# uzh-rpg/rpg_ramnet

Measured on AMD Instinct MI355X. Metric: depth samples/sec (346x260 cropped to 256x344, 5-bin grids, K=5 grids + 1 frame per sample; training step), higher is better.
Workload: dtype f32; 1 GPU; EventScape-shaped 346x260 -> 256x344 crop, 5 event bins, K=5, batch 8/GPU, seq-len 8, 1xMI355X-per-rank train, state=convgru, SI loss on [image,events4], Adam, backward-weights co-scheduled on a side stream, decoders on a second stream; global_batch=8, seq_len=8, parallelism=dp1

## Files before the change

include/ramnet_hip.h:

```cpp
#ifndef RAMNET_HIP_H
#define RAMNET_HIP_H
#include <stddef.h>
#include <stdint.h>

#ifdef __cplusplus
extern "C" {
#endif

#define RAMNET_ABI_VERSION 25
#define RAMNET_E_BADARG 10001
#define RAMNET_E_UNSUPPORTED 10002

enum ramnet_in_mode {
    RAMNET_IN_PLAIN = 0,
    RAMNET_IN_CAT = 1,
    RAMNET_IN_CAT_MUL = 2,
    RAMNET_IN_UP2X = 3,
    RAMNET_IN_UP2X_SKIP = 4,
    RAMNET_IN_RELUMASK = 5,
    RAMNET_IN_S2D = 6,
    RAMNET_IN_PARITY4 = 7
};

enum ramnet_algo { RAMNET_ALGO_DIRECT = 0, RAMNET_ALGO_WINOGRAD = 1, RAMNET_ALGO_HEAD = 2, RAMNET_ALGO_WINOGRAD24 = 3, RAMNET_ALGO_WINOGRAD_2X4 = 4,
                   RAMNET_ALGO_WINOGRAD_2X4_SPLIT = 5, RAMNET_ALGO_DIRECT_SPLIT = 6 };

enum ramnet_epilogue {
    RAMNET_EPI_LINEAR = 0,
    RAMNET_EPI_RELU = 1,
    RAMNET_EPI_SIGMOID = 2,
    RAMNET_EPI_RES_RELU = 3,
    RAMNET_EPI_GRU_BLEND = 4,
    RAMNET_EPI_LSTM = 5,
    RAMNET_EPI_GRU_BWD = 6,
    RAMNET_EPI_SIGMOID_HR = 7
};

typedef struct ramnet_conv_desc {
    const float *x0, *x1, *xm;
    int ld0, ld1, ldm;
    int C0, C1;
    int in_mode;
    int B, Hin, Win;
    int ntaps, stride;
    int8_t dy[25], dx[25];
    uint8_t wtap[25];
    const float *w;
    const float *bias;
    int Cout;
    int Ho, Wo;
    int HoF, WoF;
    int osy, osx, ooy, oox;
    int epi;
    float beta;
    const float *e0, *e1;
    int lde0, lde1;
    float *out, *o1, *o2;
    int ldo, ldo1, ldo2;
    int algo;
    int frame;
    int out_s2d;
    int head_cin;
    int s2d_5x5;
    float *splitk_ws;
    size_t splitk_floats;
    const int *active;
} ramnet_conv_desc;

#define RAMNET_WGRAD_MAX_SEGMENTS 48
typedef struct ramnet_wgrad_seg {
    const float *x0, *x1, *xm, *dout, *gmask;
} ramnet_wgrad_seg;

typedef struct ramnet_wgrad_desc {
    const float *x0, *x1, *xm;
    int ld0, ld1, ldm, C0, C1, in_mode;
    int B, Hin, Win;
    int ntaps, stride;
    int8_t dy[25], dx[25];
    const float *dout, *gmask;
    int ldg, ldgm;
    int Cout, Ho, Wo;
    float *dw;
    float *dbias;
    int algo;
    int gsy, gsx, goy, gox;
    int HoG, WoG;
    int head_cin;
    int dw_slabs;
    int nseg;
    const ramnet_wgrad_seg *segs;
} ramnet_wgrad_desc;

int ramnet_set_option(const char *name, int value);
int ramnet_get_option(const char *name);
const char *ramnet_last_error(void);
int ramnet_abi_version(void);
const char *ramnet_last_kernel(void);
int ramnet_stream_fork(void *from, void *to);

int ramnet_gemm(const float *A, const float *B, float *C, int M, int N, int K, int lda, int ldb, int ldc, int trans_a,
                int accumulate, int batch, long stride_a, long stride_b, long stride_c, void *stream);
int ramnet_gemm2(const float *A, const float *B, float *C, int M, long stride_a, long stride_b, long stride_c, int batch, const float *A2,
                 const float *B2, float *C2, int M2, long stride_a2, long stride_b2, long stride_c2, int batch2, int N, int K, int K2, int lda,
                 int ldb, int ldc, int trans_a, int accumulate, void *stream);

int ramnet_nchw_to_nhwc_pad(const float *src, float *dst, int B, int C, int H, int W, int Cpad, void *stream);
int ramnet_reflect_pad(const float *src, float *dst, int B, int C, int H, int W, int Cpad, int top, int left, int Hc, int Wc, int nhwc,
                       void *stream);
int ramnet_wgrad_wino_slabs(int Cin, int Cout);
int ramnet_wgrad_wino2x4_slabs(int Cin, int Cout);
int ramnet_wgrad_dsplit_slabs(int Cin, int Cout);
size_t ramnet_wgrad_dsplit_ws_floats(int Cin, int Cout);
int ramnet_unpack_wgrad_dsplit(const float *ws, float *grad, int Cout, int Cin, int CinWs, int CoutWs, int n_off, void *stream);
size_t ramnet_wgrad_wino2x4_ws_floats(int Cin, int Cout);
int ramnet_reduce_slabs(float *ws, int slabs, size_t n, void *stream);
size_t ramnet_packed_weight_elems(int Cout, int Cin, int KH, int KW, int transposed, int gates);
size_t ramnet_packed_weight_elems_wino(int Cout, int Cin, int transposed, int gates);
int ramnet_pack_weight_wino(const float *w_oihw, float *wp, int Cout, int Cin, int transposed, int gates, void *stream);
size_t ramnet_packed_weight_elems_wino2x4(int Cout, int Cin, int transposed);
int ramnet_pack_weight_wino2x4(const float *w_oihw, float *wp, int Cout, int Cin, int transposed, void *stream);
int ramnet_conv_wino_variant(const ramnet_conv_desc *d, int force);
int ramnet_conv_wino_split_ok(const ramnet_conv_desc *d, int force);
size_t ramnet_packed_weight_elems_wino2x4_split(int Cout, int Cin, int transposed);
int ramnet_pack_weight_wino2x4_split(const float *w_oihw, float *wp, int Cout, int Cin, int transposed, void *stream);
size_t ramnet_conv_splitk_floats(const ramnet_conv_desc *d);
int ramnet_wino2x4_config(int min_wgs);
int ramnet_fold_wino_supported(int Cout, int Cin);
size_t ramnet_packed_weight_elems_fold_wino(int Cout, int Cin);
int ramnet_pack_weight_fold_wino(const float *w_oihw, float *wp, int Cout, int Cin, void *stream);
int ramnet_pack_weight_fold_wino_dgrad(const float *w_oihw, float *wp, int Cout, int Cin, void *stream);
int ramnet_pack_border_weights(const float *w_oihw, float *rows, float *cols, float *rows_t, float *cols_t, int Cout, int Cin, void *stream);
int ramnet_fold_unpack_wgrad(float *w4, float *dU, float *wr, float *wc, float *grad, int Cout, int Cin, int CinWs, void *stream);
size_t ramnet_packed_weight_elems_head(int Cin);
int ramnet_head_supported(int Cin, int Cout);
int ramnet_pack_weight_head(const float *w_oihw, float *wp, int Cout, int Cin, void *stream);
int ramnet_pack_weight(const float *w_oihw, float *wp, int Cout, int Cin, int KH, int KW,
                       int transposed, int gates, void *stream);
int ramnet_unpack_wgrad(const float *ws, float *grad_oihw, int Cout, int Cin, int CinWs, int CoutWs, int n_off,
                        int KH, int KW, void *stream);

int ramnet_unpack_wgrad_wino(const float *ws, float *grad_oihw, int Cout, int Cin, int CinWs, int CoutWs, int n_off,
                             void *stream);
int ramnet_unpack_wgrad_wino2x4(const float *ws, float *grad_oihw, int Cout, int Cin, int CinWs, int CoutWs, int n_off,
                                void *stream);

int ramnet_conv_launch(const ramnet_conv_desc *d, void *stream);
int ramnet_conv_launch_multi(const ramnet_conv_desc *descs, int n, void *stream);
int ramnet_wgrad_launch(const ramnet_wgrad_desc *d, void *stream);

int ramnet_pred_sigmoid_fwd(const float *x, int ldx, int C, const float *w, const float *b, float *y,
                            size_t npix, void *stream);
int ramnet_pred_sigmoid_bwd(const float *x, int ldx, int C, const float *w, const float *y, const float *dy,
                            float *dx, int lddx, float *dw, float *db, size_t npix, void *stream);
#define RAMNET_PRED_SI_MAX_SEGMENTS 8
size_t ramnet_pred_si_scratch_doubles(size_t seg_pix, int nseg);
int ramnet_pred_sigmoid_si_fwd(const float *x, int ldx, int C, const float *w, const float *b, float *y, size_t seg_pix, int nseg,
                               const float *const *targets, float weight, float lambda, double *scratch, double *stats, float *loss,
                               void *stream);
int ramnet_pred_sigmoid_si_bwd(const float *x, int ldx, int C, const float *w, const float *y, const float *dy, size_t seg_pix, int nseg,
                               const float *const *targets, const double *stats, const float *gscale, float weight, float lambda,
                               float *dx, int lddx, float *dw, float *db, double *scratch, int mask_x, void *stream);
int ramnet_pred_linear_fwd(const float *x, int ldx, int C, const float *w, const float *b, float *z, size_t npix, void *stream);
int ramnet_pred_linear_bwd(const float *x, int ldx, int C, const float *w, const float *dz, float *dx, int lddx, float *dw, float *db,
                           size_t npix, void *stream);
int ramnet_relu_bwd(const float *dy, const float *y, float *dx, size_t n, void *stream);
int ramnet_pad2_sum(const float *x, const float *skip, float *out, int B, int H, int W, int C, void *stream);
int ramnet_up2x_border_im2col(const float *x, const float *skip, float *rows, float *cols, int B, int H, int W, int C, void *stream);
int ramnet_pad2_sum_im2col(const float *x, const float *skip, float *out, float *rows, float *cols, int B, int H, int W, int C, void *stream);
int ramnet_unpad2_fold(const float *dxpad, float *dx, int B, int H, int W, int C, void *stream);
int ramnet_up2x_border_col2im(const float *rows, const float *cols, float *dx, int B, int H, int W, int C, void *stream);
int ramnet_frame_gather(const float *dy, const float *mask, float *rows, float *cols, int B, int H2, int W2, int C, void *stream);
int ramnet_space_to_depth2(const float *x, float *out, int B, int H, int W, int C, int inverse, void *stream);
int ramnet_upsample2x_bwd(const float *dup, float *dx, int B, int H, int W, int C, void *stream);
int ramnet_gru_bwd_a(const float *dhn, const float *ur, const float *o, const float *h, float *dpo,
                     float *dpur, float *dh, size_t npix, int C, int ld_dhn ,
                     void *stream);
int ramnet_gru_bwd_a2(const float *dhn, const float *ur, const float *o, const float *h, float *dpo,
                      float *dpur, float *dh, size_t npix, int C, int ld_dhn, int ld_dh ,
                      void *stream);
int ramnet_gru_bwd_b(const float *dxhr, const float *ur, const float *h, float *dpur, float *dh,
                     size_t npix, int C, void *stream);
int ramnet_lstm_bwd(const float *gates, const float *cprev, const float *cnew, const float *dhn,
                    const float *dcn, float *dpre, float *dcprev, size_t npix, int C, void *stream);
int ramnet_lstm_bwd_masked(const float *gates, const float *cprev, const float *cnew, const float *dhn, const float *dcn,
                           const int *active, float *dpre, float *dcprev, float *dxh, size_t npix, int hw, int C, void *stream);
int ramnet_bias_grad(const float *dy, const float *mask, float *db, size_t npix, int C, void *stream);
int ramnet_norm_slabs(int groups, long npix, int C);
int ramnet_norm_partial(const float *a, int lda, const float *y, int ldy, int act, const float *b, int ldb, int groups, long npix,
                        int C, int nslab, double *part, void *stream);
int ramnet_norm_finalize(const double *part, int groups, int nslab, int C, long npix, double eps, const float *gamma, const float *beta,
                         float *running_mean, float *running_var, double momentum, int update_running, int use_running,
                         long long *num_batches_tracked, double *mean, double *rstd, float *scale, float *shift, void *stream);
int ramnet_norm_finalize_bwd(const double *part, int groups, int nslab, int C, long npix, const double *mean, const double *rstd,
                             const float *gamma, int batch_stats, float *c1, float *c2, float *c3, float *dgamma, float *dbeta, void *stream);
int ramnet_norm_apply(const float *x, int ldx, const float *scale, const float *shift, const float *res, int ldr, int act, float *out,
                      int ldo, int groups, long npix, int C, void *stream);
int ramnet_norm_bwd(const float *dy, int lddy, const float *y, int ldy, int act, const float *x, int ldx, const float *c1, const float *c2,
                    const float *c3, float *dx, int lddx, float *dres, int lddres, int groups, long npix, int C, void *stream);
int ramnet_add(const float *a, const float *b, float *y, size_t n, void *stream);
int ramnet_concat2(const float *a, int lda, int Ca, const float *b, int ldb, int Cb, float *y, size_t npix, void *stream);
int ramnet_cat_batch_add(const float *const *parts, int n, size_t npix, int C, int ld, const float *base, float *out, void *stream);
int ramnet_cat_batch_add_masked(const float *const *parts, int n, size_t npix, int C, int ld, const float *base, const float *mask, float *out,
                                void *stream);
int ramnet_split2(const float *y, int ldy, int Ca, int Cb, float *a, float *b, size_t npix, void *stream);

int ramnet_si_loss_fwd(const float *pred, const float *target, size_t n, float weight, float lambda,
                       double *stats, float *loss, void *stream);
int ramnet_si_loss_from_stats(const double *stats, float weight, float lambda, float *loss, void *stream);
int ramnet_si_loss_bwd(const float *pred, const float *target, size_t n, float weight, float lambda,
                       const double *stats, const float *gscale, float *dpred, void *stream);

int ramnet_si_log_loss_fwd(const float *pred, const float *target, size_t n, float lambda, double *stats, float *loss, void *stream);
int ramnet_si_log_loss_bwd(const float *pred, const float *target, size_t n, float lambda, const double *stats, const float *gscale,
                           float *dpred, void *stream);
int ramnet_mse_loss_fwd(const float *pred, const float *target, int B, int H, int W, int half, double *stats, float *loss, void *stream);
int ramnet_mse_loss_bwd(const float *pred, const float *target, int B, int H, int W, int half, const double *stats, const float *gscale,
                        float *dpred, void *stream);

int ramnet_depth_metrics(const float *pred, const float *target, size_t n, float clip_distance, float reg_factor,
                         float cutoff, double *out11, void *stream);

size_t ramnet_msg_workspace_elems(int B, int H, int W, int num_scales);
int ramnet_msg_loss_fwd(const float *pred, const float *target, int B, int H, int W, int num_scales, float *ws,
                        double *stats, float *loss, void *stream);
int ramnet_msg_loss_bwd(const float *ws, const double *stats, const float *gscale, int B, int H, int W, int num_scales,
                        float *dws, float *dpred, void *stream);

int ramnet_voxelize(const double *events, size_t n_events, int bins, int W, int H, float *grid, void *stream);
int ramnet_voxel_indices(const double *events, size_t n_events, int bins, int W, int H,
                         long long *idx_left, long long *idx_right, void *stream);
int ramnet_normalize_nonzero(float *grid, size_t n, double *scratch, void *stream);
int ramnet_voxelize_batch(const double *events, const long long *offsets, int n_grids, size_t max_events, int bins, int W, int H,
                          float *grids, void *stream);
int ramnet_normalize_nonzero_batch(float *grids, int n_grids, size_t n, double *scratch, void *stream);

#ifdef __cplusplus
}
#endif
#endif
```

rpg_ramnet_amd/_hip.py:

```python
import ctypes as C
import os

_PKG = os.path.dirname(os.path.abspath(__file__))
LIB_PATH = os.environ.get("RAMNET_HIP_LIB") or os.path.join(_PKG, "librpg_ramnet_hip.so")

IN_PLAIN, IN_CAT, IN_CAT_MUL, IN_UP2X, IN_UP2X_SKIP, IN_RELUMASK, IN_S2D, IN_PARITY4 = range(8)
ALGO_DIRECT, ALGO_WINOGRAD, ALGO_HEAD, ALGO_WINOGRAD24, ALGO_WINOGRAD_2X4, ALGO_WINOGRAD_2X4_SPLIT, ALGO_DIRECT_SPLIT = 0, 1, 2, 3, 4, 5, 6
EPI_LINEAR, EPI_RELU, EPI_SIGMOID, EPI_RES_RELU, EPI_GRU_BLEND, EPI_LSTM, EPI_GRU_BWD, EPI_SIGMOID_HR = range(8)

_fp = C.c_void_p


class ConvDesc(C.Structure):
    _fields_ = [
        ("x0", _fp), ("x1", _fp), ("xm", _fp),
        ("ld0", C.c_int), ("ld1", C.c_int), ("ldm", C.c_int),
        ("C0", C.c_int), ("C1", C.c_int), ("in_mode", C.c_int),
        ("B", C.c_int), ("Hin", C.c_int), ("Win", C.c_int),
        ("ntaps", C.c_int), ("stride", C.c_int),
        ("dy", C.c_int8 * 25), ("dx", C.c_int8 * 25), ("wtap", C.c_uint8 * 25),
        ("w", _fp), ("bias", _fp),
        ("Cout", C.c_int), ("Ho", C.c_int), ("Wo", C.c_int), ("HoF", C.c_int), ("WoF", C.c_int),
        ("osy", C.c_int), ("osx", C.c_int), ("ooy", C.c_int), ("oox", C.c_int),
        ("epi", C.c_int), ("beta", C.c_float),
        ("e0", _fp), ("e1", _fp), ("lde0", C.c_int), ("lde1", C.c_int),
        ("out", _fp), ("o1", _fp), ("o2", _fp),
        ("ldo", C.c_int), ("ldo1", C.c_int), ("ldo2", C.c_int),
        ("algo", C.c_int),
        ("frame", C.c_int),
        ("out_s2d", C.c_int),
        ("head_cin", C.c_int),
        ("s2d_5x5", C.c_int),
        ("splitk_ws", C.c_void_p), ("splitk_floats", C.c_size_t),
        ("active", _fp),
    ]


class WgradSeg(C.Structure):
    _fields_ = [("x0", _fp), ("x1", _fp), ("xm", _fp), ("dout", _fp), ("gmask", _fp)]


WGRAD_MAX_SEGMENTS = 48


class WgradDesc(C.Structure):
    _fields_ = [
        ("x0", _fp), ("x1", _fp), ("xm", _fp),
        ("ld0", C.c_int), ("ld1", C.c_int), ("ldm", C.c_int),
        ("C0", C.c_int), ("C1", C.c_int), ("in_mode", C.c_int),
        ("B", C.c_int), ("Hin", C.c_int), ("Win", C.c_int),
        ("ntaps", C.c_int), ("stride", C.c_int),
        ("dy", C.c_int8 * 25), ("dx", C.c_int8 * 25),
        ("dout", _fp), ("gmask", _fp), ("ldg", C.c_int), ("ldgm", C.c_int),
        ("Cout", C.c_int), ("Ho", C.c_int), ("Wo", C.c_int),
        ("dw", _fp), ("dbias", _fp),
        ("algo", C.c_int),
        ("gsy", C.c_int), ("gsx", C.c_int), ("goy", C.c_int), ("gox", C.c_int), ("HoG", C.c_int), ("WoG", C.c_int),
        ("head_cin", C.c_int),
        ("dw_slabs", C.c_int),
        ("nseg", C.c_int), ("segs", C.POINTER(WgradSeg)),
    ]


_SIGS = {
    "ramnet_abi_version": (C.c_int, []),
    "ramnet_last_error": (C.c_char_p, []),
    "ramnet_set_option": (C.c_int, [C.c_char_p, C.c_int]),
    "ramnet_get_option": (C.c_int, [C.c_char_p]),
    "ramnet_last_kernel": (C.c_char_p, []),
    "ramnet_stream_fork": (C.c_int, [_fp, _fp]),
    "ramnet_gemm": (C.c_int, [_fp, _fp, _fp] + [C.c_int] * 9 + [C.c_long] * 3 + [_fp]),
    "ramnet_gemm2": (C.c_int, [_fp, _fp, _fp, C.c_int, C.c_long, C.c_long, C.c_long, C.c_int, _fp, _fp, _fp, C.c_int, C.c_long, C.c_long, C.c_long,
                               C.c_int, C.c_int, C.c_int, C.c_int, C.c_int, C.c_int, C.c_int, C.c_int, C.c_int, _fp]),
    "ramnet_nchw_to_nhwc_pad": (C.c_int, [_fp, _fp, C.c_int, C.c_int, C.c_int, C.c_int, C.c_int, _fp]),
    "ramnet_reflect_pad": (C.c_int, [_fp, _fp] + [C.c_int] * 10 + [_fp]),
    "ramnet_wgrad_wino_slabs": (C.c_int, [C.c_int, C.c_int]),
    "ramnet_wgrad_wino2x4_slabs": (C.c_int, [C.c_int, C.c_int]),
    "ramnet_wgrad_dsplit_slabs": (C.c_int, [C.c_int, C.c_int]),
    "ramnet_wgrad_dsplit_ws_floats": (C.c_size_t, [C.c_int, C.c_int]),
    "ramnet_unpack_wgrad_dsplit": (C.c_int, [_fp, _fp, C.c_int, C.c_int, C.c_int, C.c_int, C.c_int, _fp]),
    "ramnet_wgrad_wino2x4_ws_floats": (C.c_size_t, [C.c_int, C.c_int]),
    "ramnet_reduce_slabs": (C.c_int, [_fp, C.c_int, C.c_size_t, _fp]),
    "ramnet_packed_weight_elems": (C.c_size_t, [C.c_int] * 6),
    "ramnet_pack_weight": (C.c_int, [_fp, _fp, C.c_int, C.c_int, C.c_int, C.c_int, C.c_int, C.c_int, _fp]),
    "ramnet_packed_weight_elems_wino": (C.c_size_t, [C.c_int] * 4),
    "ramnet_pack_weight_wino": (C.c_int, [_fp, _fp, C.c_int, C.c_int, C.c_int, C.c_int, _fp]),
    "ramnet_packed_weight_elems_wino2x4": (C.c_size_t, [C.c_int] * 3),
    "ramnet_pack_weight_wino2x4": (C.c_int, [_fp, _fp, C.c_int, C.c_int, C.c_int, _fp]),
    "ramnet_wino2x4_config": (C.c_int, [C.c_int]),
    "ramnet_conv_wino_variant": (C.c_int, [C.POINTER(ConvDesc), C.c_int]),
    "ramnet_conv_wino_split_ok": (C.c_int, [C.POINTER(ConvDesc), C.c_int]),
    "ramnet_packed_weight_elems_wino2x4_split": (C.c_size_t, [C.c_int] * 3),
    "ramnet_pack_weight_wino2x4_split": (C.c_int, [_fp, _fp, C.c_int, C.c_int, C.c_int, _fp]),
    "ramnet_conv_splitk_floats": (C.c_size_t, [C.POINTER(ConvDesc)]),
    "ramnet_packed_weight_elems_head": (C.c_size_t, [C.c_int]),
    "ramnet_head_supported": (C.c_int, [C.c_int, C.c_int]),
    "ramnet_pack_weight_head": (C.c_int, [_fp, _fp, C.c_int, C.c_int, _fp]),
    "ramnet_fold_wino_supported": (C.c_int, [C.c_int, C.c_int]),
    "ramnet_packed_weight_elems_fold_wino": (C.c_size_t, [C.c_int, C.c_int]),
    "ramnet_pack_weight_fold_wino": (C.c_int, [_fp, _fp, C.c_int, C.c_int, _fp]),
    "ramnet_pack_weight_fold_wino_dgrad": (C.c_int, [_fp, _fp, C.c_int, C.c_int, _fp]),
    "ramnet_pack_border_weights": (C.c_int, [_fp] * 5 + [C.c_int, C.c_int, _fp]),
    "ramnet_fold_unpack_wgrad": (C.c_int, [_fp] * 5 + [C.c_int, C.c_int, C.c_int, _fp]),
    "ramnet_unpad2_fold": (C.c_int, [_fp, _fp, C.c_int, C.c_int, C.c_int, C.c_int, _fp]),
    "ramnet_up2x_border_col2im": (C.c_int, [_fp, _fp, _fp, C.c_int, C.c_int, C.c_int, C.c_int, _fp]),
    "ramnet_pad2_sum": (C.c_int, [_fp, _fp, _fp, C.c_int, C.c_int, C.c_int, C.c_int, _fp]),
    "ramnet_up2x_border_im2col": (C.c_int, [_fp, _fp, _fp, _fp, C.c_int, C.c_int, C.c_int, C.c_int, _fp]),
    "ramnet_pad2_sum_im2col": (C.c_int, [_fp, _fp, _fp, _fp, _fp, C.c_int, C.c_int, C.c_int, C.c_int, _fp]),
    "ramnet_space_to_depth2": (C.c_int, [_fp, _fp, C.c_int, C.c_int, C.c_int, C.c_int, C.c_int, _fp]),
    "ramnet_frame_gather": (C.c_int, [_fp, _fp, _fp, _fp, C.c_int, C.c_int, C.c_int, C.c_int, _fp]),
    "ramnet_unpack_wgrad": (C.c_int, [_fp, _fp] + [C.c_int] * 7 + [_fp]),
    "ramnet_unpack_wgrad_wino": (C.c_int, [_fp, _fp] + [C.c_int] * 5 + [_fp]),
    "ramnet_unpack_wgrad_wino2x4": (C.c_int, [_fp, _fp] + [C.c_int] * 5 + [_fp]),
    "ramnet_conv_launch": (C.c_int, [C.POINTER(ConvDesc), _fp]),
    "ramnet_conv_launch_multi": (C.c_int, [C.POINTER(ConvDesc), C.c_int, _fp]),
    "ramnet_wgrad_launch": (C.c_int, [C.POINTER(WgradDesc), _fp]),
    "ramnet_pred_sigmoid_fwd": (C.c_int, [_fp, C.c_int, C.c_int, _fp, _fp, _fp, C.c_size_t, _fp]),
    "ramnet_pred_sigmoid_bwd": (C.c_int, [_fp, C.c_int, C.c_int, _fp, _fp, _fp, _fp, C.c_int, _fp, _fp, C.c_size_t, _fp]),
    "ramnet_pred_si_scratch_doubles": (C.c_size_t, [C.c_size_t, C.c_int]),
    "ramnet_pred_sigmoid_si_fwd": (C.c_int, [_fp, C.c_int, C.c_int, _fp, _fp, _fp, C.c_size_t, C.c_int, C.POINTER(C.c_void_p), C.c_float, C.c_float,
                                             _fp, _fp, _fp, _fp]),
    "ramnet_pred_sigmoid_si_bwd": (C.c_int, [_fp, C.c_int, C.c_int, _fp, _fp, _fp, C.c_size_t, C.c_int, C.POINTER(C.c_void_p), _fp, _fp, C.c_float,
                                             C.c_float, _fp, C.c_int, _fp, _fp, _fp, C.c_int, _fp]),
    "ramnet_pred_linear_fwd": (C.c_int, [_fp, C.c_int, C.c_int, _fp, _fp, _fp, C.c_size_t, _fp]),
    "ramnet_pred_linear_bwd": (C.c_int, [_fp, C.c_int, C.c_int, _fp, _fp, _fp, C.c_int, _fp, _fp, C.c_size_t, _fp]),
    "ramnet_cat_batch_add": (C.c_int, [_fp, C.c_int, C.c_size_t, C.c_int, C.c_int, _fp, _fp, _fp]),
    "ramnet_cat_batch_add_masked": (C.c_int, [_fp, C.c_int, C.c_size_t, C.c_int, C.c_int, _fp, _fp, _fp, _fp]),
    "ramnet_relu_bwd": (C.c_int, [_fp, _fp, _fp, C.c_size_t, _fp]),
    "ramnet_upsample2x_bwd": (C.c_int, [_fp, _fp, C.c_int, C.c_int, C.c_int, C.c_int, _fp]),
    "ramnet_gru_bwd_a": (C.c_int, [_fp] * 7 + [C.c_size_t, C.c_int, C.c_int, _fp]),
    "ramnet_gru_bwd_a2": (C.c_int, [_fp] * 7 + [C.c_size_t, C.c_int, C.c_int, C.c_int, _fp]),
    "ramnet_gru_bwd_b": (C.c_int, [_fp] * 5 + [C.c_size_t, C.c_int, _fp]),
    "ramnet_lstm_bwd": (C.c_int, [_fp] * 7 + [C.c_size_t, C.c_int, _fp]),
    "ramnet_lstm_bwd_masked": (C.c_int, [_fp, _fp, _fp, _fp, _fp, _fp, _fp, _fp, _fp, C.c_size_t, C.c_int, C.c_int, _fp]),
    "ramnet_norm_slabs": (C.c_int, [C.c_int, C.c_long, C.c_int]),
    "ramnet_norm_partial": (C.c_int, [_fp, C.c_int, _fp, C.c_int, C.c_int, _fp, C.c_int, C.c_int, C.c_long, C.c_int, C.c_int, _fp, _fp]),
    "ramnet_norm_finalize": (C.c_int, [_fp, C.c_int, C.c_int, C.c_int, C.c_long, C.c_double, _fp, _fp, _fp, _fp, C.c_double, C.c_int, C.c_int,
                                       _fp, _fp, _fp, _fp, _fp, _fp]),
    "ramnet_norm_finalize_bwd": (C.c_int, [_fp, C.c_int, C.c_int, C.c_int, C.c_long, _fp, _fp, _fp, C.c_int, _fp, _fp, _fp, _fp, _fp, _fp]),
    "ramnet_norm_apply": (C.c_int, [_fp, C.c_int, _fp, _fp, _fp, C.c_int, C.c_int, _fp, C.c_int, C.c_int, C.c_long, C.c_int, _fp]),
    "ramnet_norm_bwd": (C.c_int, [_fp, C.c_int, _fp, C.c_int, C.c_int, _fp, C.c_int, _fp, _fp, _fp, _fp, C.c_int, _fp, C.c_int,
                                  C.c_int, C.c_long, C.c_int, _fp]),
    "ramnet_add": (C.c_int, [_fp, _fp, _fp, C.c_size_t, _fp]),
    "ramnet_split2": (C.c_int, [_fp, C.c_int, C.c_int, C.c_int, _fp, _fp, C.c_size_t, _fp]),
    "ramnet_concat2": (C.c_int, [_fp, C.c_int, C.c_int, _fp, C.c_int, C.c_int, _fp, C.c_size_t, _fp]),
    "ramnet_bias_grad": (C.c_int, [_fp, _fp, _fp, C.c_size_t, C.c_int, _fp]),
    "ramnet_si_loss_fwd": (C.c_int, [_fp, _fp, C.c_size_t, C.c_float, C.c_float, _fp, _fp, _fp]),
    "ramnet_si_loss_from_stats": (C.c_int, [_fp, C.c_float, C.c_float, _fp, _fp]),
    "ramnet_si_loss_bwd": (C.c_int, [_fp, _fp, C.c_size_t, C.c_float, C.c_float, _fp, _fp, _fp, _fp]),
    "ramnet_si_log_loss_fwd": (C.c_int, [_fp, _fp, C.c_size_t, C.c_float, _fp, _fp, _fp]),
    "ramnet_si_log_loss_bwd": (C.c_int, [_fp, _fp, C.c_size_t, C.c_float, _fp, _fp, _fp, _fp]),
    "ramnet_mse_loss_fwd": (C.c_int, [_fp, _fp, C.c_int, C.c_int, C.c_int, C.c_int, _fp, _fp, _fp]),
    "ramnet_mse_loss_bwd": (C.c_int, [_fp, _fp, C.c_int, C.c_int, C.c_int, C.c_int, _fp, _fp, _fp, _fp]),
    "ramnet_depth_metrics": (C.c_int, [_fp, _fp, C.c_size_t, C.c_float, C.c_float, C.c_float, _fp, _fp]),
    "ramnet_msg_workspace_elems": (C.c_size_t, [C.c_int] * 4),
    "ramnet_msg_loss_fwd": (C.c_int, [_fp, _fp, C.c_int, C.c_int, C.c_int, C.c_int, _fp, _fp, _fp, _fp]),
    "ramnet_msg_loss_bwd": (C.c_int, [_fp, _fp, _fp, C.c_int, C.c_int, C.c_int, C.c_int, _fp, _fp, _fp]),
    "ramnet_voxelize": (C.c_int, [_fp, C.c_size_t, C.c_int, C.c_int, C.c_int, _fp, _fp]),
    "ramnet_voxel_indices": (C.c_int, [_fp, C.c_size_t, C.c_int, C.c_int, C.c_int, _fp, _fp, _fp]),
    "ramnet_normalize_nonzero": (C.c_int, [_fp, C.c_size_t, _fp, _fp]),
    "ramnet_voxelize_batch": (C.c_int, [_fp, _fp, C.c_int, C.c_size_t, C.c_int, C.c_int, C.c_int, _fp, _fp]),
    "ramnet_normalize_nonzero_batch": (C.c_int, [_fp, C.c_int, C.c_size_t, _fp, _fp]),
}
EXPORTS = tuple(_SIGS)

_lib = None
_tracer = None


class _Traced:
    def __init__(self, l):
        self._l = l

    def __getattr__(self, name):
        fn = getattr(self._l, name)
        tr = _tracer
        if tr is None:
            return fn
        return lambda *a: tr(name, fn, a)


def set_tracer(fn):
    global _tracer
    _tracer = fn


class HipLibraryMissing(RuntimeError):
    pass


def lib():
    global _lib
    if _lib is None:
        if not os.path.exists(LIB_PATH):
            raise HipLibraryMissing(
                "%s not found: build it with `python -c 'import __graft_entry__ as g; g.build()'` "
                "(hipcc --offload-arch=gfx950). rpg_ramnet_amd has no CPU fallback." % LIB_PATH)
        import torch
        rt = os.path.join(os.path.dirname(torch.__file__), "lib", "libamdhip64.so")
        if os.path.exists(rt):
            C.CDLL(rt, mode=C.RTLD_GLOBAL)
        l = C.CDLL(LIB_PATH)
        for name, (res, args) in _SIGS.items():
            fn = getattr(l, name)
            fn.restype, fn.argtypes = res, args
        if l.ramnet_abi_version() != 25:
            raise RuntimeError("ABI version mismatch in %s" % LIB_PATH)
        _lib = l
    return _lib if _tracer is None else _Traced(_lib)


def check(code, what):
    if code != 0:
        msg = lib().ramnet_last_error()
        raise RuntimeError("%s failed (code %d): %s" % (what, code, msg.decode() if msg else "?"))
```

rpg_ramnet_amd/csrc/conv_igemm.hip:

```cpp
#include <stdlib.h>
#include "common.hpp"
#include "conv_epilogue.hpp"

namespace ramnet {

struct ConvCommon {
    InSrc src;
    int nchunks, CoutPad;
    int patch_floats;
    int nclass;
    int xcd_swizzle;
};

struct ConvClass {
    int ntaps, Ho, Wo, ooy, oox;
    int PH, PW, dymin, dxmin;
    int tiles_x, tiles_y;
    int toff[25];
    unsigned woff[25];
};
struct ConvClasses { ConvClass c[4]; };

template <int BM, int BN, int WM, int WN, bool MASK = false>
__global__ void __launch_bounds__(256) conv_igemm_kernel(const ramnet_conv_desc p, const ConvCommon qc, const ConvClasses qk) {
    int flat = blockIdx.x + gridDim.x * (blockIdx.y + gridDim.y * blockIdx.z);
    if (qc.xcd_swizzle) {
        const int nwg = gridDim.x * gridDim.y * gridDim.z, xcd = flat & 7, qq = nwg >> 3, rr = nwg & 7;
        flat = (xcd < rr ? xcd * (qq + 1) : rr * (qq + 1) + (xcd - rr) * qq) + (flat >> 3);
    }
    int bid = flat % gridDim.x;
    const int by = (flat / gridDim.x) % gridDim.y, bz = flat / (gridDim.x * gridDim.y);
    const ConvClass &q = qk.c[bz];
    constexpr int TM = BM / WM / 32, TN = BN / WN / 32;
    constexpr int TH = BM / TWID;
    constexpr int CKC = CK;
    static_assert(WM * WN == 4 && TM >= 1 && TN >= 1, "4 waves per workgroup");
    extern __shared__ __attribute__((aligned(16))) float smem[];
    float *patch = smem;
    float *wsm = smem + qc.patch_floats;

    const int tid = threadIdx.x, lane = tid & 63;
    const int wave = __builtin_amdgcn_readfirstlane(tid >> 6);
    const int wm = wave / WN, wn = wave % WN;
    const int l31 = lane & 31, kk = lane >> 5;

    if (bid >= q.tiles_x * q.tiles_y * p.B) return;
    const int tx_i = bid % q.tiles_x;
    bid /= q.tiles_x;
    const int ty_i = bid % q.tiles_y;
    const int b = bid / q.tiles_y;
    const int n0 = by * BN;
    const int oy0 = ty_i * TH, ox0 = tx_i * TWID;
    const int iy0 = oy0 * p.stride + q.dymin, ix0 = ox0 * p.stride + q.dxmin;

    int aBase[TM], bBase[TN];
#pragma unroll
    for (int ms = 0; ms < TM; ++ms) {
        const int m = (wm * TM + ms) * 32 + l31;
        aBase[ms] = (((m >> 4) * p.stride) * q.PW + (m & 15) * p.stride) * LDP + 4 * kk;
    }
#pragma unroll
    for (int ns = 0; ns < TN; ++ns) bBase[ns] = ((wn * TN + ns) * 32 + l31) * LDP + 4 * kk;

    f32x16 acc[TM][TN];
#pragma unroll
    for (int ms = 0; ms < TM; ++ms)
#pragma unroll
        for (int ns = 0; ns < TN; ++ns)
#pragma unroll
            for (int r = 0; r < 16; ++r) acc[ms][ns][r] = 0.f;

    constexpr int WF4 = BN * 4;
    constexpr int WPT = (WF4 + 255) / 256;
    float4 wreg[WPT];
    const int ntaps = q.ntaps;
    auto load_w = [&](int chunk, int t) {
        const float *src = p.w + ((size_t)q.woff[t] + ((size_t)chunk * qc.CoutPad + n0)) * 16;
#pragma unroll
        for (int i = 0; i < WPT; ++i) {
            const int f = tid + i * 256;
            if (WF4 % 256 == 0 || f < WF4) wreg[i] = ld4(src + (size_t)f * 4);
        }
    };
    auto store_w = [&](int buf) {
        float *dst = wsm + buf * (BN * LDP);
#pragma unroll
        for (int i = 0; i < WPT; ++i) {
            const int f = tid + i * 256;
            if (WF4 % 256 == 0 || f < WF4) st4(dst + (f >> 2) * LDP + (f & 3) * 4, wreg[i]);
        }
    };

    load_w(0, 0);
    int buf = 0;
    for (int chunk = 0; chunk < qc.nchunks; ++chunk) {
        __syncthreads();
        stage_patch<CKC / 4, LDP, 4, 256>(patch, qc.src, b, iy0, ix0, chunk * CKC, q.PH, q.PW, tid);
        for (int t = 0; t < ntaps; ++t) {
            store_w(buf);
            __syncthreads();
            if (t + 1 < ntaps) load_w(chunk, t + 1);
            else if (chunk + 1 < qc.nchunks) load_w(chunk + 1, 0);
            const float *pa = patch + q.toff[t];
            const float *wb = wsm + buf * (BN * LDP);
#pragma unroll
            for (int k8 = 0; k8 < 2; ++k8) {
                float4 a[TM], bb[TN];
#pragma unroll
                for (int ms = 0; ms < TM; ++ms) a[ms] = ld4(pa + aBase[ms] + k8 * 8);
#pragma unroll
                for (int ns = 0; ns < TN; ++ns) bb[ns] = ld4(wb + bBase[ns] + k8 * 8);
#pragma unroll
                for (int ms = 0; ms < TM; ++ms)
#pragma unroll
                    for (int ns = 0; ns < TN; ++ns) {
                        acc[ms][ns] = __builtin_amdgcn_mfma_f32_32x32x2f32(a[ms].x, bb[ns].x, acc[ms][ns], 0, 0, 0);
                        acc[ms][ns] = __builtin_amdgcn_mfma_f32_32x32x2f32(a[ms].y, bb[ns].y, acc[ms][ns], 0, 0, 0);
                        acc[ms][ns] = __builtin_amdgcn_mfma_f32_32x32x2f32(a[ms].z, bb[ns].z, acc[ms][ns], 0, 0, 0);
                        acc[ms][ns] = __builtin_amdgcn_mfma_f32_32x32x2f32(a[ms].w, bb[ns].w, acc[ms][ns], 0, 0, 0);
                    }
            }
            buf ^= 1;
        }
    }

    const int epi = p.epi;
    const bool act = !MASK || sample_active(p, b);
#pragma unroll
    for (int ms = 0; ms < TM; ++ms) {
#pragma unroll
        for (int r = 0; r < 16; ++r) {
            const int m = (wm * TM + ms) * 32 + (r & 3) + 8 * (r >> 2) + 4 * kk;
            const int oy = oy0 + (m >> 4), ox = ox0 + (m & 15);
            if (oy >= q.Ho || ox >= q.Wo) continue;
            const size_t pix = ((size_t)b * p.HoF + (oy * p.osy + q.ooy)) * p.WoF + (ox * p.osx + q.oox);
            const bool addold = epilogue_addold(p, oy * p.osy + q.ooy, ox * p.osx + q.oox);
            if (epi == RAMNET_EPI_LSTM) {
                if constexpr (TN == 4) {
                    const int C = p.Cout, ch = by * 32 + l31;
                    if (MASK && !act) {
                        if (ch < C) epilogue_inactive(p, epi, pix, ch);
                    } else if (ch < C) {
                        const float gi = sigmoidf_(acc[ms][0][r] + p.bias[ch]);
                        const float gf = sigmoidf_(acc[ms][1][r] + p.bias[C + ch]);
                        const float go = sigmoidf_(acc[ms][2][r] + p.bias[2 * C + ch]);
                        const float gc = tanhf_(acc[ms][3][r] + p.bias[3 * C + ch]);
                        const float cp = p.e1 ? p.e1[pix * p.lde1 + ch] : 0.f;
                        const float cn = gf * cp + gi * gc;
                        p.out[pix * p.ldo + ch] = go * tanhf_(cn);
                        p.o1[pix * p.ldo1 + ch] = cn;
                        if (p.o2) {
                            float *g = p.o2 + pix * p.ldo2 + ch;
                            g[0] = gi, g[C] = gf, g[2 * C] = go, g[3 * C] = gc;
                        }
                    }
                }
                continue;
            }
#pragma unroll
            for (int ns = 0; ns < TN; ++ns) {
                const int n = n0 + (wn * TN + ns) * 32 + l31;
                if (n >= p.Cout) continue;
                if (MASK && !act) {
                    epilogue_inactive(p, epi, pix, n);
                    continue;
                }
                epilogue_store(p, epi, pix, n, acc[ms][ns][r] + epilogue_side(p, epi, b, oy * p.osy + q.ooy, ox * p.osx + q.oox, n), addold);
            }
        }
    }
}

template <int BM, int BN, int WM, int WN>
static int launch_cfg(const ramnet_conv_desc &d, const ConvCommon &qc, const ConvClasses &qk, int max_tiles, hipStream_t st) {
    auto kern = d.active ? conv_igemm_kernel<BM, BN, WM, WN, true> : conv_igemm_kernel<BM, BN, WM, WN>;
    const size_t lds = ((size_t)qc.patch_floats + 2 * BN * LDP) * sizeof(float);
    static size_t lds_set[2] = {0, 0};
    if (lds > lds_set[d.active != nullptr]) {
        RAMNET_FULL_LDS((kern));
        lds_set[d.active != nullptr] = 160 * 1024;
    }
    if (lds > 160 * 1024) {
        set_error("conv patch does not fit LDS (%zu bytes)", lds);
        return RAMNET_E_UNSUPPORTED;
    }
    dim3 grid(max_tiles * d.B, qc.CoutPad / BN, qc.nclass);
    note_kernel(d.active ? "conv_igemm_kernel<%d,%d,%d,%d,masked>" : "conv_igemm_kernel<%d,%d,%d,%d>", BM, BN, WM, WN);
    hipLaunchKernelGGL(kern, grid, dim3(256), lds, st, d, qc, qk);
    RAMNET_LAUNCH_CHECK();
    return 0;
}

static int check_desc(const ramnet_conv_desc &d) {
    RAMNET_CHECK_ARG(d.x0 && d.w && d.out);
    RAMNET_CHECK_ARG(d.ntaps >= 1 && d.ntaps <= 25 && (d.stride == 1 || d.stride == 2));
    RAMNET_CHECK_ARG(d.B > 0 && d.Ho > 0 && d.Wo > 0 && d.Hin > 0 && d.Win > 0 && d.Cout > 0);
    RAMNET_CHECK_ARG(d.C0 > 0 && d.C0 % 4 == 0 && d.ld0 % 4 == 0 && d.ldo > 0);
    RAMNET_CHECK_ARG(d.osy >= 1 && d.osx >= 1);
    const bool cat = d.in_mode == RAMNET_IN_CAT || d.in_mode == RAMNET_IN_CAT_MUL;
    if (cat) RAMNET_CHECK_ARG(d.x1 && d.C1 > 0 && d.C1 % 4 == 0 && d.ld1 % 4 == 0);
    if (d.in_mode == RAMNET_IN_CAT_MUL || d.in_mode == RAMNET_IN_RELUMASK) RAMNET_CHECK_ARG(d.xm && d.ldm % 4 == 0);
    if (d.in_mode == RAMNET_IN_UP2X_SKIP) RAMNET_CHECK_ARG(d.x1 && d.ld1 % 4 == 0);
    if (d.in_mode == RAMNET_IN_UP2X || d.in_mode == RAMNET_IN_UP2X_SKIP) RAMNET_CHECK_ARG(d.Hin % 2 == 0 && d.Win % 2 == 0);
    if (d.epi == RAMNET_EPI_RES_RELU) RAMNET_CHECK_ARG(d.e0);
    if (d.epi == RAMNET_EPI_GRU_BLEND) RAMNET_CHECK_ARG(d.e0);
    if (d.epi == RAMNET_EPI_LSTM) RAMNET_CHECK_ARG(d.o1 && d.bias);
    if (d.epi == RAMNET_EPI_GRU_BWD) RAMNET_CHECK_ARG(d.e0 && d.o1 && d.Cout % 8 == 0 && !d.bias && d.beta == 0.f && d.frame == 0 && d.out_s2d == 0);
    if (d.epi == RAMNET_EPI_SIGMOID_HR) RAMNET_CHECK_ARG(d.e1 && d.o1 && d.Cout % 8 == 0 && d.beta == 0.f && d.frame == 0 && d.out_s2d == 0 &&
                                                         d.algo != RAMNET_ALGO_WINOGRAD24 && d.algo != RAMNET_ALGO_HEAD);
    {
        unsigned long long ld = (unsigned long long)d.ld0;
        if (cat || d.in_mode == RAMNET_IN_UP2X_SKIP) ld = ld > (unsigned long long)d.ld1 ? ld : (unsigned long long)d.ld1;
        if (d.xm) ld = ld > (unsigned long long)d.ldm ? ld : (unsigned long long)d.ldm;
        const unsigned long long px = (unsigned long long)d.B * d.Hin * d.Win * (d.in_mode == RAMNET_IN_S2D ? 4 : 1);
        RAMNET_CHECK_ARG(px * ld < (1ull << 32));
    }
    RAMNET_CHECK_ARG(d.frame >= 0);
    if (d.active) RAMNET_CHECK_ARG((d.epi == RAMNET_EPI_SIGMOID || d.epi == RAMNET_EPI_SIGMOID_HR || d.epi == RAMNET_EPI_GRU_BLEND ||
                                    (d.epi == RAMNET_EPI_LSTM && d.e0)) && d.frame == 0 && d.out_s2d == 0 &&
                                   (d.algo == RAMNET_ALGO_DIRECT || d.algo == RAMNET_ALGO_WINOGRAD || d.algo == RAMNET_ALGO_WINOGRAD_2X4 ||
                                    d.algo == RAMNET_ALGO_WINOGRAD_2X4_SPLIT));
    if (d.frame > 0) RAMNET_CHECK_ARG(d.e0 && d.e1 && (d.epi == RAMNET_EPI_RELU || d.epi == RAMNET_EPI_LINEAR));
    return 0;
}

static int launch_classes(const ramnet_conv_desc *ds, int n, hipStream_t st) {
    const ramnet_conv_desc &d = ds[0];
    for (int i = 0; i < n; ++i) {
        const int rc = check_desc(ds[i]);
        if (rc) return rc;
        RAMNET_CHECK_ARG(ds[i].x0 == d.x0 && ds[i].w == d.w && ds[i].out == d.out && ds[i].stride == d.stride &&
                         ds[i].Cout == d.Cout && ds[i].epi == d.epi && ds[i].osy == d.osy && ds[i].osx == d.osx &&
                         ds[i].B == d.B && ds[i].in_mode == d.in_mode && ds[i].active == d.active);
    }
    const bool cat = d.in_mode == RAMNET_IN_CAT || d.in_mode == RAMNET_IN_CAT_MUL;
    ConvCommon qc;
    ConvClasses qk;
    qc.src.x0 = d.x0, qc.src.x1 = d.x1, qc.src.xm = d.xm;
    qc.src.ld0 = d.ld0, qc.src.ld1 = d.ld1, qc.src.ldm = d.ldm;
    qc.src.C0 = d.C0, qc.src.Cin = d.C0 + (cat ? d.C1 : 0);
    qc.src.mode = d.in_mode, qc.src.Hin = d.Hin, qc.src.Win = d.Win;
    qc.nchunks = cdiv(qc.src.Cin, CK);
    qc.CoutPad = d.epi == RAMNET_EPI_LSTM ? 4 * roundup(d.Cout, 32) : roundup(d.Cout, 32);
    qc.nclass = n;
    qc.xcd_swizzle = 0;
    const int lstm = d.epi == RAMNET_EPI_LSTM;
    int BM = 128, BN = lstm ? 128 : (qc.CoutPad % 128 == 0 ? 128 : qc.CoutPad % 64 == 0 ? 64 : 32);
    auto blocks = [&](int bm, int bn) {
        long t = 0;
        for (int i = 0; i < n; ++i) t += (long)cdiv(ds[i].Wo, TWID) * cdiv(ds[i].Ho, bm / TWID);
        return t * d.B * (qc.CoutPad / bn);
    };
    if (!lstm && BN >= 64) {
        const long want = 768;
        if (blocks(BM, BN) < want) BM = 64;
        if (blocks(BM, BN) < want && BN == 128) BN = 64;
    }
    if (!lstm && BN == 32 && blocks(256, 32) >= 1024)
        BM = 256;
    const int TH = BM / TWID;
    int max_tiles = 0;
    qc.patch_floats = 0;
    for (int i = 0; i < n; ++i) {
        const ramnet_conv_desc &e = ds[i];
        ConvClass &q = qk.c[i];
        int dymin = 127, dymax = -127, dxmin = 127, dxmax = -127;
        for (int t = 0; t < e.ntaps; ++t) {
            dymin = e.dy[t] < dymin ? e.dy[t] : dymin, dymax = e.dy[t] > dymax ? e.dy[t] : dymax;
            dxmin = e.dx[t] < dxmin ? e.dx[t] : dxmin, dxmax = e.dx[t] > dxmax ? e.dx[t] : dxmax;
        }
        q.ntaps = e.ntaps, q.Ho = e.Ho, q.Wo = e.Wo, q.ooy = e.ooy, q.oox = e.oox;
        q.dymin = dymin, q.dxmin = dxmin;
        q.PH = (TH - 1) * e.stride + (dymax - dymin) + 1;
        q.PW = (TWID - 1) * e.stride + (dxmax - dxmin) + 1;
        q.tiles_x = cdiv(e.Wo, TWID), q.tiles_y = cdiv(e.Ho, TH);
        for (int t = 0; t < e.ntaps; ++t) {
            q.toff[t] = ((e.dy[t] - dymin) * q.PW + (e.dx[t] - dxmin)) * LDP;
            q.woff[t] = (unsigned)e.wtap[t] * (unsigned)qc.nchunks * (unsigned)qc.CoutPad;
        }
        if (q.PH * q.PW * LDP > qc.patch_floats) qc.patch_floats = q.PH * q.PW * LDP;
        if (q.tiles_x * q.tiles_y > max_tiles) max_tiles = q.tiles_x * q.tiles_y;
    }
    if (lstm) return launch_cfg<128, 128, 4, 1>(d, qc, qk, max_tiles, st);
    if (BM == 128 && BN == 128) return launch_cfg<128, 128, 2, 2>(d, qc, qk, max_tiles, st);
    if (BM == 128 && BN == 64) return launch_cfg<128, 64, 2, 2>(d, qc, qk, max_tiles, st);
    if (BM == 64 && BN == 128) return launch_cfg<64, 128, 2, 2>(d, qc, qk, max_tiles, st);
    if (BM == 64 && BN == 64) return launch_cfg<64, 64, 2, 2>(d, qc, qk, max_tiles, st);
    if (BM == 256) return launch_cfg<256, 32, 4, 1>(d, qc, qk, max_tiles, st);
    return launch_cfg<128, 32, 4, 1>(d, qc, qk, max_tiles, st);
}

}

using namespace ramnet;

extern "C" int ramnet_conv_launch(const ramnet_conv_desc *dp, void *stream) {
    RAMNET_CHECK_ARG(dp != nullptr);
    if (dp->algo == RAMNET_ALGO_WINOGRAD) {
        const int rc = check_desc(*dp);
        return rc ? rc : launch_wino(*dp, (hipStream_t)stream);
    }
    if (dp->algo == RAMNET_ALGO_WINOGRAD_2X4) {
        const int rc = check_desc(*dp);
        return rc ? rc : launch_wino6(*dp, (hipStream_t)stream);
    }
    if (dp->algo == RAMNET_ALGO_WINOGRAD_2X4_SPLIT) {
        const int rc = check_desc(*dp);
        return rc ? rc : launch_wino6s(*dp, (hipStream_t)stream);
    }
    if (dp->algo == RAMNET_ALGO_WINOGRAD24) {
        const int rc = check_desc(*dp);
        return rc ? rc : launch_wino24(*dp, (hipStream_t)stream);
    }
    if (dp->algo == RAMNET_ALGO_HEAD) {
        const int rc = check_desc(*dp);
        return rc ? rc : launch_head(*dp, (hipStream_t)stream);
    }
    RAMNET_CHECK_ARG(dp->algo == RAMNET_ALGO_DIRECT && dp->in_mode != RAMNET_IN_S2D && dp->out_s2d == 0);
    return launch_classes(dp, 1, (hipStream_t)stream);
}

extern "C" int ramnet_conv_launch_multi(const ramnet_conv_desc *descs, int n, void *stream) {
    RAMNET_CHECK_ARG(descs != nullptr && n >= 1 && n <= 4);
    for (int i = 0; i < n; ++i) RAMNET_CHECK_ARG(descs[i].in_mode != RAMNET_IN_S2D && descs[i].out_s2d == 0);
    return launch_classes(descs, n, (hipStream_t)stream);
}
```

rpg_ramnet_amd/csrc/conv_wino24.hip:

```cpp
#include <stdlib.h>
#include "common.hpp"
#include "conv_epilogue.hpp"

typedef float f32x4 __attribute__((ext_vector_type(4)));

namespace ramnet {

constexpr int W24_PS = 512;
constexpr int W24_V = 25 * W24_PS;

__device__ __forceinline__ float2 ld2f(const float *p) { return *reinterpret_cast<const float2 *>(p); }

__device__ __forceinline__ auto make_rsrc(const void *p, unsigned bytes) {
    const unsigned long long a = (unsigned long long)p;
    const unsigned lo = __builtin_amdgcn_readfirstlane((unsigned)a), hi = __builtin_amdgcn_readfirstlane((unsigned)(a >> 32));
    return __builtin_amdgcn_make_buffer_rsrc((void *)(((unsigned long long)hi << 32) | lo), (short)0, (int)bytes, 0x00020000);
}

#ifdef W24_TRACE
__device__ unsigned long long *g_w24_trace;
#define W24_STAMP(chunk_, slot)                                                                                          \
    do {                                                                                                                 \
        if (lane == 0 && (chunk_) <= 16) g_w24_trace[(((size_t)blockIdx.x * 8 + wave) * 17 + (chunk_)) * 6 + (slot)] = __builtin_amdgcn_s_memtime(); \
    } while (0)
#else
#define W24_STAMP(chunk_, slot)
#endif

struct Wino24Params {
    const float *x;
    const float *wp;
    int Hp, Wp, ldx, nchunks, nblk, tiles_x, tiles_y, Hc, Wc;
    int cpc;
    unsigned xbytes, wbytes;
    int ksplit;
    float *ws;
    int *cnt;
};

template <int NCQ, bool DG, int TXW, bool PAIR = false>
__global__ void __launch_bounds__(512, 1) conv_wino24_kernel(const ramnet_conv_desc p, const Wino24Params q) {
    static_assert(!PAIR || (NCQ == 4 && !DG), "pair mode: forward, 64-column workgroups");
    constexpr int W24_K = NCQ == 4 ? 16 : 8;
    constexpr int W24_TX = TXW, W24_TY = (NCQ == 4 ? 32 : 64) / TXW;
    constexpr int VEC = W24_K / 4;
    constexpr int W24_U = 25 * NCQ * 64 * VEC;
    extern __shared__ __attribute__((aligned(16))) float smem[];
    float *V = smem;
    const int tid = threadIdx.x, lane = tid & 63;
    const int wave = __builtin_amdgcn_readfirstlane(tid >> 6);
    const int l15 = lane & 15, ks = lane >> 4;
    const int th = NCQ == 4 ? wave & 1 : wave & 3, cq = NCQ == 4 ? wave >> 1 : wave >> 2;

    int bid = blockIdx.x;
    const int cls = DG ? 0 : PAIR ? bid & 1 : bid & 3;
    if (!DG) bid >>= PAIR ? 1 : 2;
    const int nb = bid % q.nblk;
    bid /= q.nblk;
    const int tbx = bid % q.tiles_x;
    bid /= q.tiles_x;
    const int tby = bid % q.tiles_y, b = bid / q.tiles_y;
    const int py = PAIR ? cls : cls >> 1, px = PAIR ? 0 : cls & 1;
    const int n0 = nb * 16 * NCQ;

    const int it = tid / W24_K, ik = tid % W24_K;
    const int iy0 = 2 * (tby * W24_TY + it / W24_TX) + py, ix0 = 2 * (tbx * W24_TX + it % W24_TX) + px;
    unsigned rowo[5], colo[5];
    int cur_cls = -1;
    auto set_class = [&](int c) {
        cur_cls = c;
        const int cy = c >> 1, cx = c & 1;
        const int u0 = 2 * (tby * W24_TY + it / W24_TX), v0 = 2 * (tbx * W24_TX + it % W24_TX);
#pragma unroll
        for (int r = 0; r < 5; ++r) {
            const int i = u0 - cy - 3 + r, j = v0 - cx - 3 + r;
            rowo[r] = (unsigned)i < (unsigned)q.Hc ? 4u * (unsigned)((b * q.Hp + 2 * i + cy) * q.Wp * q.ldx) : 0x40000000u;
            colo[r] = (unsigned)j < (unsigned)q.Wc ? 4u * (unsigned)((2 * j + cx) * q.ldx + ik) : 0x40000000u;
        }
    };
    if (!DG) {
#pragma unroll
        for (int r = 0; r < 5; ++r)
            rowo[r] = 4u * (unsigned)((b * q.Hp + min(iy0 + r, q.Hp - 1)) * q.Wp * q.ldx), colo[r] = 4u * (unsigned)(min(ix0 + r, q.Wp - 1) * q.ldx + ik);
    }
    const int ksp = DG ? 1 : q.ksplit;
    const int cps = ((q.nchunks / 2 + ksp - 1) / ksp) * 2, cbeg = DG ? 0 : (int)blockIdx.y * cps;
    const auto xrs = make_rsrc(q.x + cbeg * W24_K, q.xbytes - (unsigned)cbeg * W24_K * 4u);
    const int vdst = NCQ == 4 ? it * 16 + (((ik >> 2) ^ ((it >> 2) & 3)) << 2) + (ik & 3) : it * 8 + (((ik >> 1) ^ ((it >> 3) & 1)) << 1) + (ik & 1);
    float raw[25];
    auto load_raw = [&](int chunk) {
        int soff = chunk * (W24_K * 4);
        if (DG) {
            const int c = chunk / q.cpc;
            if (c != cur_cls) set_class(c);
            soff = (chunk - c * q.cpc) * (W24_K * 4);
        }
#pragma unroll
        for (int r = 0; r < 5; ++r)
#pragma unroll
            for (int c = 0; c < 5; ++c)
                raw[r * 5 + c] = __builtin_bit_cast(float, __builtin_amdgcn_raw_buffer_load_b32(xrs, (int)(rowo[r] + colo[c]), soff, 0));
    };
    int lr_soff = 0;
    auto load_row_begin = [&](int chunk) {
        lr_soff = chunk * (W24_K * 4);
        if (DG) {
            const int c = chunk / q.cpc;
            if (c != cur_cls) set_class(c);
            lr_soff = (chunk - c * q.cpc) * (W24_K * 4);
        }
    };
    auto load_row = [&](int r) {
#pragma unroll
        for (int c = 0; c < 5; ++c)
            raw[r * 5 + c] = __builtin_bit_cast(float, __builtin_amdgcn_raw_buffer_load_b32(xrs, (int)(rowo[r] + colo[c]), lr_soff, 0));
    };
    auto tr_col = [&](int c) {
        const float d0 = raw[c], d1 = raw[5 + c], d2 = raw[10 + c], d3 = raw[15 + c], d4 = raw[20 + c];
        raw[c] = 2.f * (d0 - d2) - d1 + d3;
        raw[5 + c] = d3 - d2 - 2.f * d1;
        raw[10 + c] = 2.f * d1 - 3.f * d2 + d3;
        raw[15 + c] = d3 - d1;
        raw[20 + c] = 2.f * (d1 - d3) - d2 + d4;
    };
    auto tr_row = [&](float *vbuf, int i) {
        const float d0 = raw[i * 5], d1 = raw[i * 5 + 1], d2 = raw[i * 5 + 2], d3 = raw[i * 5 + 3], d4 = raw[i * 5 + 4];
        float *dst = vbuf + (i * 5) * W24_PS + vdst;
        dst[0 * W24_PS] = 2.f * (d0 - d2) - d1 + d3;
        dst[1 * W24_PS] = d3 - d2 - 2.f * d1;
        dst[2 * W24_PS] = 2.f * d1 - 3.f * d2 + d3;
        dst[3 * W24_PS] = d3 - d1;
        dst[4 * W24_PS] = 2.f * (d1 - d3) - d2 + d4;
    };

    const int tile = th * 16 + l15;
    const int aoff = NCQ == 4 ? tile * 16 + ((ks ^ ((tile >> 2) & 3)) << 2) : tile * 8 + ((ks ^ ((tile >> 3) & 1)) << 1);
    constexpr int WPOS = NCQ * 64 * VEC;
    const auto wrs = make_rsrc(q.wp, q.wbytes);
    const int wsrc = (((cls * q.nchunks + cbeg) * q.nblk + nb) * W24_U + cq * (64 * VEC)) * 4;
    const int wlane = lane * VEC * 4;
    auto ldv = [&](const float *ptr) {
        if (VEC == 4) return ld4(ptr);
        const float2 t = ld2f(ptr);
        return make_float4(t.x, t.y, 0.f, 0.f);
    };
    auto ldw = [&](int soff) {
        if constexpr (VEC == 4) {
            return __builtin_bit_cast(float4, __builtin_amdgcn_raw_buffer_load_b128(wrs, wlane, soff, 0));
        } else {
            const float2 t = __builtin_bit_cast(float2, __builtin_amdgcn_raw_buffer_load_b64(wrs, wlane, soff, 0));
            return make_float4(t.x, t.y, 0.f, 0.f);
        }
    };
    const int wchunk = q.nblk * W24_U * 4;

    f32x4 acc[25];
#pragma unroll
    for (int i = 0; i < 25; ++i) acc[i] = f32x4{0.f, 0.f, 0.f, 0.f};

    const int nch = DG ? q.nchunks : min(cps, q.nchunks - cbeg);
    W24_STAMP(16, 0);
    load_raw(0);
    constexpr int RING = 10, DIST = 8;
    float4 bq[RING];
#pragma unroll
    for (int i = 0; i < DIST; ++i) bq[i] = ldw(wsrc + i * (WPOS * 4));
#pragma unroll
    for (int c = 0; c < 5; ++c) tr_col(c);
#pragma unroll
    for (int i = 0; i < 5; ++i) tr_row(V, i);
    load_raw(min(1, nch - 1));
    __syncthreads();

    W24_STAMP(16, 1);
    for (int chunk0 = 0; chunk0 < nch; chunk0 += 2) {
#pragma unroll
        for (int half = 0; half < 2; ++half) {
            const int chunk = chunk0 + half;
            const float *vb = V + half * W24_V;
            float *vn = V + (half ^ 1) * W24_V;
            const int cnext = min(chunk + 1, nch - 1), cnext2 = min(chunk + 2, nch - 1);
            const int wcur = wsrc + chunk * wchunk, wnext = wsrc + cnext * wchunk;
            W24_STAMP(chunk, 0);
            float4 aq[2][2];
            aq[0][0] = ldv(vb + aoff), aq[0][1] = ldv(vb + W24_PS + aoff);
#pragma unroll
            for (int pp = 0; pp < 13; ++pp) {
                const int pos = 2 * pp, g = half * 25 + pos;
                const bool two = pos + 1 < 25;
                if (pos + 2 < 25) aq[(pp + 1) & 1][0] = ldv(vb + (pos + 2) * W24_PS + aoff);
                if (pos + 3 < 25) aq[(pp + 1) & 1][1] = ldv(vb + (pos + 3) * W24_PS + aoff);
                const float4 a0 = aq[pp & 1][0], a1 = aq[pp & 1][1];
#if !defined(W24_ABLATE) || !(W24_ABLATE & 2)
                bq[(g + DIST) % RING] = pos + DIST < 25 ? ldw(wcur + (pos + DIST) * (WPOS * 4)) : ldw(wnext + (pos + DIST - 25) * (WPOS * 4));
                if (two) bq[(g + 1 + DIST) % RING] = pos + 1 + DIST < 25 ? ldw(wcur + (pos + 1 + DIST) * (WPOS * 4)) : ldw(wnext + (pos + 1 + DIST - 25) * (WPOS * 4));
#endif
                const float4 b0 = bq[g % RING], b1 = bq[(g + 1) % RING];
                __builtin_amdgcn_sched_barrier(0);
                acc[pos] = __builtin_amdgcn_mfma_f32_16x16x4f32(a0.x, b0.x, acc[pos], 0, 0, 0);
                if (two) acc[pos + 1] = __builtin_amdgcn_mfma_f32_16x16x4f32(a1.x, b1.x, acc[pos + 1], 0, 0, 0);
                acc[pos] = __builtin_amdgcn_mfma_f32_16x16x4f32(a0.y, b0.y, acc[pos], 0, 0, 0);
                if (two) acc[pos + 1] = __builtin_amdgcn_mfma_f32_16x16x4f32(a1.y, b1.y, acc[pos + 1], 0, 0, 0);
                __builtin_amdgcn_sched_barrier(0);
                auto slot = [&](int sl) {
                    if (sl == 4) W24_STAMP(chunk, 1);
                    if (sl >= 4 && sl <= 8) tr_col(sl - 4);
                    if (sl == 9) W24_STAMP(chunk, 2);
                    if (sl >= 9 && sl <= 17 && (sl & 1)) tr_row(vn, (sl - 9) >> 1);
#if !defined(W24_ABLATE) || !(W24_ABLATE & 1)
                    if (sl == 10) load_row_begin(cnext2);
                    if (sl >= 10 && sl <= 18 && !(sl & 1)) load_row((sl - 10) >> 1);
#endif
                    if (sl == 18) W24_STAMP(chunk, 3);
                };
                slot(2 * pp);
                __builtin_amdgcn_sched_barrier(0);
                if (VEC == 4) {
                    acc[pos] = __builtin_amdgcn_mfma_f32_16x16x4f32(a0.z, b0.z, acc[pos], 0, 0, 0);
                    if (two) acc[pos + 1] = __builtin_amdgcn_mfma_f32_16x16x4f32(a1.z, b1.z, acc[pos + 1], 0, 0, 0);
                    acc[pos] = __builtin_amdgcn_mfma_f32_16x16x4f32(a0.w, b0.w, acc[pos], 0, 0, 0);
                    if (two) acc[pos + 1] = __builtin_amdgcn_mfma_f32_16x16x4f32(a1.w, b1.w, acc[pos + 1], 0, 0, 0);
                }
                __builtin_amdgcn_sched_barrier(0);
                slot(2 * pp + 1);
                __builtin_amdgcn_sched_barrier(0);
            }
            W24_STAMP(chunk, 4);
            __syncthreads();
            W24_STAMP(chunk, 5);
        }
    }
    W24_STAMP(16, 2);

    const int ncol = n0 + cq * 16 + l15;
    const int pxc = PAIR ? ncol >> 5 : px, n = PAIR ? ncol & 31 : ncol;
    if (n >= p.Cout) return;
    const int epi = p.epi;
    const float bias_n = (!DG && p.bias) ? p.bias[n] : 0.f;
    const bool relu = epi == RAMNET_EPI_RELU;
    float ov[16];
    size_t op[16];
    bool oo[16];
#pragma unroll
    for (int r = 0; r < 4; ++r) {
        float s[2][5];
#pragma unroll
        for (int j = 0; j < 5; ++j) {
            const float m0 = acc[j][r], m1 = acc[5 + j][r], m2 = acc[10 + j][r], m3 = acc[15 + j][r], m4 = acc[20 + j][r];
            s[0][j] = m0 + m1 + m2 + m3;
            s[1][j] = m1 - m2 + 2.f * m3 + m4;
        }
#pragma unroll
        for (int a2 = 0; a2 < 2; ++a2) {
            ov[(r * 2 + a2) * 2] = s[a2][0] + s[a2][1] + s[a2][2] + s[a2][3];
            ov[(r * 2 + a2) * 2 + 1] = s[a2][1] - s[a2][2] + 2.f * s[a2][3] + s[a2][4];
        }
    }
    if (!DG && ksp > 1) {
        typedef unsigned u32x4 __attribute__((ext_vector_type(4)));
        constexpr int AUX_SC1 = 16;
        const auto wr = make_rsrc(q.ws + (size_t)blockIdx.x * ksp * 8192, (unsigned)(ksp * 8192 * 4));
#pragma unroll
        for (int i = 0; i < 4; ++i)
            __builtin_amdgcn_raw_buffer_store_b128(__builtin_bit_cast(u32x4, make_float4(ov[4 * i], ov[4 * i + 1], ov[4 * i + 2], ov[4 * i + 3])), wr,
                                                   (i * 512 + tid) * 16, (int)blockIdx.y * 32768, AUX_SC1);
        __builtin_amdgcn_fence(__ATOMIC_RELEASE, "workgroup");
        __syncthreads();
        if (tid == 0) {
            const int arrived = __hip_atomic_fetch_add(q.cnt + blockIdx.x, 1, __ATOMIC_RELAXED, __HIP_MEMORY_SCOPE_AGENT);
            if (arrived == ksp - 1) __hip_atomic_store(q.cnt + blockIdx.x, 0, __ATOMIC_RELAXED, __HIP_MEMORY_SCOPE_AGENT);
            reinterpret_cast<int *>(smem)[0] = arrived == ksp - 1;
        }
        __syncthreads();
        if (!reinterpret_cast<int *>(smem)[0]) return;
#pragma unroll
        for (int i = 0; i < 16; ++i) ov[i] = 0.f;
        for (int sp = 0; sp < ksp; ++sp)
#pragma unroll
            for (int i = 0; i < 4; ++i) {
                const float4 t = __builtin_bit_cast(float4, __builtin_amdgcn_raw_buffer_load_b128(wr, (i * 512 + tid) * 16, sp * 32768, AUX_SC1));
                ov[4 * i] += t.x, ov[4 * i + 1] += t.y, ov[4 * i + 2] += t.z, ov[4 * i + 3] += t.w;
            }
    }
#pragma unroll
    for (int r = 0; r < 4; ++r) {
        const int t = th * 16 + 4 * ks + r;
        const int oy0 = 2 * (tby * W24_TY + t / W24_TX), ox0 = 2 * (tbx * W24_TX + t % W24_TX) - (PAIR ? pxc : 0);
#pragma unroll
        for (int a2 = 0; a2 < 2; ++a2) {
#pragma unroll
            for (int c2 = 0; c2 < 2; ++c2) {
                const int oy = oy0 + a2, ox = ox0 + c2, idx = (r * 2 + a2) * 2 + c2;
                if (DG) {
                    oo[idx] = oy < p.Ho && ox < p.Wo;
                    op[idx] = (((size_t)b * p.Ho + oy) * p.Wo + ox) * p.ldo + n;
                    continue;
                }
                oo[idx] = !(oy >= q.Hc || ox >= q.Wc || (PAIR && ox < 0));
                const int oyF = 2 * oy + py, oxF = 2 * ox + pxc;
                op[idx] = (((size_t)b * p.HoF + oyF) * p.WoF + oxF) * p.ldo + n;
                float v = ov[idx] + bias_n;
                if (oo[idx]) v += epilogue_side(p, epi, b, oyF, oxF, n);
                ov[idx] = relu ? fmaxf(v, 0.f) : v;
            }
        }
    }
#pragma unroll
    for (int idx = 0; idx < 16; ++idx)
        if (oo[idx]) p.out[op[idx]] = ov[idx];
    W24_STAMP(16, 3);
}

__global__ void pack_weight_fold_wino_kernel(const float *__restrict__ w, float *__restrict__ wp, int Cout, int Cin, int kc, int ncq,
                                             int pair, size_t total) {
    const double FA[2][4][5] = {{{.25, 0, 0, 0, 0}, {.75, .75, .25, 0, 0}, {0, .25, .75, .75, .25}, {0, 0, 0, .25, .75}},
                                {{.75, .25, 0, 0, 0}, {.25, .75, .75, .25, 0}, {0, 0, .25, .75, .75}, {0, 0, 0, 0, .25}}};
    const double G[5][4] = {{0.5, 0, 0, 0}, {-0.5, -0.5, -0.5, -0.5}, {-1.0 / 6, 1.0 / 6, -1.0 / 6, 1.0 / 6}, {1.0 / 6, 1.0 / 3, 2.0 / 3, 4.0 / 3}, {0, 0, 0, 1}};
    const int vec = kc / 4, nblk = pair ? 1 : Cout / (16 * ncq), nch = Cin / kc;
    for (size_t i = blockIdx.x * (size_t)blockDim.x + threadIdx.x; i < total; i += (size_t)gridDim.x * blockDim.x) {
        size_t r = i;
        const int j = (int)(r % vec);
        r /= vec;
        const int l15 = (int)(r % 16);
        r /= 16;
        const int ks = (int)(r % 4);
        r /= 4;
        const int cq = (int)(r % ncq);
        r /= ncq;
        const int pos = (int)(r % 25);
        r /= 25;
        const int nb = (int)(r % nblk);
        r /= nblk;
        const int chunk = (int)(r % nch), cls = (int)(r / nch);
        const int k = chunk * kc + ks * vec + j, col = (nb * ncq + cq) * 16 + l15;
        const int n = pair ? col & 31 : col;
        const int py = pair ? cls : cls >> 1, px = pair ? col >> 5 : cls & 1, a = pos / 5, b = pos % 5;
        double ga[5], gb[5];
        for (int kh = 0; kh < 5; ++kh) {
            ga[kh] = 0, gb[kh] = 0;
            for (int t = 0; t < 4; ++t) ga[kh] += G[a][t] * FA[py][t][kh], gb[kh] += G[b][t] * FA[px][t][kh];
        }
        double u = 0;
        const float *wk = w + ((size_t)n * Cin + k) * 25;
        for (int kh = 0; kh < 5; ++kh)
            for (int kw = 0; kw < 5; ++kw) u += ga[kh] * gb[kw] * (double)wk[kh * 5 + kw];
        wp[i] = (float)u;
    }
}

static bool fold_wino_pair(int Cout, int Cin) {
    return Cout == 32 && Cin % 32 == 0 && g_opt_fold_pair;
}

static bool fold_wino_geometry(int Cout, int Cin, int &kc, int &ncq) {
    kc = ((Cout % 64 == 0 && Cin % 16 == 0) || fold_wino_pair(Cout, Cin)) ? 16 : 8, ncq = kc == 16 ? 4 : 2;
    return Cout % 32 == 0 && Cin % (2 * kc) == 0;
}

static int launch_wino24_dgrad(const ramnet_conv_desc &d, hipStream_t st) {
    RAMNET_CHECK_ARG(d.stride == 1 && d.C0 % 16 == 0 && d.Cout % 64 == 0);
    RAMNET_CHECK_ARG(d.Hin % 2 == 0 && d.Win % 2 == 0 && d.Ho == d.Hin / 2 + 4 && d.Wo == d.Win / 2 + 4 && d.HoF == d.Ho && d.WoF == d.Wo);
    RAMNET_CHECK_ARG(d.epi == RAMNET_EPI_LINEAR && !d.bias && d.beta == 0.f && d.frame == 0 && d.out_s2d == 0);
    Wino24Params q;
    q.x = d.x0, q.wp = d.w, q.Hp = d.Hin, q.Wp = d.Win, q.ldx = d.ld0;
    q.cpc = d.C0 / 16, q.nchunks = 4 * q.cpc, q.nblk = d.Cout / 64;
    q.ksplit = 1, q.ws = nullptr, q.cnt = nullptr;
    q.Hc = d.Hin / 2, q.Wc = d.Win / 2;
    const size_t xb = (size_t)d.B * d.Hin * d.Win * d.ld0 * sizeof(float), wb = (size_t)100 * d.C0 * d.Cout * sizeof(float);
    RAMNET_CHECK_ARG(xb < 0x40000000ull && wb < 0x7fffffffull);
    q.xbytes = (unsigned)xb, q.wbytes = (unsigned)wb;
    const bool flat = cdiv(d.Wo, 16) * cdiv(d.Ho, 8) < cdiv(d.Wo, 8) * cdiv(d.Ho, 16);
    q.tiles_x = cdiv(d.Wo, flat ? 16 : 8), q.tiles_y = cdiv(d.Ho, flat ? 8 : 16);
    const size_t lds = (size_t)2 * W24_V * sizeof(float);
    const dim3 grid((unsigned)(q.tiles_x * q.tiles_y * d.B * q.nblk));
    if (flat) {
        RAMNET_FULL_LDS((conv_wino24_kernel<4, true, 8>));
        note_kernel("conv_wino24_kernel<4,1,8,0>");
        hipLaunchKernelGGL((conv_wino24_kernel<4, true, 8>), grid, dim3(512), lds, st, d, q);
    } else {
        RAMNET_FULL_LDS((conv_wino24_kernel<4, true, 4>));
        note_kernel("conv_wino24_kernel<4,1,4,0>");
        hipLaunchKernelGGL((conv_wino24_kernel<4, true, 4>), grid, dim3(512), lds, st, d, q);
    }
    RAMNET_LAUNCH_CHECK();
    return 0;
}

static int wino24_ksplit(const ramnet_conv_desc &d, int gridx, int nchunks) {
    if (!g_opt_wino_ksplit || d.in_mode != RAMNET_IN_PLAIN) return 1;
    const bool pair = fold_wino_pair(d.Cout, d.C0), wide = pair || (d.Cout % 64 == 0 && d.C0 % 16 == 0);
    if (!pair && d.Cout % (wide ? 64 : 32) != 0) return 1;
    int ks = 256 / gridx < 4 ? 256 / gridx : 4;
    if (nchunks / 4 < ks) ks = nchunks / 4;
    if (g_opt_wino_ksplit > 1) ks = g_opt_wino_ksplit < nchunks / 2 ? g_opt_wino_ksplit : nchunks / 2;
    if (ks < 1) ks = 1;
    while (ks > 1 && (ks - 1) * (cdiv(nchunks / 2, ks) * 2) >= nchunks) --ks;
    return ks;
}
static size_t wino24_ksplit_floats(unsigned gridx, int ks) { return (size_t)cdiv((int)gridx, 64) * 64 + (size_t)gridx * ks * 8192; }

size_t wino24_splitk_floats(const ramnet_conv_desc &d) {
    if (d.in_mode != RAMNET_IN_PLAIN || d.C0 % 16 != 0 || d.Cout % 32 != 0) return 0;
    const bool pair = fold_wino_pair(d.Cout, d.C0), wide = pair || (d.Cout % 64 == 0 && d.C0 % 16 == 0);
    if (d.C0 % (wide ? 32 : 16) != 0) return 0;
    const int nchunks = d.C0 / (wide ? 16 : 8), nblk = pair ? 1 : d.Cout / (wide ? 64 : 32);
    const int Wt = pair ? d.Wo + 2 : d.Wo;
    const bool flat = wide && cdiv(Wt, 16) * cdiv(d.Ho, 8) < cdiv(Wt, 8) * cdiv(d.Ho, 16);
    const int tiles_x = cdiv(Wt, wide && !flat ? 8 : 16), tiles_y = cdiv(d.Ho, flat ? 8 : 16);
    const unsigned gridx = (unsigned)(tiles_x * tiles_y * d.B * nblk * (pair ? 2 : 4));
    const int ks = wino24_ksplit(d, (int)gridx, nchunks);
    return ks > 1 ? wino24_ksplit_floats(gridx, ks) : 0;
}

int launch_wino24(const ramnet_conv_desc &d, hipStream_t st) {
    if (d.in_mode == RAMNET_IN_PARITY4) return launch_wino24_dgrad(d, st);
    RAMNET_CHECK_ARG(d.in_mode == RAMNET_IN_PLAIN && d.stride == 1);
    const bool pair = fold_wino_pair(d.Cout, d.C0);
    const bool wide = pair || (d.Cout % 64 == 0 && d.C0 % 16 == 0);
    RAMNET_CHECK_ARG(d.C0 % (wide ? 32 : 16) == 0);
    RAMNET_CHECK_ARG(d.C0 % 8 == 0 && d.Cout % 32 == 0 && d.Hin == d.Ho + 4 && d.Win == d.Wo + 4 && d.HoF == 2 * d.Ho && d.WoF == 2 * d.Wo);
    RAMNET_CHECK_ARG((d.epi == RAMNET_EPI_RELU || d.epi == RAMNET_EPI_LINEAR) && d.beta == 0.f && d.out_s2d == 0 && d.Ho >= 2 && d.Wo >= 2);
    Wino24Params q;
    q.x = d.x0, q.wp = d.w, q.Hp = d.Hin, q.Wp = d.Win, q.ldx = d.ld0;
    q.nchunks = d.C0 / (wide ? 16 : 8), q.nblk = pair ? 1 : d.Cout / (wide ? 64 : 32);
    q.Hc = d.Ho, q.Wc = d.Wo, q.cpc = 1;
    const size_t xb = (size_t)d.B * d.Hin * d.Win * d.ld0 * sizeof(float), wb = (size_t)100 * d.C0 * d.Cout * sizeof(float);
    RAMNET_CHECK_ARG(xb < 0xffffffffull && wb < 0x7fffffffull);
    q.xbytes = (unsigned)xb, q.wbytes = (unsigned)wb;
    const int Wt = pair ? d.Wo + 2 : d.Wo;
    const bool flat = wide && cdiv(Wt, 16) * cdiv(d.Ho, 8) < cdiv(Wt, 8) * cdiv(d.Ho, 16);
    q.tiles_x = cdiv(Wt, wide && !flat ? 8 : 16), q.tiles_y = cdiv(d.Ho, flat ? 8 : 16);
    const size_t lds = (size_t)2 * W24_V * sizeof(float);
    const unsigned gridx = (unsigned)(q.tiles_x * q.tiles_y * d.B * q.nblk * (pair ? 2 : 4));
    const int want = wino24_ksplit(d, (int)gridx, q.nchunks);
    q.ksplit = d.splitk_ws ? want : 1;
    q.cnt = reinterpret_cast<int *>(d.splitk_ws);
    q.ws = d.splitk_ws ? d.splitk_ws + cdiv((int)gridx, 64) * 64 : nullptr;
    if (q.ksplit > 1) RAMNET_CHECK_ARG(d.splitk_floats >= wino24_ksplit_floats(gridx, want) && ((uintptr_t)d.splitk_ws & 15) == 0);
    const dim3 grid(gridx, q.ksplit);
    if (pair && flat) {
        RAMNET_FULL_LDS((conv_wino24_kernel<4, false, 8, true>));
        note_kernel("conv_wino24_kernel<4,0,8,1>");
        hipLaunchKernelGGL((conv_wino24_kernel<4, false, 8, true>), grid, dim3(512), lds, st, d, q);
    } else if (pair) {
        RAMNET_FULL_LDS((conv_wino24_kernel<4, false, 4, true>));
        note_kernel("conv_wino24_kernel<4,0,4,1>");
        hipLaunchKernelGGL((conv_wino24_kernel<4, false, 4, true>), grid, dim3(512), lds, st, d, q);
    } else if (wide && flat) {
        RAMNET_FULL_LDS((conv_wino24_kernel<4, false, 8>));
        note_kernel("conv_wino24_kernel<4,0,8,0>");
        hipLaunchKernelGGL((conv_wino24_kernel<4, false, 8>), grid, dim3(512), lds, st, d, q);
    } else if (wide) {
        RAMNET_FULL_LDS((conv_wino24_kernel<4, false, 4>));
        note_kernel("conv_wino24_kernel<4,0,4,0>");
        hipLaunchKernelGGL((conv_wino24_kernel<4, false, 4>), grid, dim3(512), lds, st, d, q);
    } else {
        RAMNET_FULL_LDS((conv_wino24_kernel<2, false, 8>));
        note_kernel("conv_wino24_kernel<2,0,8,0>");
        hipLaunchKernelGGL((conv_wino24_kernel<2, false, 8>), grid, dim3(512), lds, st, d, q);
    }
    RAMNET_LAUNCH_CHECK();
    return 0;
}

__global__ void pack_weight_fold_wino_dgrad_kernel(const float *__restrict__ w, float *__restrict__ wp, int Cout, int Cin, size_t total) {
    const double FA[2][4][5] = {{{.25, 0, 0, 0, 0}, {.75, .75, .25, 0, 0}, {0, .25, .75, .75, .25}, {0, 0, 0, .25, .75}},
                                {{.75, .25, 0, 0, 0}, {.25, .75, .75, .25, 0}, {0, 0, .25, .75, .75}, {0, 0, 0, 0, .25}}};
    const double G[5][4] = {{0.5, 0, 0, 0}, {-0.5, -0.5, -0.5, -0.5}, {-1.0 / 6, 1.0 / 6, -1.0 / 6, 1.0 / 6}, {1.0 / 6, 1.0 / 3, 2.0 / 3, 4.0 / 3}, {0, 0, 0, 1}};
    const int NB = Cin / 64;
    for (size_t i = blockIdx.x * (size_t)blockDim.x + threadIdx.x; i < total; i += (size_t)gridDim.x * blockDim.x) {
        size_t r = i;
        const int j = (int)(r & 3), l15 = (int)((r >> 2) & 15), ks = (int)((r >> 6) & 3), cq = (int)((r >> 8) & 3);
        r >>= 10;
        const int pos = (int)(r % 25);
        r /= 25;
        const int nb = (int)(r % NB), chunk = (int)(r / NB);
        const int k = chunk * 16 + ks * 4 + j, c = nb * 64 + cq * 16 + l15;
        const int pq = k / Cout, n = k - pq * Cout, pp = pq >> 1, qq = pq & 1, a = pos / 5, b = pos % 5;
        double ga[5], gb[5];
        for (int kh = 0; kh < 5; ++kh) {
            ga[kh] = 0, gb[kh] = 0;
            for (int t = 0; t < 4; ++t) ga[kh] += G[a][t] * FA[pp][3 - t][kh], gb[kh] += G[b][t] * FA[qq][3 - t][kh];
        }
        double u = 0;
        const float *wk = w + ((size_t)n * Cin + c) * 25;
        for (int kh = 0; kh < 5; ++kh)
            for (int kw = 0; kw < 5; ++kw) u += ga[kh] * gb[kw] * (double)wk[kh * 5 + kw];
        wp[i] = (float)u;
    }
}

__global__ void pack_border_weights_kernel(const float *__restrict__ w, float *__restrict__ rows, float *__restrict__ cols, float *__restrict__ rows_t,
                                           float *__restrict__ cols_t, int Cout, int Cin, size_t total) {
    for (size_t i = blockIdx.x * (size_t)blockDim.x + threadIdx.x; i < total; i += (size_t)gridDim.x * blockDim.x) {
        size_t r = i;
        const int co = (int)(r % Cout);
        r /= Cout;
        const int slot = (int)(r & 1);
        r >>= 1;
        const int ci = (int)(r % Cin);
        r /= Cin;
        const int kb = (int)(r % 5), side = (int)(r / 5);
        const int a0 = side == 0 ? 0 : (slot == 0 ? 4 : 3), na = side == 0 ? (slot == 0 ? 2 : 1) : (slot == 0 ? 1 : 2);
        const float *wk = w + ((size_t)co * Cin + ci) * 25;
        float sr = 0.f, sc = 0.f;
        for (int e = 0; e < na; ++e) sr += wk[(a0 + e) * 5 + kb], sc += wk[kb * 5 + (a0 + e)];
        const size_t K = (size_t)kb * Cin + ci, N = (size_t)slot * Cout + co;
        rows[((size_t)side * 5 * Cin + K) * 2 * Cout + N] = -sr;
        cols[((size_t)side * 5 * Cin + K) * 2 * Cout + N] = -sc;
        rows_t[((size_t)side * 2 * Cout + N) * 5 * Cin + K] = -sr;
        cols_t[((size_t)side * 2 * Cout + N) * 5 * Cin + K] = -sc;
    }
}

__global__ void fold_unpack_wgrad_kernel(float *__restrict__ w4, float *__restrict__ dU, float *__restrict__ wr, float *__restrict__ wc,
                                         float *__restrict__ grad, int Cout, int Cin, int CinWs) {
    const float FA[2][4][5] = {{{.25f, 0, 0, 0, 0}, {.75f, .75f, .25f, 0, 0}, {0, .25f, .75f, .75f, .25f}, {0, 0, 0, .25f, .75f}},
                               {{.75f, .25f, 0, 0, 0}, {.25f, .75f, .75f, .25f, 0}, {0, 0, .25f, .75f, .75f}, {0, 0, 0, 0, .25f}}};
    const float G[5][4] = {{0.5f, 0, 0, 0}, {-0.5f, -0.5f, -0.5f, -0.5f}, {-1.f / 6, 1.f / 6, -1.f / 6, 1.f / 6}, {1.f / 6, 1.f / 3, 2.f / 3, 4.f / 3}, {0, 0, 0, 1.f}};
    const size_t total = (size_t)Cout * Cin;
    for (size_t idx = blockIdx.x * (size_t)blockDim.x + threadIdx.x; idx < total; idx += (size_t)gridDim.x * blockDim.x) {
        const int o = (int)(idx % Cout), i = (int)(idx / Cout);
        float g5[25];
        for (int e = 0; e < 25; ++e) g5[e] = 0.f;
        for (int pq = 0; pq < 4; ++pq) {
            const int pp = pq >> 1, qq = pq & 1;
            float d4[16];
            for (int ts = 0; ts < 16; ++ts) {
                float *cell = w4 + ((size_t)(pq * 16 + ts) * CinWs + i) * Cout + o;
                d4[ts] = *cell;
                *cell = 0.f;
            }
            if (dU != nullptr) {
                for (int ab = 0; ab < 25; ++ab) {
                    float *cell = dU + ((size_t)(pq * 25 + ab) * CinWs + i) * Cout + o;
                    const float u = *cell;
                    *cell = 0.f;
                    const int a = ab / 5, b = ab % 5;
                    for (int t = 0; t < 4; ++t)
                        for (int s = 0; s < 4; ++s) d4[t * 4 + s] += G[a][t] * G[b][s] * u;
                }
            }
            for (int t = 0; t < 4; ++t)
                for (int s = 0; s < 4; ++s) {
                    const float v = d4[t * 4 + s];
                    for (int k = 0; k < 5; ++k) {
                        const float fk = FA[pp][t][k] * v;
                        for (int l = 0; l < 5; ++l) g5[k * 5 + l] += fk * FA[qq][s][l];
                    }
                }
        }
        for (int side = 0; side < 2; ++side)
            for (int slot = 0; slot < 2; ++slot) {
                const int a0 = side == 0 ? 0 : (slot == 0 ? 4 : 3), na = side == 0 ? (slot == 0 ? 2 : 1) : (slot == 0 ? 1 : 2);
                for (int kb = 0; kb < 5; ++kb) {
                    float *rc = wr + (((size_t)side * 5 + kb) * Cin + i) * 2 * Cout + (size_t)slot * Cout + o;
                    float *cc = wc + (((size_t)side * 5 + kb) * Cin + i) * 2 * Cout + (size_t)slot * Cout + o;
                    const float r = *rc, c = *cc;
                    *rc = 0.f, *cc = 0.f;
                    for (int e = 0; e < na; ++e) g5[(a0 + e) * 5 + kb] -= r, g5[kb * 5 + (a0 + e)] -= c;
                }
            }
        float *g = grad + ((size_t)o * Cin + i) * 25;
        for (int e = 0; e < 25; ++e) g[e] += g5[e];
    }
}

}

using namespace ramnet;

extern "C" int ramnet_fold_wino_supported(int Cout, int Cin) {
    int kc, ncq;
    return fold_wino_geometry(Cout, Cin, kc, ncq) ? 1 : 0;
}

extern "C" size_t ramnet_packed_weight_elems_fold_wino(int Cout, int Cin) { return (size_t)100 * Cout * Cin; }

extern "C" int ramnet_pack_weight_fold_wino(const float *w, float *wp, int Cout, int Cin, void *stream) {
    int kc, ncq;
    RAMNET_CHECK_ARG(w && wp && Cout > 0 && Cin > 0 && fold_wino_geometry(Cout, Cin, kc, ncq));
    const size_t total = (size_t)100 * Cout * Cin;
    size_t blocks = (total + 255) / 256;
    if (blocks > 65535) blocks = 65535;
    hipLaunchKernelGGL(pack_weight_fold_wino_kernel, dim3((unsigned)blocks), dim3(256), 0, (hipStream_t)stream, w, wp, Cout, Cin, kc, ncq,
                       (int)fold_wino_pair(Cout, Cin), total);
    RAMNET_LAUNCH_CHECK();
    return 0;
}

extern "C" int ramnet_pack_weight_fold_wino_dgrad(const float *w, float *wp, int Cout, int Cin, void *stream) {
    RAMNET_CHECK_ARG(w && wp && Cout > 0 && Cin > 0 && Cin % 64 == 0 && (4 * Cout) % 16 == 0);
    const size_t total = (size_t)100 * Cout * Cin;
    size_t blocks = (total + 255) / 256;
    if (blocks > 65535) blocks = 65535;
    hipLaunchKernelGGL(pack_weight_fold_wino_dgrad_kernel, dim3((unsigned)blocks), dim3(256), 0, (hipStream_t)stream, w, wp, Cout, Cin, total);
    RAMNET_LAUNCH_CHECK();
    return 0;
}

extern "C" int ramnet_pack_border_weights(const float *w, float *rows, float *cols, float *rows_t, float *cols_t, int Cout, int Cin, void *stream) {
    RAMNET_CHECK_ARG(w && rows && cols && rows_t && cols_t && Cout > 0 && Cin > 0);
    const size_t total = (size_t)2 * 5 * Cin * 2 * Cout;
    size_t blocks = (total + 255) / 256;
    if (blocks > 65535) blocks = 65535;
    hipLaunchKernelGGL(pack_border_weights_kernel, dim3((unsigned)blocks), dim3(256), 0, (hipStream_t)stream, w, rows, cols, rows_t, cols_t, Cout, Cin, total);
    RAMNET_LAUNCH_CHECK();
    return 0;
}

extern "C" int ramnet_fold_unpack_wgrad(float *w4, float *dU, float *wr, float *wc, float *grad, int Cout, int Cin, int CinWs, void *stream) {
    RAMNET_CHECK_ARG(w4 && wr && wc && grad && Cout > 0 && Cin > 0 && CinWs >= Cin);
    const size_t total = (size_t)Cout * Cin;
    size_t blocks = (total + 127) / 128;
    if (blocks > 65535) blocks = 65535;
    hipLaunchKernelGGL(fold_unpack_wgrad_kernel, dim3((unsigned)blocks), dim3(128), 0, (hipStream_t)stream, w4, dU, wr, wc, grad, Cout, Cin, CinWs);
    RAMNET_LAUNCH_CHECK();
    return 0;
}
```

rpg_ramnet_amd/ops.py:

```python
import contextlib
import ctypes as C
import os as _os

import torch
from torch.autograd import Function

from . import _hip as H

_NULL = None
_ABL_SKIP_WGRAD = _os.environ.get("RAMNET_ABL_SKIP_WGRAD") == "1"
if _ABL_SKIP_WGRAD:
    import warnings as _warnings
    _warnings.warn("RAMNET_ABL_SKIP_WGRAD=1: backward-weights launches are SKIPPED — every weight gradient of this process is zero "
                   "(tuning runs only; unset the variable for anything else)", RuntimeWarning)

_WINOGRAD = True
_WINO_MIN_CIN = 32


def set_winograd(on):
    global _WINOGRAD
    _WINOGRAD = bool(on)


_WINO_2X4 = "auto"
_WGRAD_SLABS = True
_WGRAD_2X4 = "auto"


def set_wgrad_slabs(on):
    global _WGRAD_SLABS
    _WGRAD_SLABS = bool(on)



def set_winograd_2x4(mode, min_wgs=None):
    global _WINO_2X4
    assert mode in ("auto", "off", "force")
    _WINO_2X4 = mode
    if min_wgs is not None:
        H.check(H.lib().ramnet_wino2x4_config(int(min_wgs)), "wino2x4_config")
        invalidate_descs()


def get_winograd():
    return _WINOGRAD


_FOLD_UP = True


_FOLD_WINO = True
_FOLD_WINO_MIN_COUT = 32
_FOLD_WINO_WGRAD = True
_SAVE_XPAD = False


def set_fold_winograd_wgrad(on):
    global _FOLD_WINO_WGRAD
    _FOLD_WINO_WGRAD = bool(on)


def set_fold_pair(on):
    H.check(H.lib().ramnet_set_option(b"fold_pair", int(bool(on))), "set_option")
    invalidate_packs()
    invalidate_descs()


_GRU_BWD_FUSED = True


def set_gru_bwd_fused(on):
    global _GRU_BWD_FUSED
    _GRU_BWD_FUSED = bool(on)


_GRU_HR = _os.environ.get("RAMNET_GRU_HR", "1") != "0"


def set_gru_materialize_hr(on):
    global _GRU_HR
    _GRU_HR = bool(on)


_SPLIT_OPERANDS = False


def set_split_operands(on):
    global _SPLIT_OPERANDS
    _SPLIT_OPERANDS = bool(on)
    invalidate_descs()


def get_split_operands():
    return _SPLIT_OPERANDS


_SPLIT_WGRAD = _os.environ.get("RAMNET_SPLIT_WGRAD", "0") == "1"


def set_split_wgrad(on):
    global _SPLIT_WGRAD
    _SPLIT_WGRAD = bool(on)


def get_split_wgrad():
    return _SPLIT_WGRAD


def set_wgrad_winograd_2x4(mode):
    global _WGRAD_2X4
    assert mode in ("auto", "off", "force")
    _WGRAD_2X4 = mode


def set_winograd_split(on):
    H.check(H.lib().ramnet_set_option(b"wino_ksplit", int(on)), "set_option")
    invalidate_descs()


def _fold_pair(Cout, Cin):
    return Cout == 32 and Cin % 32 == 0 and bool(H.lib().ramnet_get_option(b"fold_pair"))


def _fold_wino_ok(Cin, Cout):
    kc = 16 if ((Cout % 64 == 0 and Cin % 16 == 0) or _fold_pair(Cout, Cin)) else 8
    return Cout % 32 == 0 and Cout >= _FOLD_WINO_MIN_COUT and Cin % (2 * kc) == 0


def set_fold_winograd(on):
    global _FOLD_WINO
    _FOLD_WINO = bool(on)


def set_fold_upsample(on):
    global _FOLD_UP
    _FOLD_UP = bool(on)


def get_fold_upsample():
    return _FOLD_UP


_RAW_STREAM = getattr(torch._C, "_cuda_getCurrentRawStream", None)
_RAW_DEVICE = getattr(torch._C, "_cuda_getDevice", None)


def _st():
    if _RAW_STREAM is not None and _RAW_DEVICE is not None:
        return C.c_void_p(_RAW_STREAM(_RAW_DEVICE()))
    return C.c_void_p(torch.cuda.current_stream().cuda_stream)


def _p(t, off=0):
    return None if t is None else C.c_void_p(t.data_ptr() + 4 * off)


def dense(t):
    if t is None:
        return None
    B, Hh, W, Cc = t.shape
    s = t.stride()
    ok = (s[3] == 1 or Cc == 1) and s[2] % 4 == 0 and s[1] == W * s[2] and s[0] == Hh * s[1] and t.data_ptr() % 16 == 0
    if ok and t.dtype == torch.float32:
        return t
    return t.contiguous().float()


def ld(t):
    return t.stride(2)


class Taps:
    _cache = {}

    def __init__(self, triples):
        self.n = len(triples)
        assert 1 <= self.n <= 25
        self.dy = (C.c_int8 * 25)(*[t[0] for t in triples])
        self.dx = (C.c_int8 * 25)(*[t[1] for t in triples])
        self.wt = (C.c_uint8 * 25)(*[t[2] for t in triples])
        self.wino = False
        self.head = False
        self.flop_taps = self.n

    @classmethod
    def get(cls, kind, k, pad, py=0, px=0):
        key = (kind, k, pad, py, px)
        if key not in cls._cache:
            if kind in ("conv", "conv_s2d"):
                tr = [(kh - pad, kw - pad, kh * k + kw) for kh in range(k) for kw in range(k)]
            elif kind in ("dgrad1", "dgrad1_s2d"):
                tr = [(pad - kh, pad - kw, kh * k + kw) for kh in range(k) for kw in range(k)]
            elif kind == "dgrad2":
                tr = [((py + pad - kh) // 2, (px + pad - kw) // 2, kh * k + kw)
                      for kh in range(k) for kw in range(k)
                      if (py + pad - kh) % 2 == 0 and (px + pad - kw) % 2 == 0]
            elif kind == "fold":
                tr = [(py + ty, px + tx, (py * 2 + px) * 16 + ty * 4 + tx) for ty in range(4) for tx in range(4)]
            else:
                raise KeyError(kind)
            cls._cache[key] = cls(tr)
            cls._cache[key].wino = kind in ("conv", "dgrad1", "conv_s2d", "dgrad1_s2d") and k == 3 and pad == 1
            cls._cache[key].head = kind == "conv" and k == 5 and pad == 2
            if kind.endswith("_s2d"):
                cls._cache[key].flop_taps = 25.0 / 4.0
            if kind == "fold":
                cls._cache[key].flop_taps = 25
        return cls._cache[key]


def conv_launch(x0, taps, w, out, Cout, active=None, **kw):
    d = _conv_desc(x0, taps, w, out, Cout, **kw)
    if active is not None:
        d.active = _p(active)
    H.check(H.lib().ramnet_conv_launch(C.byref(d), _st()), "ramnet_conv_launch")


def conv_launch_multi(x0, w, out, Cout, classes, **kw):
    arr = (H.ConvDesc * len(classes))()
    if isinstance(w, PackRef):
        w = w.cp.pack(w.transposed, False)
    for i, (taps, Ho, Wo, os_) in enumerate(classes):
        arr[i] = _conv_desc(x0, taps, w, out, Cout, Ho=Ho, Wo=Wo, os=os_, **kw)
    H.check(H.lib().ramnet_conv_launch_multi(arr, len(classes), _st()), "ramnet_conv_launch_multi")


def uses_winograd(taps, w, stride, epi, in_mode, C0, C1):
    return bool(isinstance(w, PackRef) and _WINOGRAD and taps.wino and stride == 1
                and (w.cp.gates == 1 or w.transposed or (epi == H.EPI_LSTM and w.cp.Cout % 16 == 0))
                and (epi != H.EPI_LSTM or w.cp.gates == 4) and in_mode not in (H.IN_UP2X, H.IN_UP2X_SKIP)
                and C0 + C1 >= _WINO_MIN_CIN and (C1 == 0 or C0 % 8 == 0))


_HEAD = True


def set_head_kernel(on):
    global _HEAD
    _HEAD = bool(on)


def get_head_kernel():
    return _HEAD


def uses_head(taps, w, stride, epi, in_mode):
    return bool(isinstance(w, PackRef) and _HEAD and taps.head and stride == 1 and not w.transposed
                and w.cp.gates == 1 and len(w.cp.weights) == 1 and in_mode == H.IN_PLAIN and epi in (H.EPI_LINEAR, H.EPI_RELU)
                and H.lib().ramnet_head_supported(w.cp.Cin, w.cp.Cout))


_DESC_CACHE = {}
_DESC_EPOCH = 0
_DESC_CACHE_ON = _os.environ.get("RAMNET_DESC_CACHE", "1") != "0"


def invalidate_descs():
    global _DESC_EPOCH
    _DESC_EPOCH += 1
    _DESC_CACHE.clear()
    _WDESC_CACHE.clear()


def _sd(t):
    return -1 if t is None else t.stride(2)


def _conv_desc(x0, taps, w, out, Cout, *, stride=1, x1=None, xm=None, xm_off=0, in_mode=H.IN_PLAIN,
               C0=None, C1=0, Hin=None, Win=None, bias=None, epi=H.EPI_LINEAR, beta=0.0, e0=None, e1=None,
               o1=None, o2=None, Ho=None, Wo=None, os=(1, 1, 0, 0), out_off=0, frame=0, out_s2d=0, wino24=False, ws_owner=None):
    is_ref = isinstance(w, PackRef)
    al = out.data_ptr() | (4 * out_off)
    for t in (e0, e1, o1, o2, bias):
        if t is not None:
            al |= t.data_ptr()
    key = (id(taps), id(w.cp) if is_ref else 0, w.transposed if is_ref else -1, id(ws_owner), Cout, stride, in_mode, C0, C1, Hin, Win, epi, beta, Ho,
           Wo, os, out_off, frame, out_s2d, wino24, xm_off, tuple(x0.shape), x0.stride(2), _sd(x1), _sd(xm), out.shape[1], out.shape[2],
           out.stride(2), _sd(e0), _sd(e1), _sd(o1), _sd(o2), bias is None, al & 15, _WINOGRAD, _WINO_2X4, _SPLIT_OPERANDS, _HEAD, _S2D_SPARSE, _S2D_2X4,
           _DESC_EPOCH, x0.device.index)
    hit = _DESC_CACHE.get(key) if _DESC_CACHE_ON else None
    if hit is not None and (not is_ref or hit[3]() is w.cp) and (ws_owner is None or hit[4]() is ws_owner):
        tmpl, kind, nsplit = hit[0], hit[1], hit[2]
        d = H.ConvDesc.from_buffer_copy(tmpl)
        d.x0, d.x1, d.xm = _p(x0), _p(x1), _p(xm, xm_off)
        d.bias, d.e0, d.e1 = _p(bias), _p(e0), _p(e1)
        d.out, d.o1, d.o2 = _p(out, out_off), _p(o1), _p(o2)
        d.w = _p(w) if kind is None else _p(w.cp.pack(0, "head") if kind == "head" else w.cp.pack(w.transposed, kind))
        if nsplit:
            d.splitk_ws = _p((w.cp if is_ref else ws_owner).splitk_ws(nsplit, x0.device))
        return d
    meta = []
    d = _conv_desc_build(x0, taps, w, out, Cout, meta, stride=stride, x1=x1, xm=xm, xm_off=xm_off, in_mode=in_mode, C0=C0, C1=C1, Hin=Hin, Win=Win,
                         bias=bias, epi=epi, beta=beta, e0=e0, e1=e1, o1=o1, o2=o2, Ho=Ho, Wo=Wo, os=os, out_off=out_off, frame=frame,
                         out_s2d=out_s2d, wino24=wino24, ws_owner=ws_owner)
    import weakref
    if len(_DESC_CACHE) > 4096:
        _DESC_CACHE.clear()
    _DESC_CACHE[key] = (H.ConvDesc.from_buffer_copy(d), meta[0], meta[1], weakref.ref(w.cp) if is_ref else None,
                        weakref.ref(ws_owner) if ws_owner is not None else None)
    return d


def _conv_desc_build(x0, taps, w, out, Cout, meta, *, stride=1, x1=None, xm=None, xm_off=0, in_mode=H.IN_PLAIN,
                     C0=None, C1=0, Hin=None, Win=None, bias=None, epi=H.EPI_LINEAR, beta=0.0, e0=None, e1=None,
                     o1=None, o2=None, Ho=None, Wo=None, os=(1, 1, 0, 0), out_off=0, frame=0, out_s2d=0, wino24=False, ws_owner=None):
    B = x0.shape[0]
    kind, nsplit = None, 0
    d = H.ConvDesc()
    d.x0, d.x1, d.xm = _p(x0), _p(x1), _p(xm, xm_off)
    d.ld0, d.ld1, d.ldm = ld(x0), (ld(x1) if x1 is not None else 0), (ld(xm) if xm is not None else 0)
    d.C0, d.C1, d.in_mode = (x0.shape[3] if C0 is None else C0), C1, in_mode
    d.algo = H.ALGO_DIRECT
    ref = None
    cp = w.cp if isinstance(w, PackRef) else ws_owner
    if isinstance(w, PackRef) and beta == 0.0 and frame == 0 and os == (1, 1, 0, 0) and uses_head(taps, w, stride, epi, in_mode):
        d.algo, d.head_cin = H.ALGO_HEAD, w.cp.Cin
        kind = "head"
        w = w.cp.pack(0, "head")
    elif isinstance(w, PackRef):
        wino = uses_winograd(taps, w, stride, epi, in_mode, d.C0, C1)
        d.algo = H.ALGO_WINOGRAD if wino else H.ALGO_DIRECT
        d.s2d_5x5 = int(wino and isinstance(w.cp, S2DConvParam) and _S2D_SPARSE and (in_mode == H.IN_S2D or out_s2d > 0))
        if wino and w.cp.gates == 1 and os == (1, 1, 0, 0) and (_S2D_2X4 or not isinstance(w.cp, S2DConvParam)):
            ref = w
        kind = bool(wino)
        w = w.cp.pack(w.transposed, wino)
    d.B, d.Hin, d.Win = B, (x0.shape[1] if Hin is None else Hin), (x0.shape[2] if Win is None else Win)
    d.ntaps, d.stride = taps.n, stride
    d.dy, d.dx, d.wtap = taps.dy, taps.dx, taps.wt
    d.w, d.bias = _p(w), _p(bias)
    d.Cout = Cout
    d.HoF, d.WoF = out.shape[1], out.shape[2]
    d.Ho, d.Wo = (d.HoF if Ho is None else Ho), (d.WoF if Wo is None else Wo)
    d.osy, d.osx, d.ooy, d.oox = os
    d.epi, d.beta, d.frame, d.out_s2d = epi, beta, frame, out_s2d
    d.e0, d.e1 = _p(e0), _p(e1)
    d.lde0, d.lde1 = (ld(e0) if e0 is not None else 0), (ld(e1) if e1 is not None else 0)
    d.out, d.o1, d.o2 = _p(out, out_off), _p(o1), _p(o2)
    d.ldo, d.ldo1, d.ldo2 = ld(out), (ld(o1) if o1 is not None else 0), (ld(o2) if o2 is not None else 0)
    if wino24:
        d.algo = H.ALGO_WINOGRAD24
    if ref is not None and _WINO_2X4 != "off" and H.lib().ramnet_conv_wino_variant(C.byref(d), int(_WINO_2X4 == "force")):
        d.algo, d.s2d_5x5 = H.ALGO_WINOGRAD_2X4, 0
        kind = "2x4"
        if _SPLIT_OPERANDS and H.lib().ramnet_conv_wino_split_ok(C.byref(d), int(_WINO_2X4 == "force")):
            d.algo, kind = H.ALGO_WINOGRAD_2X4_SPLIT, "2x4s"
        d.w = _p(ref.cp.pack(ref.transposed, kind))
    if d.algo in (H.ALGO_WINOGRAD, H.ALGO_WINOGRAD24) and cp is not None:
        n = H.lib().ramnet_conv_splitk_floats(C.byref(d))
        if n:
            d.splitk_ws, d.splitk_floats = _p(cp.splitk_ws(n, x0.device)), n
            nsplit = n
    meta[:] = [kind, nsplit]
    return d


_WDESC_CACHE = {}


def _wgrad_desc_build(x0, taps, dout, dw, Cout, stride, x1, xm, xm_off, in_mode, C0, C1, Hin, Win, gmask, dbias, Ho, Wo, gview, dw_off, wino24):
    d = H.WgradDesc()
    d.x0, d.x1, d.xm = _p(x0), _p(x1), _p(xm, xm_off)
    d.ld0, d.ld1, d.ldm = ld(x0), (ld(x1) if x1 is not None else 0), (ld(xm) if xm is not None else 0)
    d.C0, d.C1, d.in_mode = (x0.shape[3] if C0 is None else C0), C1, in_mode
    d.B, d.Hin, d.Win = x0.shape[0], (x0.shape[1] if Hin is None else Hin), (x0.shape[2] if Win is None else Win)
    d.ntaps, d.stride = taps.n, stride
    d.dy, d.dx = taps.dy, taps.dx
    d.dout, d.gmask = _p(dout), _p(gmask)
    d.ldg, d.ldgm = ld(dout), (ld(gmask) if gmask is not None else 0)
    d.Cout, d.Ho, d.Wo = Cout, (dout.shape[1] if Ho is None else Ho), (dout.shape[2] if Wo is None else Wo)
    d.dw, d.dbias = _p(dw, dw_off), _p(dbias)
    if gview is not None:
        d.gsy, d.gsx, d.goy, d.gox, d.HoG, d.WoG = gview
    d.algo = H.ALGO_WINOGRAD if getattr(dw, "wino", False) else H.ALGO_DIRECT
    if getattr(dw, "wino6", False):
        d.algo = H.ALGO_WINOGRAD_2X4
    if getattr(dw, "wg_dsplit", False):
        d.algo = H.ALGO_DIRECT_SPLIT
    d.dw_slabs = getattr(dw, "slabs", 0) if (d.algo in (H.ALGO_WINOGRAD, H.ALGO_WINOGRAD_2X4, H.ALGO_DIRECT_SPLIT) and _WGRAD_SLABS) else 0
    if wino24:
        d.algo = H.ALGO_WINOGRAD24
    hc = getattr(dw, "head_cin", 0)
    if hc and _HEAD and taps.head and stride == 1 and in_mode == H.IN_PLAIN and gview is None and dw_off == 0:
        d.algo, d.head_cin = H.ALGO_HEAD, hc
    if d.algo in (H.ALGO_WINOGRAD, H.ALGO_WINOGRAD_2X4) and C1 and d.C0 % 32:
        raise RuntimeError("Winograd backward-weights needs the concatenation boundary at a multiple of 32 channels")
    return d


def wgrad_launch(x0, taps, dout, dw, Cout, *, stride=1, x1=None, xm=None, xm_off=0, in_mode=H.IN_PLAIN, C0=None,
                 C1=0, Hin=None, Win=None, gmask=None, dbias=None, Ho=None, Wo=None, gview=None, dw_off=0, wino24=False, segs=None, stream=None):
    key = (id(taps), id(dw), getattr(dw, "wino", False), getattr(dw, "wino6", False), getattr(dw, "wg_dsplit", False), getattr(dw, "slabs", 0), getattr(dw, "head_cin", 0), Cout, stride,
           in_mode, C0, C1, Hin, Win, Ho, Wo, gview, dw_off, wino24, xm_off, tuple(x0.shape), x0.stride(2), _sd(x1), _sd(xm), dout.shape[1],
           dout.shape[2], dout.stride(2), _sd(gmask), _WGRAD_SLABS, _HEAD, x0.device.index)
    tmpl = _WDESC_CACHE.get(key) if _DESC_CACHE_ON else None
    if tmpl is not None:
        d = H.WgradDesc.from_buffer_copy(tmpl)
        d.x0, d.x1, d.xm = _p(x0), _p(x1), _p(xm, xm_off)
        d.dout, d.gmask = _p(dout), _p(gmask)
        d.dw, d.dbias = _p(dw, dw_off), _p(dbias)
    else:
        d = _wgrad_desc_build(x0, taps, dout, dw, Cout, stride, x1, xm, xm_off, in_mode, C0, C1, Hin, Win, gmask, dbias, Ho, Wo, gview, dw_off, wino24)
        if len(_WDESC_CACHE) > 4096:
            _WDESC_CACHE.clear()
        _WDESC_CACHE[key] = H.WgradDesc.from_buffer_copy(d)
    if segs is not None:
        d.nseg, d.segs = len(segs), C.cast(segs, C.POINTER(H.WgradSeg))
    if _ABL_SKIP_WGRAD:
        return
    H.check(H.lib().ramnet_wgrad_launch(C.byref(d), _st() if stream is None else stream), "ramnet_wgrad_launch")


_SIDE = {}
_USE_SIDE = False


def set_wgrad_overlap(on):
    global _USE_SIDE
    _USE_SIDE = bool(on)
    H.check(H.lib().ramnet_set_option(b"wgrad_wino_nf", 2 if _USE_SIDE else 1), "set_option")


_DECODE = {}
_USE_DECODE = False
_DECODE_USED = set()


def set_decoder_overlap(on):
    global _USE_DECODE
    _USE_DECODE = bool(on)


def decoder_overlap():
    return _USE_DECODE


def decode_stream(dev):
    st = _DECODE.get(dev)
    if st is None:
        st = _DECODE[dev] = torch.cuda.Stream(device=dev)
    _DECODE_USED.add(dev)
    return st


_BRANCH = {}
_USE_BRANCH = False


def set_branch_overlap(on):
    global _USE_BRANCH
    _USE_BRANCH = bool(on)


def branch_overlap():
    return _USE_BRANCH


def branch_stream(dev, i):
    st = _BRANCH.get((dev, i))
    if st is None:
        st = _BRANCH[(dev, i)] = torch.cuda.Stream(device=dev)
    return st


def _side_stream(dev):
    st = _SIDE.get(dev)
    if st is None:
        st = _SIDE[dev] = torch.cuda.Stream(device=dev)
    return st


@contextlib.contextmanager
def side_work(tensors, dev):
    if not _USE_SIDE:
        yield
        return
    side = _side_stream(dev)
    side.wait_event(torch.cuda.current_stream().record_event())
    with torch.cuda.stream(side):
        yield
    for t in tensors:
        if t is not None:
            t.record_stream(side)
    _Engine.side_used = dev


def wgrad_side(tensors, *args, **kw):
    if not _USE_SIDE:
        return wgrad_launch(*args, **kw)
    dev = args[0].device
    side = _side_stream(dev)
    raw = C.c_void_p(side.cuda_stream)
    H.check(H.lib().ramnet_stream_fork(_st(), raw), "ramnet_stream_fork")
    wgrad_launch(*args, stream=raw, **kw)
    for t in tensors:
        if t is not None:
            t.record_stream(side)
    _Engine.side_used = dev


_WGRAD_DEFER = 0


def set_wgrad_defer(n):
    global _WGRAD_DEFER
    n = int(n)
    assert 0 <= n <= H.WGRAD_MAX_SEGMENTS
    _WGRAD_DEFER = n


def wgrad_defer():
    return _WGRAD_DEFER


def _wgrad_cell(cp, dw, tensors, x0, taps, dout, Cout, **kw):
    if _WGRAD_DEFER <= 1 or not getattr(dw, "wino6", False) or not _WGRAD_SLABS:
        return wgrad_side(tensors, x0, taps, dout, dw, Cout, **kw)
    x1, xm = kw.get("x1"), kw.get("xm")
    key = (id(dw), tuple(x0.shape), ld(x0), ld(x1) if x1 is not None else 0, ld(xm) if xm is not None else 0, ld(dout), Cout,
           kw.get("in_mode"), kw.get("C1"), kw.get("xm_off", 0), x0.device)
    q = cp._defer
    if q and q[0][0] != key:
        cp.flush_deferred()
    cp._defer.append((key, tensors, x0, taps, dout, dw, Cout, kw))
    if len(cp._defer) >= _WGRAD_DEFER:
        cp.flush_deferred()


_ZERO_BATCH = None


def _zero_later(t):
    if _ZERO_BATCH is None:
        t.zero_()
    else:
        _ZERO_BATCH.append(t)


class _Engine:
    dirty = []
    task = -1
    side_used = None

    @classmethod
    def enter(cls):
        tid = torch._C._current_graph_task_id()
        if tid != cls.task:
            if cls.dirty:
                cls.reset()
            cls.task = tid
            if tid != -1:
                torch.autograd.Variable._execution_engine.queue_callback(cls.flush)

    @classmethod
    def mark(cls, cp):
        cls.enter()
        if not cp._dirty:
            cp._dirty = True
            cls.dirty.append(cp)

    @classmethod
    def _join(cls):
        for dev in _DECODE_USED:
            torch.cuda.current_stream(dev).wait_stream(_DECODE[dev])
        if cls.side_used is not None:
            torch.cuda.current_stream().wait_event(_side_stream(cls.side_used).record_event())
            cls.side_used = None

    @classmethod
    def flush(cls):
        for cp in cls.dirty:
            cp.flush_deferred()
        cls._join()
        dirty, cls.dirty, cls.task = cls.dirty, [], -1
        hook = _FINALIZE_HOOK if (_FINALIZE_HOOK is not None and not (torch.cuda.is_available() and torch.cuda.is_current_stream_capturing())) else None
        if hook is not None:
            hook.begin(dirty)
        global _ZERO_BATCH
        _ZERO_BATCH = []
        try:
            for cp in dirty:
                cp.finalize()
                if hook is not None:
                    hook.finalized(cp)
        finally:
            zs, _ZERO_BATCH = _ZERO_BATCH, None
            zs = [z for z in zs if z.numel() > 0]
            if zs:
                torch._foreach_zero_(zs)
        if hook is not None and hasattr(hook, "end"):
            hook.end()

    @classmethod
    def reset(cls):
        for cp in cls.dirty:
            cp._defer = []
        cls._join()
        dirty, cls.dirty, cls.task = cls.dirty, [], -1
        for cp in dirty:
            cp.discard()


_FINALIZE_HOOK = None


def set_finalize_hook(hook):
    global _FINALIZE_HOOK
    _FINALIZE_HOOK = hook


def get_finalize_hook():
    return _FINALIZE_HOOK


def ensure_grad(p):
    if p.grad is None:
        p.grad = torch.zeros_like(p)
    return p.grad


FOLD_A = ([[.25, 0, 0, 0, 0], [.75, .75, .25, 0, 0], [0, .25, .75, .75, .25], [0, 0, 0, .25, .75]],
          [[.75, .25, 0, 0, 0], [.25, .75, .75, .25, 0], [0, 0, .25, .75, .75], [0, 0, 0, 0, .25]])


_CONSTS = {}


def _const(name, values, device, dtype):
    key = (name, str(device), dtype)
    t = _CONSTS.get(key)
    if t is None:
        t = _CONSTS[key] = torch.tensor(values, dtype=dtype, device=device)
    return t


def fold_weights(w):
    A = _const("FOLD_A", FOLD_A, w.device, torch.float64)
    return torch.einsum("ptk,qsl,oikl->oipqts", A, A, w.double())


S2D_TAP = [(-1, 0), (-1, 1), (0, 0), (0, 1), (1, 0)]


def s2d_weights(w):
    O, I = w.shape[0], w.shape[1]
    out = w.new_zeros(O, 4, I, 3, 3)
    for ky, (dy, a) in enumerate(S2D_TAP):
        for kx, (dx, b) in enumerate(S2D_TAP):
            out[:, a * 2 + b, :, dy + 1, dx + 1] = w[:, :, ky, kx]
    return out.reshape(O, 4 * I, 3, 3)


_S2D_ADJ_IDX = {}


def s2d_weights_adjoint(g3, I):
    O = g3.shape[0]
    idx = _S2D_ADJ_IDX.get(g3.device)
    if idx is None:
        idx = _S2D_ADJ_IDX[g3.device] = torch.tensor([(a * 2 + b) * 9 + (dy + 1) * 3 + (dx + 1) for (dy, a) in S2D_TAP for (dx, b) in S2D_TAP],
                                                     dtype=torch.int64, device=g3.device)
    t = g3.view(O, 4, I, 9).permute(0, 2, 1, 3).reshape(O, I, 36)
    return t.index_select(2, idx).view(O, I, 5, 5)


_PACK_EPOCH = 0


def invalidate_packs():
    global _PACK_EPOCH
    _PACK_EPOCH += 1


class PackRef:
    __slots__ = ("cp", "transposed")

    def __init__(self, cp, transposed):
        self.cp, self.transposed = cp, transposed


class ConvParam:

    def __init__(self, weights, biases, gates=1):
        self.weights, self.biases, self.gates = list(weights), list(biases), gates
        w0 = self.weights[0]
        self.Cout = sum(w.shape[0] for w in self.weights)
        self.Cin, self.k = w0.shape[1], w0.shape[2]
        self.CinWs = (self.Cin + 3) // 4 * 4
        self._bias = self._ws = self._bws = None
        self._ws_fold = None
        self._fold_used = self._ws_used = False
        self._vbias = None
        self._packs = {}
        self._dirty = False
        self._defer = []

    def flush_deferred(self):
        q, self._defer = self._defer, []
        if not q:
            return
        _, _, x0, taps, dout, dw, Cout, kw = q[0]
        if len(q) == 1:
            return wgrad_side(q[0][1], x0, taps, dout, dw, Cout, **kw)
        segs = (H.WgradSeg * len(q))()
        keep = []
        for i, (_, tensors, xi, _, di, _, _, kwi) in enumerate(q):
            segs[i].x0, segs[i].x1, segs[i].xm = _p(xi), _p(kwi.get("x1")), _p(kwi.get("xm"), kwi.get("xm_off", 0))
            segs[i].dout, segs[i].gmask = _p(di), _p(kwi.get("gmask"))
            keep += list(tensors)
        wgrad_side(keep, x0, taps, dout, dw, Cout, segs=segs, **kw)

    def splitk_ws(self, n, device):
        pool = self.__dict__.setdefault("_splitk", {})
        ws = pool.get(n)
        if ws is None or ws.device != device:
            if torch.cuda.is_current_stream_capturing():
                raise RuntimeError("split-reduction workspace of a layer first used inside a graph capture: run the launch eagerly once "
                                   "before capturing (graph._warm)")
            ws = pool[n] = torch.zeros(n, device=device, dtype=torch.float32)
        return ws

    def _versions(self, ts):
        return (_PACK_EPOCH,) + tuple((t._version, t.data_ptr()) for t in ts)

    def _cat_w(self):
        w = self.weights[0] if len(self.weights) == 1 else torch.cat([w.detach() for w in self.weights], 0)
        return w.detach().contiguous()

    def _pack(self, transposed, wino):
        L, g = H.lib(), (self.gates if not transposed else 1)
        w = self._cat_w()
        if wino == "head":
            out = torch.empty(L.ramnet_packed_weight_elems_head(self.Cin), device=w.device, dtype=torch.float32)
            H.check(L.ramnet_pack_weight_head(_p(w), _p(out), self.Cout, self.Cin, _st()), "ramnet_pack_weight_head")
            return out
        if wino == "2x4":
            out = torch.empty(L.ramnet_packed_weight_elems_wino2x4(self.Cout, self.Cin, transposed), device=w.device, dtype=torch.float32)
            H.check(L.ramnet_pack_weight_wino2x4(_p(w), _p(out), self.Cout, self.Cin, transposed, _st()), "ramnet_pack_weight_wino2x4")
            return out
        if wino == "2x4s":
            out = torch.empty(L.ramnet_packed_weight_elems_wino2x4_split(self.Cout, self.Cin, transposed), device=w.device, dtype=torch.float32)
            H.check(L.ramnet_pack_weight_wino2x4_split(_p(w), _p(out), self.Cout, self.Cin, transposed, _st()), "ramnet_pack_weight_wino2x4_split")
            return out
        if wino:
            n = L.ramnet_packed_weight_elems_wino(self.Cout, self.Cin, transposed, g)
            out = torch.empty(n, device=w.device, dtype=torch.float32)
            H.check(L.ramnet_pack_weight_wino(_p(w), _p(out), self.Cout, self.Cin, transposed, g, _st()), "ramnet_pack_weight_wino")
            return out
        n = L.ramnet_packed_weight_elems(self.Cout, self.Cin, self.k, self.k, transposed, g)
        out = torch.empty(n, device=w.device, dtype=torch.float32)
        H.check(L.ramnet_pack_weight(_p(w), _p(out), self.Cout, self.Cin, self.k, self.k, transposed, g, _st()), "ramnet_pack_weight")
        return out

    def pack(self, transposed, wino=False):
        v = self._versions(self.weights)
        wino = wino if wino in ("head", "2x4", "2x4s") else bool(wino)
        key = (transposed, wino)
        hit = self._packs.get(key)
        if hit is None or hit[0] != v:
            hit = self._packs[key] = (v, self._pack(transposed, wino))
        return hit[1]

    def fwd(self):
        return PackRef(self, 0)

    _FOLD_A = FOLD_A

    def pack_fold(self):
        v = (self._versions(self.weights), "fold")
        hit = self._packs.get("fold")
        if hit is None or hit[0] != v:
            w4 = fold_weights(self._cat_w()).reshape(self.Cout, self.Cin, 8, 8).float().contiguous()
            L = H.lib()
            out = torch.empty(L.ramnet_packed_weight_elems(self.Cout, self.Cin, 8, 8, 0, 1), device=w4.device)
            H.check(L.ramnet_pack_weight(_p(w4), _p(out), self.Cout, self.Cin, 8, 8, 0, 1, _st()), "ramnet_pack_weight")
            hit = self._packs["fold"] = (v, out)
        return hit[1]

    def pack_fold_wino(self):
        v = (self._versions(self.weights), "fold24")
        hit = self._packs.get("fold24")
        if hit is None or hit[0] != v:
            L, w = H.lib(), self._cat_w()
            out = torch.empty(L.ramnet_packed_weight_elems_fold_wino(self.Cout, self.Cin), device=w.device, dtype=torch.float32)
            H.check(L.ramnet_pack_weight_fold_wino(_p(w), _p(out), self.Cout, self.Cin, _st()), "ramnet_pack_weight_fold_wino")
            hit = self._packs["fold24"] = (v, out)
        return hit[1]

    def pack_fold_wino_dgrad(self):
        v = (self._versions(self.weights), "fold24d")
        hit = self._packs.get("fold24d")
        if hit is None or hit[0] != v:
            L, w = H.lib(), self._cat_w()
            out = torch.empty(L.ramnet_packed_weight_elems_fold_wino(self.Cout, self.Cin), device=w.device, dtype=torch.float32)
            H.check(L.ramnet_pack_weight_fold_wino_dgrad(_p(w), _p(out), self.Cout, self.Cin, _st()), "ramnet_pack_weight_fold_wino_dgrad")
            hit = self._packs["fold24d"] = (v, out)
        return hit[1]

    def _border_pack(self):
        v = (self._versions(self.weights), "border")
        hit = self._packs.get("border")
        if hit is None or hit[0] != v:
            w = self._cat_w()
            rows, cols = (torch.empty(2, 5 * self.Cin, 2 * self.Cout, device=w.device) for _ in range(2))
            rows_t, cols_t = (torch.empty(2, 2 * self.Cout, 5 * self.Cin, device=w.device) for _ in range(2))
            H.check(H.lib().ramnet_pack_border_weights(_p(w), _p(rows), _p(cols), _p(rows_t), _p(cols_t), self.Cout, self.Cin, _st()),
                    "ramnet_pack_border_weights")
            hit = self._packs["border"] = (v, (rows, cols, rows_t, cols_t))
        return hit[1]

    def border_weights(self):
        return self._border_pack()[:2]

    def border_weights_t(self):
        return self._border_pack()[2:]

    def bwd(self):
        return PackRef(self, 1)

    def s2d(self):
        if getattr(self, "_s2d", None) is None:
            self._s2d = S2DConvParam(self)
        return self._s2d

    def bias(self):
        if self.biases[0] is None:
            return None
        if len(self.biases) == 1:
            return self.biases[0].detach()
        v = self._versions(self.biases)
        if self._bias is None or v != self._vbias:
            self._bias, self._vbias = torch.cat([b.detach() for b in self.biases]).contiguous(), v
        return self._bias

    def grad_ws(self, wino_ok=False):
        if self._ws is None:
            dev = self.weights[0].device
            slots = 24 if self.k == 3 else self.k * self.k
            self._slabs = H.lib().ramnet_wgrad_wino_slabs(self.CinWs, self.Cout) if self.k == 3 else 1
            n6 = H.lib().ramnet_wgrad_wino2x4_ws_floats(self.CinWs, self.Cout) * H.lib().ramnet_wgrad_wino2x4_slabs(self.CinWs, self.Cout) if self.k == 3 else 0
            self._ws = torch.zeros(max(self._slabs * slots * self.CinWs * self.Cout, n6), device=dev)
            self._bws = torch.zeros(self._slabs * self.Cout, device=dev)
            self._ws.slabs = self._slabs
        _Engine.enter()
        if not self._dirty:
            self._ws.wino = bool(wino_ok and _WINOGRAD and self.k == 3
                                 and self.CinWs >= _WINO_MIN_CIN)
            self._ws.wino6 = bool(self._ws.wino and (_WGRAD_2X4 == "force" or (_WGRAD_2X4 == "auto" and _USE_SIDE))
                                  and (type(self) is ConvParam or (_S2D_2X4 and self.Cin >= 128)) and self.CinWs >= 64)
            self._ws.wg_dsplit = bool(self._ws.wino6 and _SPLIT_OPERANDS and _SPLIT_WGRAD)
            if self._ws.wg_dsplit:
                ns, nf = H.lib().ramnet_wgrad_dsplit_slabs(self.CinWs, self.Cout), H.lib().ramnet_wgrad_dsplit_ws_floats(self.CinWs, self.Cout)
                if self._ws.numel() < ns * nf or self._bws.numel() < ns * self.Cout:
                    old = self._ws
                    self._ws = torch.zeros(max(ns * nf, old.numel()), device=old.device)
                    self._ws.wg_dsplit = True
                    self._bws = torch.zeros(max(ns, self._slabs) * self.Cout, device=old.device)
                self._ws.wino = self._ws.wino6 = False
                self._ws.slabs = ns
            elif self._ws.wino6:
                self._ws.wino = False
                self._ws.slabs = min(self._slabs, H.lib().ramnet_wgrad_wino2x4_slabs(self.CinWs, self.Cout))
            else:
                self._ws.slabs = self._slabs
            self._ws.head_cin = self.Cin if (self.k == 5 and self.gates == 1 and len(self.weights) == 1
                                             and H.lib().ramnet_head_supported(self.Cin, self.Cout)) else 0
        _Engine.mark(self)
        self._ws_used = True
        return self._ws, self._bws

    def grad_ws_fold(self):
        assert len(self.weights) == 1 and self.k == 5
        dev = self.weights[0].device
        if self._bws is None:
            self._bws = torch.zeros(self.Cout, device=dev)
        if self._ws_fold is None:
            self._ws_fold = (torch.zeros(64 * self.CinWs * self.Cout, device=dev),
                             torch.zeros(2, 5 * self.Cin, 2 * self.Cout, device=dev),
                             torch.zeros(2, 5 * self.Cin, 2 * self.Cout, device=dev))
        _Engine.mark(self)
        self._fold_used = True
        return self._ws_fold + (self._bws,)

    def grad_ws_fold24(self):
        if getattr(self, "_ws_fold24", None) is None:
            self._ws_fold24 = torch.zeros(4 * 25 * self.CinWs * self.Cout, device=self.weights[0].device)
        self._fold24_used = True
        return self._ws_fold24

    def _finalize_fold(self):
        w4, wr, wc = self._ws_fold
        g = ensure_grad(self.weights[0])
        dU = self._ws_fold24 if getattr(self, "_fold24_used", False) else None
        H.check(H.lib().ramnet_fold_unpack_wgrad(_p(w4), _p(dU), _p(wr), _p(wc), _p(g), self.Cout, self.Cin, self.CinWs, _st()),
                "ramnet_fold_unpack_wgrad")
        self._fold24_used = False
        self._fold_used = False

    def discard(self):
        for t in (self._ws, self._bws, getattr(self, "_ws_fold24", None)) + tuple(self._ws_fold or ()):
            if t is not None:
                t.zero_()
        self._dirty = self._ws_used = self._fold_used = self._fold24_used = False

    def _join_slabs(self):
        w6, ds = getattr(self._ws, "wino6", False), getattr(self._ws, "wg_dsplit", False)
        ns = getattr(self._ws, "slabs", 1)
        if ns > 1 and (w6 or ds or getattr(self._ws, "wino", False)):
            n = (H.lib().ramnet_wgrad_wino2x4_ws_floats(self.CinWs, self.Cout) if w6 else
                 H.lib().ramnet_wgrad_dsplit_ws_floats(self.CinWs, self.Cout) if ds else 16 * self.CinWs * self.Cout)
            H.check(H.lib().ramnet_reduce_slabs(_p(self._ws), ns, n, _st()), "ramnet_reduce_slabs")
            H.check(H.lib().ramnet_reduce_slabs(_p(self._bws), ns, self.Cout, _st()), "ramnet_reduce_slabs")

    def _zero_ws(self):
        w6, wn, ds = getattr(self._ws, "wino6", False), getattr(self._ws, "wino", False), getattr(self._ws, "wg_dsplit", False)
        ns = getattr(self._ws, "slabs", 1)
        if w6:
            n = H.lib().ramnet_wgrad_wino2x4_ws_floats(self.CinWs, self.Cout)
        elif wn:
            n = 16 * self.CinWs * self.Cout
        elif ds:
            n = H.lib().ramnet_wgrad_dsplit_ws_floats(self.CinWs, self.Cout)
        else:
            n, ns = self.k * self.k * self.CinWs * self.Cout, 1
        joined = ns > 1 and (w6 or wn or ds)
        _zero_later(self._ws[:n if joined else min(self._ws.numel(), n * max(ns, 1))])
        _zero_later(self._bws[:self.Cout if joined else self._bws.numel()])

    def finalize(self):
        if self._fold_used:
            self._finalize_fold()
        if self._ws_used:
            self._join_slabs()
        if not self._ws_used:
            if self.biases[0] is not None and self.biases[0].shape[0] == self.Cout:
                ensure_grad(self.biases[0]).add_(self._bws[:self.Cout])
            _zero_later(self._bws)
            self._dirty = False
            return
        off = 0
        for w, b in zip(self.weights, self.biases):
            n = w.shape[0]
            g = ensure_grad(w)
            if getattr(self._ws, "wino6", False):
                H.check(H.lib().ramnet_unpack_wgrad_wino2x4(_p(self._ws), _p(g), n, self.Cin, self.CinWs, self.Cout, off, _st()),
                        "ramnet_unpack_wgrad_wino2x4")
            elif getattr(self._ws, "wg_dsplit", False):
                H.check(H.lib().ramnet_unpack_wgrad_dsplit(_p(self._ws), _p(g), n, self.Cin, self.CinWs, self.Cout, off, _st()),
                        "ramnet_unpack_wgrad_dsplit")
            elif getattr(self._ws, "wino", False):
                H.check(H.lib().ramnet_unpack_wgrad_wino(_p(self._ws), _p(g), n, self.Cin, self.CinWs, self.Cout, off, _st()),
                        "ramnet_unpack_wgrad_wino")
            else:
                H.check(H.lib().ramnet_unpack_wgrad(_p(self._ws), _p(g), n, self.Cin, self.CinWs, self.Cout, off,
                                                    self.k, self.k, _st()), "ramnet_unpack_wgrad")
            if b is not None and b.shape[0] == n:
                ensure_grad(b).add_(self._bws[off:off + n])
            off += n
        self._zero_ws()
        self._dirty = self._ws_used = False


class S2DConvParam(ConvParam):

    def __init__(self, parent):
        assert len(parent.weights) == 1 and parent.k == 5 and parent.gates == 1
        self.parent = parent
        self.weights, self.biases, self.gates = parent.weights, parent.biases, 1
        self.Cout, self.Cin, self.k = parent.Cout, 4 * parent.Cin, 3
        self.CinWs = self.Cin
        self._bias = self._ws = self._bws = None
        self._vbias = None
        self._ws_fold = None
        self._fold_used = self._ws_used = False
        self._packs = {}
        self._dirty = False
        self._defer = []

    def _cat_w(self):
        return s2d_weights(self.parent.weights[0].detach()).contiguous()

    def finalize(self):
        w, b = self.parent.weights[0], self.parent.biases[0]
        g3 = torch.zeros(self.Cout, self.Cin, 3, 3, device=w.device)
        L = H.lib()
        self._join_slabs()
        if getattr(self._ws, "wino6", False):
            H.check(L.ramnet_unpack_wgrad_wino2x4(_p(self._ws), _p(g3), self.Cout, self.Cin, self.CinWs, self.Cout, 0, _st()), "ramnet_unpack_wgrad_wino2x4")
        elif getattr(self._ws, "wg_dsplit", False):
            H.check(L.ramnet_unpack_wgrad_dsplit(_p(self._ws), _p(g3), self.Cout, self.Cin, self.CinWs, self.Cout, 0, _st()), "ramnet_unpack_wgrad_dsplit")
        elif getattr(self._ws, "wino", False):
            H.check(L.ramnet_unpack_wgrad_wino(_p(self._ws), _p(g3), self.Cout, self.Cin, self.CinWs, self.Cout, 0, _st()), "ramnet_unpack_wgrad_wino")
        else:
            H.check(L.ramnet_unpack_wgrad(_p(self._ws), _p(g3), self.Cout, self.Cin, self.CinWs, self.Cout, 0, 3, 3, _st()), "ramnet_unpack_wgrad")
        ensure_grad(w).add_(s2d_weights_adjoint(g3, self.parent.Cin))
        if b is not None:
            ensure_grad(b).add_(self._bws[:self.Cout])
        self._zero_ws()
        self._dirty = self._ws_used = False


def pack_input(x, device, crop=None):
    x = x.to(device=device, dtype=torch.float32).contiguous()
    B, Cc, Hh, W = x.shape
    cp = (Cc + 3) // 4 * 4
    if crop is not None and (crop.height_crop_size, crop.width_crop_size) != (Hh, W):
        assert (crop.height, crop.width) == (Hh, W), "full-frame mode: CropParameters built for %dx%d, input is %dx%d" % (crop.height, crop.width, Hh, W)
        out = torch.empty(B, crop.height_crop_size, crop.width_crop_size, cp, device=device)
        H.check(H.lib().ramnet_reflect_pad(_p(x), _p(out), B, Cc, Hh, W, cp, crop.padding_top, crop.padding_left, crop.height_crop_size,
                                           crop.width_crop_size, 1, _st()), "ramnet_reflect_pad")
        return out
    out = torch.empty(B, Hh, W, cp, device=device)
    H.check(H.lib().ramnet_nchw_to_nhwc_pad(_p(x), _p(out), B, Cc, Hh, W, cp, _st()), "ramnet_nchw_to_nhwc_pad")
    return out


class CropParameters:

    def __init__(self, width, height, num_encoders):
        from math import ceil, floor
        self.height, self.width, self.num_encoders = height, width, num_encoders
        f = 2 ** num_encoders
        self.width_crop_size = int(f * ceil(width / f))
        self.height_crop_size = int(f * ceil(height / f))
        self.padding_top = ceil(0.5 * (self.height_crop_size - height))
        self.padding_bottom = floor(0.5 * (self.height_crop_size - height))
        self.padding_left = ceil(0.5 * (self.width_crop_size - width))
        self.padding_right = floor(0.5 * (self.width_crop_size - width))
        self.cx, self.cy = floor(self.width_crop_size / 2), floor(self.height_crop_size / 2)
        self.ix0, self.ix1 = self.cx - floor(width / 2), self.cx + ceil(width / 2)
        self.iy0, self.iy1 = self.cy - floor(height / 2), self.cy + ceil(height / 2)

    @property
    def identity(self):
        return (self.height_crop_size, self.width_crop_size) == (self.height, self.width)

    def pad(self, x):
        x = x.to(device=torch.device("cuda", torch.cuda.current_device()), dtype=torch.float32).contiguous()
        B, Cc, Hh, W = x.shape
        assert (Hh, W) == (self.height, self.width)
        out = torch.empty(B, Cc, self.height_crop_size, self.width_crop_size, device=x.device)
        H.check(H.lib().ramnet_reflect_pad(_p(x), _p(out), B, Cc, Hh, W, 0, self.padding_top, self.padding_left, self.height_crop_size,
                                           self.width_crop_size, 0, _st()), "ramnet_reflect_pad")
        return out

    def crop(self, y):
        return y[..., self.iy0:self.iy1, self.ix0:self.ix1]


def gemm(a, b, out, trans_a=False, accumulate=False):
    nb, M, N = out.shape
    K = a.shape[1] if trans_a else a.shape[2]
    H.check(H.lib().ramnet_gemm(_p(a), _p(b), _p(out), M, N, K, a.stride(1), b.stride(1), out.stride(1), int(trans_a), int(accumulate),
                                nb, a.stride(0), b.stride(0), out.stride(0), _st()), "ramnet_gemm")


def gemm2(a1, b1, out1, a2, b2, out2, trans_a=False, accumulate=False):
    nb1, M1, N = out1.shape
    nb2, M2, N2 = out2.shape
    K1 = a1.shape[1] if trans_a else a1.shape[2]
    K2 = a2.shape[1] if trans_a else a2.shape[2]
    assert N == N2 and a1.stride(1) == a2.stride(1) and b1.stride(1) == b2.stride(1) and out1.stride(1) == out2.stride(1)
    H.check(H.lib().ramnet_gemm2(_p(a1), _p(b1), _p(out1), M1, a1.stride(0), b1.stride(0), out1.stride(0), nb1, _p(a2), _p(b2), _p(out2), M2,
                                 a2.stride(0), b2.stride(0), out2.stride(0), nb2, N, K1, K2, a1.stride(1), b1.stride(1), out1.stride(1),
                                 int(trans_a), int(accumulate), _st()), "ramnet_gemm2")


def _folded_upsample_conv(x, skip, cp, y, epi):
    L = H.lib()
    B, Hh, W, Cc = x.shape
    dev = x.device
    if Cc != cp.Cin:
        raise RuntimeError("folded upsample-conv needs un-padded input channels")
    H2, W2 = 2 * Hh, 2 * W
    xpad = torch.empty(B, Hh + 4, W + 4, Cc, device=dev)
    side = branch_stream(dev, 8) if (_USE_BRANCH and not torch.is_grad_enabled()) else None
    main = torch.cuda.current_stream()
    w_rows, w_cols = cp.border_weights()
    if side is not None:
        side.wait_stream(main)
    if side is not None:
        H.check(L.ramnet_pad2_sum(_p(x), _p(skip), _p(xpad), B, Hh, W, Cc, _st()), "ramnet_pad2_sum")
    with torch.cuda.stream(side if side is not None else main):
        a_rows = torch.empty(2, B * W2, 5 * Cc, device=dev)
        a_cols = torch.empty(2, B * H2, 5 * Cc, device=dev)
        if side is not None:
            H.check(L.ramnet_up2x_border_im2col(_p(x), _p(skip), _p(a_rows), _p(a_cols), B, Hh, W, Cc, _st()), "ramnet_up2x_border_im2col")
        else:
            H.check(L.ramnet_pad2_sum_im2col(_p(x), _p(skip), _p(xpad), _p(a_rows), _p(a_cols), B, Hh, W, Cc, _st()), "ramnet_pad2_sum_im2col")
        g_rows = torch.empty(2, B * W2, 2 * cp.Cout, device=dev)
        g_cols = torch.empty(2, B * H2, 2 * cp.Cout, device=dev)
        gemm2(a_rows, w_rows, g_rows, a_cols, w_cols, g_cols)
    if side is not None:
        main.wait_stream(side)
        if not torch.cuda.is_current_stream_capturing():
            for t in (x, skip):
                if t is not None:
                    t.record_stream(side)
            g_rows.record_stream(main), g_cols.record_stream(main)
    desc_kw = dict(bias=cp.bias(), epi=epi, frame=2, e0=g_cols.view(2 * B, H2, 1, 2 * cp.Cout), e1=g_rows.view(2 * B, W2, 1, 2 * cp.Cout))
    if _FOLD_WINO and _fold_wino_ok(Cc, cp.Cout):
        conv_launch(xpad, Taps.get("fold", 4, 0, 0, 0), cp.pack_fold_wino(), y, cp.Cout, Ho=Hh, Wo=W, wino24=True, ws_owner=cp, **desc_kw)
        return xpad
    conv_launch_multi(xpad, cp.pack_fold(), y, cp.Cout,
                      [(Taps.get("fold", 4, 0, py, px), Hh, W, (2, 2, py, px)) for py in range(2) for px in range(2)], **desc_kw)
    return xpad


_S2D = True


def set_space_to_depth(on):
    global _S2D
    _S2D = bool(on)


def get_space_to_depth():
    return _S2D


def _s2d_eligible(x, cp, k, stride, up):
    return bool(_S2D and _WINOGRAD and stride == 2 and k == 5 and not up and x.shape[1] % 2 == 0
                and x.shape[2] % 2 == 0 and x.shape[3] == cp.Cin and cp.Cin % 8 == 0 and cp.gates == 1 and len(cp.weights) == 1)


_S2D_FUSED = True
_S2D_SPARSE = True
_S2D_2X4 = _os.environ.get("RAMNET_S2D_2X4", "1") != "0"


def set_space_to_depth_2x4(on):
    global _S2D_2X4
    _S2D_2X4 = bool(on)


def set_space_to_depth_fused(on):
    global _S2D_FUSED
    _S2D_FUSED = bool(on)


def _s2d_fused(C):
    return bool(_S2D_FUSED and C >= 32 and C & (C - 1) == 0)


def _space_to_depth(x, inverse=False):
    B, Hh, W, Cc = x.shape
    out = torch.empty((B, 2 * Hh, 2 * W, Cc // 4) if inverse else (B, Hh // 2, W // 2, 4 * Cc), device=x.device)
    full = out if inverse else x
    H.check(H.lib().ramnet_space_to_depth2(_p(x), _p(out), B, full.shape[1], full.shape[2], full.shape[3], int(inverse), _st()),
            "ramnet_space_to_depth2")
    return out


def _fold_eligible(x, cp, k, stride, up):
    return bool(up and k == 5 and stride == 1 and _FOLD_UP and x.shape[1] >= 4 and x.shape[2] >= 4
                and x.shape[3] == cp.Cin)


def _folded_upsample_wgrad(x, skip, dy, y, cp, xpad=None):
    L = H.lib()
    B, Hh, W, Cc = x.shape
    H2, W2 = 2 * Hh, 2 * W
    dev = x.device
    w4, wr, wc, bws = cp.grad_ws_fold()
    with side_work([x, skip, dy, y, xpad], dev):
        a_rows = torch.empty(2, B * W2, 5 * Cc, device=dev)
        a_cols = torch.empty(2, B * H2, 5 * Cc, device=dev)
        if xpad is None:
            xpad = torch.empty(B, Hh + 4, W + 4, Cc, device=dev)
            H.check(L.ramnet_pad2_sum_im2col(_p(x), _p(skip), _p(xpad), _p(a_rows), _p(a_cols), B, Hh, W, Cc, _st()), "ramnet_pad2_sum_im2col")
        else:
            H.check(L.ramnet_up2x_border_im2col(_p(x), _p(skip), _p(a_rows), _p(a_cols), B, Hh, W, Cc, _st()), "ramnet_up2x_border_im2col")
        if _FOLD_WINO_WGRAD and Cc == cp.CinWs and ((Cc % 32 == 0 and cp.Cout % 64 == 0) or
                                                                                 (Cc % 64 == 0 and cp.Cout % 32 == 0)):
            wgrad_launch(xpad, Taps.get("fold", 4, 0, 0, 0), dy, cp.grad_ws_fold24(), cp.Cout, gmask=y, dbias=bws, Ho=Hh, Wo=W,
                         gview=(0, 0, 0, 0, H2, W2), wino24=True)
        else:
            for py in range(2):
                for px in range(2):
                    wgrad_launch(xpad, Taps.get("fold", 4, 0, py, px), dy, w4, cp.Cout, gmask=y, dbias=bws, Ho=Hh, Wo=W,
                                 gview=(2, 2, py, px, H2, W2), dw_off=(py * 2 + px) * 16 * cp.CinWs * cp.Cout)
        g_rows = torch.empty(2, B * W2, 2 * cp.Cout, device=dev)
        g_cols = torch.empty(2, B * H2, 2 * cp.Cout, device=dev)
        H.check(L.ramnet_frame_gather(_p(dy), _p(y), _p(g_rows), _p(g_cols), B, H2, W2, cp.Cout, _st()), "ramnet_frame_gather")
        gemm2(a_rows, g_rows, wr, a_cols, g_cols, wc, trans_a=True, accumulate=True)


_FOLD_DGRAD = True


def set_fold_dgrad(on):
    global _FOLD_DGRAD
    _FOLD_DGRAD = bool(on)


def _fold_dgrad_ok(B, H2, W2, cp):
    return bool(_FOLD_DGRAD and _FOLD_UP and cp.Cout % 16 == 0 and cp.Cin % 64 == 0
                and B * H2 * W2 * cp.Cout * 4 < 2 ** 30)


def _folded_upsample_dgrad(x, dy, y, cp):
    L = H.lib()
    B, Hh, W, Cc = x.shape
    H2, W2 = 2 * Hh, 2 * W
    dev = x.device
    g = dy
    if y is not None:
        g = torch.empty_like(dy)
        H.check(L.ramnet_relu_bwd(_p(dy), _p(y), _p(g), dy.numel(), _st()), "ramnet_relu_bwd")
    dxpad = torch.empty(B, Hh + 4, W + 4, Cc, device=dev)
    conv_launch(g, Taps.get("fold", 4, 0, 0, 0), cp.pack_fold_wino_dgrad(), dxpad, Cc, in_mode=H.IN_PARITY4, wino24=True)
    dx = torch.empty(B, Hh, W, Cc, device=dev)
    H.check(L.ramnet_unpad2_fold(_p(dxpad), _p(dx), B, Hh, W, Cc, _st()), "ramnet_unpad2_fold")
    g_rows = torch.empty(2, B * W2, 2 * cp.Cout, device=dev)
    g_cols = torch.empty(2, B * H2, 2 * cp.Cout, device=dev)
    H.check(L.ramnet_frame_gather(_p(g), None, _p(g_rows), _p(g_cols), B, H2, W2, cp.Cout, _st()), "ramnet_frame_gather")
    wt_rows, wt_cols = cp.border_weights_t()
    d_rows = torch.empty(2, B * W2, 5 * Cc, device=dev)
    d_cols = torch.empty(2, B * H2, 5 * Cc, device=dev)
    gemm2(g_rows, wt_rows, d_rows, g_cols, wt_cols, d_cols)
    H.check(L.ramnet_up2x_border_col2im(_p(d_rows), _p(d_cols), _p(dx), B, Hh, W, Cc, _st()), "ramnet_up2x_border_col2im")
    return dx


class ConvAct(Function):

    @staticmethod
    def forward(ctx, x, skip, w, b, cp, stride, relu, up):
        x, skip = dense(x), dense(skip)
        if skip is not None and skip.shape != x.shape:
            raise RuntimeError("skip connection %s does not match the decoder feature map %s (NHWC)" % (tuple(skip.shape), tuple(x.shape)))
        if x.shape[3] != (cp.Cin + 3) // 4 * 4:
            raise RuntimeError("conv expects %d input channels, got %d" % (cp.Cin, x.shape[3]))
        B, Hh, W, _ = x.shape
        k, pad = cp.k, cp.k // 2
        Hin, Win = (2 * Hh, 2 * W) if up else (Hh, W)
        Ho, Wo = (Hin + 2 * pad - k) // stride + 1, (Win + 2 * pad - k) // stride + 1
        y = torch.empty(B, Ho, Wo, cp.Cout, device=x.device)
        mode = (H.IN_UP2X_SKIP if skip is not None else H.IN_UP2X) if up else H.IN_PLAIN
        epi = H.EPI_RELU if relu else H.EPI_LINEAR
        xpad = None
        ctx.s2d = _s2d_eligible(x, cp, k, stride, up)
        ctx.s2d_fused = ctx.s2d and _s2d_fused(x.shape[3])
        if ctx.s2d_fused:
            conv_launch(x, Taps.get("conv_s2d", 3, 1), cp.s2d().fwd(), y, cp.Cout, in_mode=H.IN_S2D, Hin=Hh // 2, Win=W // 2,
                        bias=cp.bias(), epi=epi)
        elif ctx.s2d:
            x = _space_to_depth(x)
            conv_launch(x, Taps.get("conv_s2d", 3, 1), cp.s2d().fwd(), y, cp.Cout, bias=cp.bias(), epi=epi)
        elif _fold_eligible(x, cp, k, stride, up):
            xpad = _folded_upsample_conv(x, skip, cp, y, epi)
        else:
            conv_launch(x, Taps.get("conv", k, pad), cp.fwd(), y, cp.Cout, stride=stride, x1=skip, in_mode=mode,
                        Hin=Hin, Win=Win, bias=cp.bias(), epi=epi)
        ctx.cp, ctx.stride, ctx.relu, ctx.up, ctx.mode = cp, stride, relu, up, mode
        ctx.premask_ok, ctx.premasked = bool(relu), False
        ctx.save_for_backward(x, skip, y, xpad if _SAVE_XPAD else None)
        return y

    @staticmethod
    def backward(ctx, dy):
        x, skip, y, xpad = ctx.saved_tensors
        cp, stride, relu, up, mode = ctx.cp, ctx.stride, ctx.relu, ctx.up, ctx.mode
        relu = relu and not ctx.premasked
        dy = dense(dy)
        if ctx.s2d_fused:
            sp = cp.s2d()
            ws, bws = sp.grad_ws(wino_ok=True)
            Hl, Wl = x.shape[1] // 2, x.shape[2] // 2
            wgrad_side([x, dy, y], x, Taps.get("conv_s2d", 3, 1), dy, ws, cp.Cout, in_mode=H.IN_S2D, Hin=Hl, Win=Wl,
                       gmask=y if relu else None, dbias=bws)
            dx = None
            if ctx.needs_input_grad[0]:
                dx = torch.empty_like(x)
                conv_launch(dy, Taps.get("dgrad1_s2d", 3, 1), sp.bwd(), dx, sp.Cin, xm=y if relu else None,
                            in_mode=H.IN_RELUMASK if relu else H.IN_PLAIN, Ho=Hl, Wo=Wl, out_s2d=x.shape[3])
            return dx, None, None, None, None, None, None, None
        if ctx.s2d:
            sp = cp.s2d()
            ws, bws = sp.grad_ws(wino_ok=True)
            wgrad_side([x, dy, y], x, Taps.get("conv_s2d", 3, 1), dy, ws, cp.Cout, gmask=y if relu else None, dbias=bws)
            dx = None
            if ctx.needs_input_grad[0]:
                gs = torch.empty_like(x)
                conv_launch(dy, Taps.get("dgrad1_s2d", 3, 1), sp.bwd(), gs, sp.Cin, xm=y if relu else None,
                            in_mode=H.IN_RELUMASK if relu else H.IN_PLAIN)
                dx = _space_to_depth(gs, inverse=True)
            return dx, None, None, None, None, None, None, None
        B, Hh, W, _ = x.shape
        k, pad = cp.k, cp.k // 2
        Hin, Win = (2 * Hh, 2 * W) if up else (Hh, W)
        if _fold_eligible(x, cp, k, stride, up):
            dy = dy.contiguous()
            _folded_upsample_wgrad(x, skip, dy, y if relu else None, cp, xpad)
        else:
            ws, bws = cp.grad_ws(wino_ok=(stride == 1 and k == 3 and pad == 1 and mode == H.IN_PLAIN))
            wgrad_side([x, skip, dy, y], x, Taps.get("conv", k, pad), dy, ws, cp.Cout, stride=stride, x1=skip, in_mode=mode,
                       Hin=Hin, Win=Win, gmask=y if relu else None, dbias=bws)
        dx = dskip = None
        if (ctx.needs_input_grad[0] or (skip is not None and ctx.needs_input_grad[1])) and _fold_eligible(x, cp, k, stride, up) \
                and _fold_dgrad_ok(B, Hin, Win, cp):
            dx = _folded_upsample_dgrad(x, dy, y if relu else None, cp)
            return dx, (dx if skip is not None else None), None, None, None, None, None, None
        if ctx.needs_input_grad[0] or (skip is not None and ctx.needs_input_grad[1]):
            gin = torch.empty(B, Hin, Win, cp.Cin, device=x.device)
            gmode = H.IN_RELUMASK if relu else H.IN_PLAIN
            if stride == 1:
                conv_launch(dy, Taps.get("dgrad1", k, pad), cp.bwd(), gin, cp.Cin, xm=y if relu else None, in_mode=gmode)
            else:
                conv_launch_multi(dy, cp.bwd(), gin, cp.Cin,
                                  [(Taps.get("dgrad2", k, pad, py, px), (Hin - py + 1) // 2, (Win - px + 1) // 2, (2, 2, py, px))
                                   for py in range(2) for px in range(2)], xm=y if relu else None, in_mode=gmode)
            if up:
                dx = torch.empty(B, Hh, W, cp.Cin, device=x.device)
                H.check(H.lib().ramnet_upsample2x_bwd(_p(gin), _p(dx), B, Hh, W, cp.Cin, _st()), "ramnet_upsample2x_bwd")
            else:
                dx = gin
            dskip = dx if skip is not None else None
        return dx, dskip, None, None, None, None, None, None


class TConvAct(Function):

    @staticmethod
    def forward(ctx, x, w, b, cp, relu=True):
        x = dense(x)
        B, Hh, W, _ = x.shape
        Ct = cp.Cin
        y = torch.empty(B, 2 * Hh, 2 * W, Ct, device=x.device)
        conv_launch_multi(x, cp.bwd(), y, Ct, [(Taps.get("dgrad2", 5, 2, py, px), Hh, W, (2, 2, py, px))
                                               for py in range(2) for px in range(2)], bias=cp.bias(),
                          epi=H.EPI_RELU if relu else H.EPI_LINEAR)
        ctx.cp, ctx.relu = cp, relu
        ctx.save_for_backward(x, y)
        return y

    @staticmethod
    def backward(ctx, dy):
        x, y = ctx.saved_tensors
        cp = ctx.cp
        dy = dense(dy)
        B, Hh, W, Cx = x.shape
        taps = Taps.get("conv", 5, 2)
        ws, _ = cp.grad_ws()
        mask, mode = (y, H.IN_RELUMASK) if ctx.relu else (None, H.IN_PLAIN)
        wgrad_launch(dy, taps, x, ws, Cx, stride=2, xm=mask, in_mode=mode)
        if cp.biases[0] is not None:
            dyc = dy.contiguous()
            H.check(H.lib().ramnet_bias_grad(_p(dyc), _p(mask), _p(ensure_grad(cp.biases[0])), B * 4 * Hh * W, cp.Cin, _st()), "bias_grad")
        dx = None
        if ctx.needs_input_grad[0]:
            dx = torch.empty(B, Hh, W, Cx, device=x.device)
            conv_launch(dy, taps, cp.fwd(), dx, Cx, stride=2, xm=mask, in_mode=mode)
        return dx, None, None, None, None


class ResConv(Function):

    @staticmethod
    def forward(ctx, t, res, w, b, cp):
        t, res = dense(t), dense(res)
        assert t.shape == res.shape
        y = torch.empty_like(res, memory_format=torch.contiguous_format)
        conv_launch(t, Taps.get("conv", 3, 1), cp.fwd(), y, cp.Cout, bias=cp.bias(), epi=H.EPI_RES_RELU, e0=res)
        ctx.cp = cp
        ctx.save_for_backward(t, y)
        return y

    @staticmethod
    def backward(ctx, dy):
        t, y = ctx.saved_tensors
        cp = ctx.cp
        dy = dense(dy).contiguous()
        dpre = torch.empty_like(y)
        H.check(H.lib().ramnet_relu_bwd(_p(dy), _p(y), _p(dpre), y.numel(), _st()), "ramnet_relu_bwd")
        ws, bws = cp.grad_ws(wino_ok=True)
        wgrad_side([t, dpre], t, Taps.get("conv", 3, 1), dpre, ws, cp.Cout, dbias=bws)
        dt = torch.empty_like(t, memory_format=torch.contiguous_format)
        conv_launch(dpre, Taps.get("dgrad1", 3, 1), cp.bwd(), dt, cp.Cin)
        dres = dpre
        if _USE_SIDE:
            dres = torch.empty_like(y)
            H.check(H.lib().ramnet_relu_bwd(_p(dy), _p(y), _p(dres), y.numel(), _st()), "ramnet_relu_bwd")
        return dt, dres, None, None, None


def _norm_partial(a, y, act, b, groups):
    B, Hh, W, Cc = b.shape
    npix = B * Hh * W // groups
    L = H.lib()
    nslab = L.ramnet_norm_slabs(groups, npix, Cc)
    part = torch.empty(groups, nslab, Cc, 2, device=b.device, dtype=torch.float64)
    H.check(L.ramnet_norm_partial(_p(a), Cc, _p(y), Cc, act, _p(b), Cc, groups, npix, Cc, nslab, _p(part), _st()), "ramnet_norm_partial")
    return part, nslab, npix


def norm_stats(x, groups):
    part, _, npix = _norm_partial(x, None, 0, x, groups)
    s = part.sum(1)
    mean = s[..., 0] / npix
    return mean, (s[..., 1] / npix - mean * mean).clamp_(min=0.0)


class NormAct(Function):

    @staticmethod
    def forward(ctx, x, gamma, beta, res, mean, rstd, scale, shift, batch_stats, act):
        x, res = dense(x).contiguous(), (dense(res).contiguous() if res is not None else None)
        B, Hh, W, Cc = x.shape
        groups = mean.shape[0]
        y = torch.empty_like(x)
        H.check(H.lib().ramnet_norm_apply(_p(x), Cc, _p(scale), _p(shift), _p(res), Cc, act, _p(y), Cc, groups, B * Hh * W // groups, Cc,
                                          _st()), "ramnet_norm_apply")
        ctx.batch_stats, ctx.act, ctx.has_res = batch_stats, act, res is not None
        ctx.save_for_backward(x, y, gamma, mean, rstd)
        return y

    @staticmethod
    def backward(ctx, dy):
        x, y, gamma, mean, rstd = ctx.saved_tensors
        dy = dense(dy).contiguous()
        Cc = x.shape[3]
        groups, act, L = mean.shape[0], ctx.act, H.lib()
        part, nslab, npix = _norm_partial(dy, y if act else None, act, x, groups)
        c = torch.empty(3, groups, Cc, device=x.device)
        dgb = torch.empty(2, Cc, device=x.device) if gamma is not None else None
        H.check(L.ramnet_norm_finalize_bwd(_p(part), groups, nslab, Cc, npix, _p(mean), _p(rstd), _p(gamma.detach()) if gamma is not None else None,
                                           int(ctx.batch_stats), _p(c[0]), _p(c[1]), _p(c[2]), _p(dgb[0]) if dgb is not None else None,
                                           _p(dgb[1]) if dgb is not None else None, _st()), "ramnet_norm_finalize_bwd")
        dx = torch.empty_like(x)
        dres = torch.empty_like(x) if ctx.has_res else None
        H.check(L.ramnet_norm_bwd(_p(dy), Cc, _p(y) if act else None, Cc, act, _p(x), Cc, _p(c[0]), _p(c[1]), _p(c[2]), _p(dx), Cc, _p(dres), Cc,
                                  groups, npix, Cc, _st()), "ramnet_norm_bwd")
        return dx, (dgb[0] if dgb is not None else None), (dgb[1] if dgb is not None else None), dres, None, None, None, None, None, None


_ACT_CODE = {None: 0, "relu": 1, "sigmoid": 2}


def norm_act(x, layer, act=None, res=None):
    x = dense(x).contiguous()
    B, Hh, W, Cc = x.shape
    inst = isinstance(layer, torch.nn.InstanceNorm2d)
    tracked = layer.running_mean is not None
    use_input = layer.training or not tracked
    groups = (B if inst else 1) if use_input else 1
    npix = B * Hh * W // groups
    update = bool(tracked and layer.training)
    if update and npix < 2:
        raise ValueError("Expected more than 1 value per channel when training, got input size %s" % ([B, Cc, Hh, W],))
    if update and layer.momentum is None:
        raise NotImplementedError("cumulative moving average (momentum=None): the reference builds its norm layers with momentum 0.1")
    dev = x.device
    mr = torch.empty(2, groups, Cc, device=dev, dtype=torch.float64)
    ss = torch.empty(2, groups, Cc, device=dev)
    part, nslab = None, 0
    if use_input:
        part, nslab, _ = _norm_partial(x, None, 0, x, groups)
    g, b = layer.weight, layer.bias
    H.check(H.lib().ramnet_norm_finalize(_p(part), groups, nslab, Cc, npix, float(layer.eps), _p(g.detach()) if g is not None else None,
                                         _p(b.detach()) if b is not None else None, _p(layer.running_mean), _p(layer.running_var),
                                         float(layer.momentum or 0.0), int(update), int(not use_input),
                                         _p(layer.num_batches_tracked) if (update and not inst) else None,
                                         _p(mr[0]), _p(mr[1]), _p(ss[0]), _p(ss[1]), _st()), "ramnet_norm_finalize")
    return NormAct.apply(x, g, b, res, mr[0], mr[1], ss[0], ss[1], use_input, _ACT_CODE[act])


def active_mask(active, B, device):
    if active is None:
        return None
    if not torch.is_tensor(active) or active.dim() != 1 or active.shape[0] != B:
        raise ValueError("active: a bool / integer tensor of shape [%d] expected, got %s" % (
            B, tuple(active.shape) if torch.is_tensor(active) else type(active).__name__))
    if active.dtype.is_floating_point or active.is_complex():
        raise ValueError("active: a bool / integer tensor expected, got %s" % active.dtype)
    if active.device.type == "cpu":
        return (active != 0).to(torch.int32).to(device)
    if active.device != device:
        raise ValueError("active: on %s, the cell runs on %s" % (active.device, device))
    return active if (active.dtype == torch.int32 and active.is_contiguous()) else (active != 0).to(torch.int32).contiguous()


class GRUCell(Function):

    @staticmethod
    def forward(ctx, x, h, wu, bu, wr, br, wo, bo, cp_ur, cp_o, out=None, active=None):
        x, h = dense(x), dense(h)
        act = active_mask(active, x.shape[0], x.device)
        if x.shape != h.shape:
            raise RuntimeError("Sizes of tensors must match except in dimension 1. Expected %s but got %s (input vs state; "
                               "NHWC)" % (tuple(x.shape), tuple(h.shape)))
        B, Hh, W, Cc = x.shape
        taps = Taps.get("conv", 3, 1)
        ur = torch.empty(B, Hh, W, 2 * Cc, device=x.device)
        hr = torch.empty(B, Hh, W, Cc, device=x.device) if (_GRU_HR and Cc % 4 == 0) else None
        if hr is not None:
            conv_launch(x, taps, cp_ur.fwd(), ur, 2 * Cc, x1=h, in_mode=H.IN_CAT, C1=Cc, bias=cp_ur.bias(), epi=H.EPI_SIGMOID_HR, e1=h, o1=hr,
                        active=act)
        else:
            conv_launch(x, taps, cp_ur.fwd(), ur, 2 * Cc, x1=h, in_mode=H.IN_CAT, C1=Cc, bias=cp_ur.bias(), epi=H.EPI_SIGMOID, active=act)
        hn = torch.empty(B, Hh, W, Cc, device=x.device) if out is None else out
        if out is not None:
            if tuple(out.shape) != (B, Hh, W, Cc) or not out.is_contiguous() or out.dtype != torch.float32:
                raise RuntimeError("GRUCell: `out` must be a contiguous fp32 NHWC buffer of the state's shape")
            ctx.mark_dirty(out)
        need = any(ctx.needs_input_grad)
        o = torch.empty_like(hn) if need else None
        if hr is not None:
            conv_launch(x, taps, cp_o.fwd(), hn, Cc, x1=hr, in_mode=H.IN_CAT, C1=Cc, bias=cp_o.bias(), epi=H.EPI_GRU_BLEND, e0=ur, e1=h, o1=o,
                        active=act)
        else:
            conv_launch(x, taps, cp_o.fwd(), hn, Cc, x1=h, xm=ur, xm_off=Cc, in_mode=H.IN_CAT_MUL, C1=Cc, bias=cp_o.bias(),
                        epi=H.EPI_GRU_BLEND, e0=ur, e1=h, o1=o, active=act)
        ctx.cps = (cp_ur, cp_o)
# ... 517 lines not shown
```

Measured before the change: 237.3 samples/s.

## Add F(2x3) Winograd variant for folded upsample conv forward and dgrad

Adds a Winograd variant with a 3-wide output tile in the folded-upsample wino24 kernel, using 5x6 input tiles (30 transform positions instead of 25). It covers 50% more output columns per tile for about 20% more transform work, so MFMA work and input loads per output should drop. It comes with new weight packing kernels, a variant selector with auto/off/force modes, and a smaller prefetch ring. The variant disables split-K and raises register and LDS pressure, which may hurt occupancy or accuracy on some shapes.

```diff
diff --git a/include/ramnet_hip.h b/include/ramnet_hip.h
--- a/include/ramnet_hip.h
+++ b/include/ramnet_hip.h
@@ -7,7 +7,7 @@
 extern "C" {
 #endif
 
-#define RAMNET_ABI_VERSION 25
+#define RAMNET_ABI_VERSION 26
 #define RAMNET_E_BADARG 10001
 #define RAMNET_E_UNSUPPORTED 10002
 
@@ -23,7 +23,7 @@
 };
 
 enum ramnet_algo { RAMNET_ALGO_DIRECT = 0, RAMNET_ALGO_WINOGRAD = 1, RAMNET_ALGO_HEAD = 2, RAMNET_ALGO_WINOGRAD24 = 3, RAMNET_ALGO_WINOGRAD_2X4 = 4,
-                   RAMNET_ALGO_WINOGRAD_2X4_SPLIT = 5, RAMNET_ALGO_DIRECT_SPLIT = 6 };
+                   RAMNET_ALGO_WINOGRAD_2X4_SPLIT = 5, RAMNET_ALGO_DIRECT_SPLIT = 6, RAMNET_ALGO_WINOGRAD24_2X3 = 7 };
 
 enum ramnet_epilogue {
     RAMNET_EPI_LINEAR = 0,
@@ -131,6 +131,10 @@
 int ramnet_pack_weight_fold_wino(const float *w_oihw, float *wp, int Cout, int Cin, void *stream);
 int ramnet_pack_weight_fold_wino_dgrad(const float *w_oihw, float *wp, int Cout, int Cin, void *stream);
 int ramnet_pack_border_weights(const float *w_oihw, float *rows, float *cols, float *rows_t, float *cols_t, int Cout, int Cin, void *stream);
+int ramnet_fold_wino_variant(const ramnet_conv_desc *d, int force);
+size_t ramnet_packed_weight_elems_fold_wino2x3(int Cout, int Cin);
+int ramnet_pack_weight_fold_wino2x3(const float *w_oihw, float *wp, int Cout, int Cin, void *stream);
+int ramnet_pack_weight_fold_wino2x3_dgrad(const float *w_oihw, float *wp, int Cout, int Cin, void *stream);
 int ramnet_fold_unpack_wgrad(float *w4, float *dU, float *wr, float *wc, float *grad, int Cout, int Cin, int CinWs, void *stream);
 size_t ramnet_packed_weight_elems_head(int Cin);
 int ramnet_head_supported(int Cin, int Cout);
diff --git a/rpg_ramnet_amd/_hip.py b/rpg_ramnet_amd/_hip.py
--- a/rpg_ramnet_amd/_hip.py
+++ b/rpg_ramnet_amd/_hip.py
@@ -6,6 +6,7 @@
 
 IN_PLAIN, IN_CAT, IN_CAT_MUL, IN_UP2X, IN_UP2X_SKIP, IN_RELUMASK, IN_S2D, IN_PARITY4 = range(8)
 ALGO_DIRECT, ALGO_WINOGRAD, ALGO_HEAD, ALGO_WINOGRAD24, ALGO_WINOGRAD_2X4, ALGO_WINOGRAD_2X4_SPLIT, ALGO_DIRECT_SPLIT = 0, 1, 2, 3, 4, 5, 6
+ALGO_WINOGRAD24_2X3 = 7
 EPI_LINEAR, EPI_RELU, EPI_SIGMOID, EPI_RES_RELU, EPI_GRU_BLEND, EPI_LSTM, EPI_GRU_BWD, EPI_SIGMOID_HR = range(8)
 
 _fp = C.c_void_p
@@ -100,6 +101,10 @@
     "ramnet_packed_weight_elems_fold_wino": (C.c_size_t, [C.c_int, C.c_int]),
     "ramnet_pack_weight_fold_wino": (C.c_int, [_fp, _fp, C.c_int, C.c_int, _fp]),
     "ramnet_pack_weight_fold_wino_dgrad": (C.c_int, [_fp, _fp, C.c_int, C.c_int, _fp]),
+    "ramnet_fold_wino_variant": (C.c_int, [C.POINTER(ConvDesc), C.c_int]),
+    "ramnet_packed_weight_elems_fold_wino2x3": (C.c_size_t, [C.c_int, C.c_int]),
+    "ramnet_pack_weight_fold_wino2x3": (C.c_int, [_fp, _fp, C.c_int, C.c_int, _fp]),
+    "ramnet_pack_weight_fold_wino2x3_dgrad": (C.c_int, [_fp, _fp, C.c_int, C.c_int, _fp]),
     "ramnet_pack_border_weights": (C.c_int, [_fp] * 5 + [C.c_int, C.c_int, _fp]),
     "ramnet_fold_unpack_wgrad": (C.c_int, [_fp] * 5 + [C.c_int, C.c_int, C.c_int, _fp]),
     "ramnet_unpad2_fold": (C.c_int, [_fp, _fp, C.c_int, C.c_int, C.c_int, C.c_int, _fp]),
@@ -204,7 +209,7 @@
         for name, (res, args) in _SIGS.items():
             fn = getattr(l, name)
             fn.restype, fn.argtypes = res, args
-        if l.ramnet_abi_version() != 25:
+        if l.ramnet_abi_version() != 26:
             raise RuntimeError("ABI version mismatch in %s" % LIB_PATH)
         _lib = l
     return _lib if _tracer is None else _Traced(_lib)
diff --git a/rpg_ramnet_amd/csrc/conv_igemm.hip b/rpg_ramnet_amd/csrc/conv_igemm.hip
--- a/rpg_ramnet_amd/csrc/conv_igemm.hip
+++ b/rpg_ramnet_amd/csrc/conv_igemm.hip
@@ -207,7 +207,7 @@
     if (d.epi == RAMNET_EPI_LSTM) RAMNET_CHECK_ARG(d.o1 && d.bias);
     if (d.epi == RAMNET_EPI_GRU_BWD) RAMNET_CHECK_ARG(d.e0 && d.o1 && d.Cout % 8 == 0 && !d.bias && d.beta == 0.f && d.frame == 0 && d.out_s2d == 0);
     if (d.epi == RAMNET_EPI_SIGMOID_HR) RAMNET_CHECK_ARG(d.e1 && d.o1 && d.Cout % 8 == 0 && d.beta == 0.f && d.frame == 0 && d.out_s2d == 0 &&
-                                                         d.algo != RAMNET_ALGO_WINOGRAD24 && d.algo != RAMNET_ALGO_HEAD);
+                                                         d.algo != RAMNET_ALGO_WINOGRAD24 && d.algo != RAMNET_ALGO_WINOGRAD24_2X3 && d.algo != RAMNET_ALGO_HEAD);
     {
         unsigned long long ld = (unsigned long long)d.ld0;
         if (cat || d.in_mode == RAMNET_IN_UP2X_SKIP) ld = ld > (unsigned long long)d.ld1 ? ld : (unsigned long long)d.ld1;
@@ -308,7 +308,7 @@
         const int rc = check_desc(*dp);
         return rc ? rc : launch_wino6s(*dp, (hipStream_t)stream);
     }
-    if (dp->algo == RAMNET_ALGO_WINOGRAD24) {
+    if (dp->algo == RAMNET_ALGO_WINOGRAD24 || dp->algo == RAMNET_ALGO_WINOGRAD24_2X3) {
         const int rc = check_desc(*dp);
         return rc ? rc : launch_wino24(*dp, (hipStream_t)stream);
     }
diff --git a/rpg_ramnet_amd/csrc/conv_wino24.hip b/rpg_ramnet_amd/csrc/conv_wino24.hip
--- a/rpg_ramnet_amd/csrc/conv_wino24.hip
+++ b/rpg_ramnet_amd/csrc/conv_wino24.hip
@@ -8,6 +8,7 @@
 
 constexpr int W24_PS = 512;
 constexpr int W24_V = 25 * W24_PS;
+constexpr int W23_V = 30 * W24_PS;
 
 __device__ __forceinline__ float2 ld2f(const float *p) { return *reinterpret_cast<const float2 *>(p); }
 
@@ -38,13 +39,16 @@
     int *cnt;
 };
 
-template <int NCQ, bool DG, int TXW, bool PAIR = false>
+template <int NCQ, bool DG, int TXW, bool PAIR = false, int TW = 2>
 __global__ void __launch_bounds__(512, 1) conv_wino24_kernel(const ramnet_conv_desc p, const Wino24Params q) {
     static_assert(!PAIR || (NCQ == 4 && !DG), "pair mode: forward, 64-column workgroups");
+    static_assert(TW == 2 || (TW == 3 && NCQ == 4), "F(2x3): 64-column workgroups");
+    constexpr int WC = TW + 3, NP = 5 * WC;
+    constexpr int VSZ = NP * W24_PS;
     constexpr int W24_K = NCQ == 4 ? 16 : 8;
     constexpr int W24_TX = TXW, W24_TY = (NCQ == 4 ? 32 : 64) / TXW;
     constexpr int VEC = W24_K / 4;
-    constexpr int W24_U = 25 * NCQ * 64 * VEC;
+    constexpr int W24_U = NP * NCQ * 64 * VEC;
     extern __shared__ __attribute__((aligned(16))) float smem[];
     float *V = smem;
     const int tid = threadIdx.x, lane = tid & 63;
@@ -64,30 +68,32 @@
     const int n0 = nb * 16 * NCQ;
 
     const int it = tid / W24_K, ik = tid % W24_K;
-    const int iy0 = 2 * (tby * W24_TY + it / W24_TX) + py, ix0 = 2 * (tbx * W24_TX + it % W24_TX) + px;
-    unsigned rowo[5], colo[5];
+    const int iy0 = 2 * (tby * W24_TY + it / W24_TX) + py, ix0 = TW * (tbx * W24_TX + it % W24_TX) + px;
+    unsigned rowo[5], colo[WC];
     int cur_cls = -1;
     auto set_class = [&](int c) {
         cur_cls = c;
         const int cy = c >> 1, cx = c & 1;
-        const int u0 = 2 * (tby * W24_TY + it / W24_TX), v0 = 2 * (tbx * W24_TX + it % W24_TX);
-#pragma unroll
-        for (int r = 0; r < 5; ++r) {
+        const int u0 = 2 * (tby * W24_TY + it / W24_TX), v0 = TW * (tbx * W24_TX + it % W24_TX);
+#pragma unroll
+        for (int r = 0; r < WC; ++r) {
             const int i = u0 - cy - 3 + r, j = v0 - cx - 3 + r;
-            rowo[r] = (unsigned)i < (unsigned)q.Hc ? 4u * (unsigned)((b * q.Hp + 2 * i + cy) * q.Wp * q.ldx) : 0x40000000u;
+            if (r < 5) rowo[r] = (unsigned)i < (unsigned)q.Hc ? 4u * (unsigned)((b * q.Hp + 2 * i + cy) * q.Wp * q.ldx) : 0x40000000u;
             colo[r] = (unsigned)j < (unsigned)q.Wc ? 4u * (unsigned)((2 * j + cx) * q.ldx + ik) : 0x40000000u;
         }
     };
     if (!DG) {
 #pragma unroll
-        for (int r = 0; r < 5; ++r)
-            rowo[r] = 4u * (unsigned)((b * q.Hp + min(iy0 + r, q.Hp - 1)) * q.Wp * q.ldx), colo[r] = 4u * (unsigned)(min(ix0 + r, q.Wp - 1) * q.ldx + ik);
-    }
-    const int ksp = DG ? 1 : q.ksplit;
+        for (int r = 0; r < WC; ++r) {
+            if (r < 5) rowo[r] = 4u * (unsigned)((b * q.Hp + min(iy0 + r, q.Hp - 1)) * q.Wp * q.ldx);
+            colo[r] = 4u * (unsigned)(min(ix0 + r, q.Wp - 1) * q.ldx + ik);
+        }
+    }
+    const int ksp = (DG || TW != 2) ? 1 : q.ksplit;
     const int cps = ((q.nchunks / 2 + ksp - 1) / ksp) * 2, cbeg = DG ? 0 : (int)blockIdx.y * cps;
     const auto xrs = make_rsrc(q.x + cbeg * W24_K, q.xbytes - (unsigned)cbeg * W24_K * 4u);
     const int vdst = NCQ == 4 ? it * 16 + (((ik >> 2) ^ ((it >> 2) & 3)) << 2) + (ik & 3) : it * 8 + (((ik >> 1) ^ ((it >> 3) & 1)) << 1) + (ik & 1);
-    float raw[25];
+    float raw[5 * WC];
     auto load_raw = [&](int chunk) {
         int soff = chunk * (W24_K * 4);
         if (DG) {
@@ -98,8 +104,8 @@
 #pragma unroll
         for (int r = 0; r < 5; ++r)
 #pragma unroll
-            for (int c = 0; c < 5; ++c)
-                raw[r * 5 + c] = __builtin_bit_cast(float, __builtin_amdgcn_raw_buffer_load_b32(xrs, (int)(rowo[r] + colo[c]), soff, 0));
+            for (int c = 0; c < WC; ++c)
+                raw[r * WC + c] = __builtin_bit_cast(float, __builtin_amdgcn_raw_buffer_load_b32(xrs, (int)(rowo[r] + colo[c]), soff, 0));
     };
     int lr_soff = 0;
     auto load_row_begin = [&](int chunk) {
@@ -112,25 +118,36 @@
     };
     auto load_row = [&](int r) {
 #pragma unroll
-        for (int c = 0; c < 5; ++c)
-            raw[r * 5 + c] = __builtin_bit_cast(float, __builtin_amdgcn_raw_buffer_load_b32(xrs, (int)(rowo[r] + colo[c]), lr_soff, 0));
+        for (int c = 0; c < WC; ++c)
+            raw[r * WC + c] = __builtin_bit_cast(float, __builtin_amdgcn_raw_buffer_load_b32(xrs, (int)(rowo[r] + colo[c]), lr_soff, 0));
     };
     auto tr_col = [&](int c) {
-        const float d0 = raw[c], d1 = raw[5 + c], d2 = raw[10 + c], d3 = raw[15 + c], d4 = raw[20 + c];
+        const float d0 = raw[c], d1 = raw[WC + c], d2 = raw[2 * WC + c], d3 = raw[3 * WC + c], d4 = raw[4 * WC + c];
         raw[c] = 2.f * (d0 - d2) - d1 + d3;
-        raw[5 + c] = d3 - d2 - 2.f * d1;
-        raw[10 + c] = 2.f * d1 - 3.f * d2 + d3;
-        raw[15 + c] = d3 - d1;
-        raw[20 + c] = 2.f * (d1 - d3) - d2 + d4;
+        raw[WC + c] = d3 - d2 - 2.f * d1;
+        raw[2 * WC + c] = 2.f * d1 - 3.f * d2 + d3;
+        raw[3 * WC + c] = d3 - d1;
+        raw[4 * WC + c] = 2.f * (d1 - d3) - d2 + d4;
     };
     auto tr_row = [&](float *vbuf, int i) {
-        const float d0 = raw[i * 5], d1 = raw[i * 5 + 1], d2 = raw[i * 5 + 2], d3 = raw[i * 5 + 3], d4 = raw[i * 5 + 4];
-        float *dst = vbuf + (i * 5) * W24_PS + vdst;
-        dst[0 * W24_PS] = 2.f * (d0 - d2) - d1 + d3;
-        dst[1 * W24_PS] = d3 - d2 - 2.f * d1;
-        dst[2 * W24_PS] = 2.f * d1 - 3.f * d2 + d3;
-        dst[3 * W24_PS] = d3 - d1;
-        dst[4 * W24_PS] = 2.f * (d1 - d3) - d2 + d4;
+        float *dst = TW == 2 ? vbuf + (i * WC) * W24_PS + vdst : vbuf + (i * WC) * W24_PS;
+        if constexpr (TW == 2) {
+            const float d0 = raw[i * 5], d1 = raw[i * 5 + 1], d2 = raw[i * 5 + 2], d3 = raw[i * 5 + 3], d4 = raw[i * 5 + 4];
+            dst[0 * W24_PS] = 2.f * (d0 - d2) - d1 + d3;
+            dst[1 * W24_PS] = d3 - d2 - 2.f * d1;
+            dst[2 * W24_PS] = 2.f * d1 - 3.f * d2 + d3;
+            dst[3 * W24_PS] = d3 - d1;
+            dst[4 * W24_PS] = 2.f * (d1 - d3) - d2 + d4;
+        } else {
+            const float d0 = raw[i * 6], d1 = raw[i * 6 + 1], d2 = raw[i * 6 + 2], d3 = raw[i * 6 + 3], d4 = raw[i * 6 + 4], d5 = raw[i * 6 + 5];
+            const float u = d3 - d1, v = d4 - d2;
+            dst[0 * W24_PS] = fmaf(-1.25f, d2, fmaf(0.25f, d0, d4));
+            dst[1 * W24_PS] = fmaf(-0.25f, d1 + d2, d3 + d4);
+            dst[2 * W24_PS] = fmaf(0.25f, d1 - d2, d4 - d3);
+            dst[3 * W24_PS] = fmaf(0.5f, u, v);
+            dst[4 * W24_PS] = fmaf(-0.5f, u, v);
+            dst[5 * W24_PS] = fmaf(-1.25f, d3, fmaf(0.25f, d1, d5));
+        }
     };
 
     const int tile = th * 16 + l15;
@@ -153,22 +170,25 @@
         }
     };
     const int wchunk = q.nblk * W24_U * 4;
-
-    f32x4 acc[25];
-#pragma unroll
-    for (int i = 0; i < 25; ++i) acc[i] = f32x4{0.f, 0.f, 0.f, 0.f};
+    int abuf1 = VSZ + aoff, dbuf1 = VSZ + vdst;
+    if constexpr (TW == 3) asm volatile("" : "+v"(abuf1), "+v"(dbuf1));
+
+    f32x4 acc[NP];
+#pragma unroll
+    for (int i = 0; i < NP; ++i) acc[i] = f32x4{0.f, 0.f, 0.f, 0.f};
 
     const int nch = DG ? q.nchunks : min(cps, q.nchunks - cbeg);
     W24_STAMP(16, 0);
     load_raw(0);
-    constexpr int RING = 10, DIST = 8;
+    constexpr int RING = TW == 2 || DG ? 10 : 6, DIST = RING - 2;
+    static_assert((2 * NP) % RING == 0, "ring slots repeat every chunk pair");
     float4 bq[RING];
 #pragma unroll
     for (int i = 0; i < DIST; ++i) bq[i] = ldw(wsrc + i * (WPOS * 4));
 #pragma unroll
-    for (int c = 0; c < 5; ++c) tr_col(c);
-#pragma unroll
-    for (int i = 0; i < 5; ++i) tr_row(V, i);
+    for (int c = 0; c < WC; ++c) tr_col(c);
+#pragma unroll
+    for (int i = 0; i < 5; ++i) tr_row(TW == 2 ? V : V + vdst, i);
     load_raw(min(1, nch - 1));
     __syncthreads();
 
@@ -177,23 +197,27 @@
 #pragma unroll
         for (int half = 0; half < 2; ++half) {
             const int chunk = chunk0 + half;
-            const float *vb = V + half * W24_V;
-            float *vn = V + (half ^ 1) * W24_V;
+            const float *vb = V + half * VSZ;
+            float *vn = TW == 2 ? V + (half ^ 1) * VSZ : V + (half ? vdst : dbuf1);
+            auto lda = [&](int pos) {
+                if constexpr (TW == 2) return ldv(vb + pos * W24_PS + aoff);
+                else return ldv(V + (half ? abuf1 : aoff) + pos * W24_PS);
+            };
             const int cnext = min(chunk + 1, nch - 1), cnext2 = min(chunk + 2, nch - 1);
             const int wcur = wsrc + chunk * wchunk, wnext = wsrc + cnext * wchunk;
             W24_STAMP(chunk, 0);
             float4 aq[2][2];
-            aq[0][0] = ldv(vb + aoff), aq[0][1] = ldv(vb + W24_PS + aoff);
-#pragma unroll
-            for (int pp = 0; pp < 13; ++pp) {
-                const int pos = 2 * pp, g = half * 25 + pos;
-                const bool two = pos + 1 < 25;
-                if (pos + 2 < 25) aq[(pp + 1) & 1][0] = ldv(vb + (pos + 2) * W24_PS + aoff);
-                if (pos + 3 < 25) aq[(pp + 1) & 1][1] = ldv(vb + (pos + 3) * W24_PS + aoff);
+            aq[0][0] = lda(0), aq[0][1] = lda(1);
+#pragma unroll
+            for (int pp = 0; pp < (NP + 1) / 2; ++pp) {
+                const int pos = 2 * pp, g = half * NP + pos;
+                const bool two = pos + 1 < NP;
+                if (pos + 2 < NP) aq[(pp + 1) & 1][0] = lda(pos + 2);
+                if (pos + 3 < NP) aq[(pp + 1) & 1][1] = lda(pos + 3);
                 const float4 a0 = aq[pp & 1][0], a1 = aq[pp & 1][1];
 #if !defined(W24_ABLATE) || !(W24_ABLATE & 2)
-                bq[(g + DIST) % RING] = pos + DIST < 25 ? ldw(wcur + (pos + DIST) * (WPOS * 4)) : ldw(wnext + (pos + DIST - 25) * (WPOS * 4));
-                if (two) bq[(g + 1 + DIST) % RING] = pos + 1 + DIST < 25 ? ldw(wcur + (pos + 1 + DIST) * (WPOS * 4)) : ldw(wnext + (pos + 1 + DIST - 25) * (WPOS * 4));
+                bq[(g + DIST) % RING] = pos + DIST < NP ? ldw(wcur + (pos + DIST) * (WPOS * 4)) : ldw(wnext + (pos + DIST - NP) * (WPOS * 4));
+                if (two) bq[(g + 1 + DIST) % RING] = pos + 1 + DIST < NP ? ldw(wcur + (pos + 1 + DIST) * (WPOS * 4)) : ldw(wnext + (pos + 1 + DIST - NP) * (WPOS * 4));
 #endif
                 const float4 b0 = bq[g % RING], b1 = bq[(g + 1) % RING];
                 __builtin_amdgcn_sched_barrier(0);
@@ -202,16 +226,17 @@
                 acc[pos] = __builtin_amdgcn_mfma_f32_16x16x4f32(a0.y, b0.y, acc[pos], 0, 0, 0);
                 if (two) acc[pos + 1] = __builtin_amdgcn_mfma_f32_16x16x4f32(a1.y, b1.y, acc[pos + 1], 0, 0, 0);
                 __builtin_amdgcn_sched_barrier(0);
+                constexpr int R0 = 4 + WC;
                 auto slot = [&](int sl) {
                     if (sl == 4) W24_STAMP(chunk, 1);
-                    if (sl >= 4 && sl <= 8) tr_col(sl - 4);
-                    if (sl == 9) W24_STAMP(chunk, 2);
-                    if (sl >= 9 && sl <= 17 && (sl & 1)) tr_row(vn, (sl - 9) >> 1);
+                    if (sl >= 4 && sl < R0) tr_col(sl - 4);
+                    if (sl == R0) W24_STAMP(chunk, 2);
+                    if (sl >= R0 && sl <= R0 + 8 && !((sl - R0) & 1)) tr_row(vn, (sl - R0) >> 1);
 #if !defined(W24_ABLATE) || !(W24_ABLATE & 1)
-                    if (sl == 10) load_row_begin(cnext2);
-                    if (sl >= 10 && sl <= 18 && !(sl & 1)) load_row((sl - 10) >> 1);
+                    if (sl == R0 + 1) load_row_begin(cnext2);
+                    if (sl > R0 && sl <= R0 + 9 && ((sl - R0) & 1)) load_row((sl - R0 - 1) >> 1);
 #endif
-                    if (sl == 18) W24_STAMP(chunk, 3);
+                    if (sl == R0 + 9) W24_STAMP(chunk, 3);
                 };
                 slot(2 * pp);
                 __builtin_amdgcn_sched_barrier(0);
@@ -238,22 +263,29 @@
     const int epi = p.epi;
     const float bias_n = (!DG && p.bias) ? p.bias[n] : 0.f;
     const bool relu = epi == RAMNET_EPI_RELU;
-    float ov[16];
-    size_t op[16];
-    bool oo[16];
+    constexpr int NOUT = 8 * TW;
+    float ov[NOUT];
+    size_t op[NOUT];
+    bool oo[NOUT];
 #pragma unroll
     for (int r = 0; r < 4; ++r) {
-        float s[2][5];
-#pragma unroll
-        for (int j = 0; j < 5; ++j) {
-            const float m0 = acc[j][r], m1 = acc[5 + j][r], m2 = acc[10 + j][r], m3 = acc[15 + j][r], m4 = acc[20 + j][r];
+        float s[2][WC];
+#pragma unroll
+        for (int j = 0; j < WC; ++j) {
+            const float m0 = acc[j][r], m1 = acc[WC + j][r], m2 = acc[2 * WC + j][r], m3 = acc[3 * WC + j][r], m4 = acc[4 * WC + j][r];
             s[0][j] = m0 + m1 + m2 + m3;
             s[1][j] = m1 - m2 + 2.f * m3 + m4;
         }
 #pragma unroll
         for (int a2 = 0; a2 < 2; ++a2) {
-            ov[(r * 2 + a2) * 2] = s[a2][0] + s[a2][1] + s[a2][2] + s[a2][3];
-            ov[(r * 2 + a2) * 2 + 1] = s[a2][1] - s[a2][2] + 2.f * s[a2][3] + s[a2][4];
+            if constexpr (TW == 2) {
+                ov[(r * 2 + a2) * 2] = s[a2][0] + s[a2][1] + s[a2][2] + s[a2][3];
+                ov[(r * 2 + a2) * 2 + 1] = s[a2][1] - s[a2][2] + 2.f * s[a2][3] + s[a2][4];
+            } else {
+                ov[(r * 2 + a2) * 3] = s[a2][0] + s[a2][1] + s[a2][2] + s[a2][3] + s[a2][4];
+                ov[(r * 2 + a2) * 3 + 1] = fmaf(0.5f, s[a2][3] - s[a2][4], s[a2][1] - s[a2][2]);
+                ov[(r * 2 + a2) * 3 + 2] = fmaf(0.25f, s[a2][3] + s[a2][4], s[a2][1] + s[a2][2]) + s[a2][5];
+            }
         }
     }
     if (!DG && ksp > 1) {
@@ -285,12 +317,12 @@
 #pragma unroll
     for (int r = 0; r < 4; ++r) {
         const int t = th * 16 + 4 * ks + r;
-        const int oy0 = 2 * (tby * W24_TY + t / W24_TX), ox0 = 2 * (tbx * W24_TX + t % W24_TX) - (PAIR ? pxc : 0);
+        const int oy0 = 2 * (tby * W24_TY + t / W24_TX), ox0 = TW * (tbx * W24_TX + t % W24_TX) - (PAIR ? pxc : 0);
 #pragma unroll
         for (int a2 = 0; a2 < 2; ++a2) {
 #pragma unroll
-            for (int c2 = 0; c2 < 2; ++c2) {
-                const int oy = oy0 + a2, ox = ox0 + c2, idx = (r * 2 + a2) * 2 + c2;
+            for (int c2 = 0; c2 < TW; ++c2) {
+                const int oy = oy0 + a2, ox = ox0 + c2, idx = (r * 2 + a2) * TW + c2;
                 if (DG) {
                     oo[idx] = oy < p.Ho && ox < p.Wo;
                     op[idx] = (((size_t)b * p.Ho + oy) * p.Wo + ox) * p.ldo + n;
@@ -306,16 +338,25 @@
         }
     }
 #pragma unroll
-    for (int idx = 0; idx < 16; ++idx)
+    for (int idx = 0; idx < NOUT; ++idx)
         if (oo[idx]) p.out[op[idx]] = ov[idx];
     W24_STAMP(16, 3);
 }
 
+__device__ __forceinline__ double fold_wino_gc(int tw, int b, int s) {
+    const double G[5][4] = {{0.5, 0, 0, 0}, {-0.5, -0.5, -0.5, -0.5}, {-1.0 / 6, 1.0 / 6, -1.0 / 6, 1.0 / 6}, {1.0 / 6, 1.0 / 3, 2.0 / 3, 4.0 / 3}, {0, 0, 0, 1}};
+    const double G3[6][4] = {{4, 0, 0, 0}, {2.0 / 3, 2.0 / 3, 2.0 / 3, 2.0 / 3}, {2.0 / 3, -2.0 / 3, 2.0 / 3, -2.0 / 3},
+                             {-8.0 / 3, -4.0 / 3, -2.0 / 3, -1.0 / 3}, {-8.0 / 3, 4.0 / 3, -2.0 / 3, 1.0 / 3}, {0, 0, 0, 1}};
+    return tw == 2 ? G[b][s] : G3[b][s];
+}
+
+template <int TW>
 __global__ void pack_weight_fold_wino_kernel(const float *__restrict__ w, float *__restrict__ wp, int Cout, int Cin, int kc, int ncq,
                                              int pair, size_t total) {
     const double FA[2][4][5] = {{{.25, 0, 0, 0, 0}, {.75, .75, .25, 0, 0}, {0, .25, .75, .75, .25}, {0, 0, 0, .25, .75}},
                                 {{.75, .25, 0, 0, 0}, {.25, .75, .75, .25, 0}, {0, 0, .25, .75, .75}, {0, 0, 0, 0, .25}}};
     const double G[5][4] = {{0.5, 0, 0, 0}, {-0.5, -0.5, -0.5, -0.5}, {-1.0 / 6, 1.0 / 6, -1.0 / 6, 1.0 / 6}, {1.0 / 6, 1.0 / 3, 2.0 / 3, 4.0 / 3}, {0, 0, 0, 1}};
+    constexpr int WC = TW + 3, NP = 5 * WC;
     const int vec = kc / 4, nblk = pair ? 1 : Cout / (16 * ncq), nch = Cin / kc;
     for (size_t i = blockIdx.x * (size_t)blockDim.x + threadIdx.x; i < total; i += (size_t)gridDim.x * blockDim.x) {
         size_t r = i;
@@ -327,18 +368,18 @@
         r /= 4;
         const int cq = (int)(r % ncq);
         r /= ncq;
-        const int pos = (int)(r % 25);
-        r /= 25;
+        const int pos = (int)(r % NP);
+        r /= NP;
         const int nb = (int)(r % nblk);
         r /= nblk;
         const int chunk = (int)(r % nch), cls = (int)(r / nch);
         const int k = chunk * kc + ks * vec + j, col = (nb * ncq + cq) * 16 + l15;
         const int n = pair ? col & 31 : col;
-        const int py = pair ? cls : cls >> 1, px = pair ? col >> 5 : cls & 1, a = pos / 5, b = pos % 5;
+        const int py = pair ? cls : cls >> 1, px = pair ? col >> 5 : cls & 1, a = pos / WC, b = pos % WC;
         double ga[5], gb[5];
         for (int kh = 0; kh < 5; ++kh) {
             ga[kh] = 0, gb[kh] = 0;
-            for (int t = 0; t < 4; ++t) ga[kh] += G[a][t] * FA[py][t][kh], gb[kh] += G[b][t] * FA[px][t][kh];
+            for (int t = 0; t < 4; ++t) ga[kh] += G[a][t] * FA[py][t][kh], gb[kh] += fold_wino_gc(TW, b, t) * FA[px][t][kh];
         }
         double u = 0;
         const float *wk = w + ((size_t)n * Cin + k) * 25;
@@ -355,6 +396,31 @@
 static bool fold_wino_geometry(int Cout, int Cin, int &kc, int &ncq) {
     kc = ((Cout % 64 == 0 && Cin % 16 == 0) || fold_wino_pair(Cout, Cin)) ? 16 : 8, ncq = kc == 16 ? 4 : 2;
     return Cout % 32 == 0 && Cin % (2 * kc) == 0;
+}
+
+static long wino23_tile(int Ho, int Wt, int &tx) {
+    const int shapes[3] = {4, 2, 16};
+    long best = -1;
+    for (int s = 0; s < 3; ++s) {
+        const int t = shapes[s], th = 2 * (32 / t), tw = 3 * t;
+        const long a = (long)cdiv(Ho, th) * th * cdiv(Wt, tw) * tw;
+        if (best < 0 || a < best) best = a, tx = t;
+    }
+    return best;
+}
+
+template <bool DG, bool PAIR>
+static int launch_wino23(int tx, dim3 grid, size_t lds, const ramnet_conv_desc &d, const Wino24Params &q, hipStream_t st) {
+#define W23_GO(T)                                                                                                         \
+    if (tx == T) {                                                                                                        \
+        RAMNET_FULL_LDS((conv_wino24_kernel<4, DG, T, PAIR, 3>));                                                           \
+        note_kernel("conv_wino24_kernel<4,%d,%d,%d,3>", (int)DG, T, (int)PAIR);                                            \
+        hipLaunchKernelGGL((conv_wino24_kernel<4, DG, T, PAIR, 3>), grid, dim3(512), lds, st, d, q);                        \
+    }
+    W23_GO(2) W23_GO(4) W23_GO(16)
+#undef W23_GO
+    RAMNET_LAUNCH_CHECK();
+    return 0;
 }
 
 static int launch_wino24_dgrad(const ramnet_conv_desc &d, hipStream_t st) {
@@ -366,9 +432,16 @@
     q.cpc = d.C0 / 16, q.nchunks = 4 * q.cpc, q.nblk = d.Cout / 64;
     q.ksplit = 1, q.ws = nullptr, q.cnt = nullptr;
     q.Hc = d.Hin / 2, q.Wc = d.Win / 2;
-    const size_t xb = (size_t)d.B * d.Hin * d.Win * d.ld0 * sizeof(float), wb = (size_t)100 * d.C0 * d.Cout * sizeof(float);
+    const bool w23 = d.algo == RAMNET_ALGO_WINOGRAD24_2X3;
+    const size_t xb = (size_t)d.B * d.Hin * d.Win * d.ld0 * sizeof(float), wb = (size_t)(w23 ? 120 : 100) * d.C0 * d.Cout * sizeof(float);
     RAMNET_CHECK_ARG(xb < 0x40000000ull && wb < 0x7fffffffull);
     q.xbytes = (unsigned)xb, q.wbytes = (unsigned)wb;
+    if (w23) {
+        int tx;
+        wino23_tile(d.Ho, d.Wo, tx);
+        q.tiles_x = cdiv(d.Wo, 3 * tx), q.tiles_y = cdiv(d.Ho, 64 / tx);
+        return launch_wino23<true, false>(tx, dim3((unsigned)(q.tiles_x * q.tiles_y * d.B * q.nblk)), (size_t)2 * W23_V * sizeof(float), d, q, st);
+    }
     const bool flat = cdiv(d.Wo, 16) * cdiv(d.Ho, 8) < cdiv(d.Wo, 8) * cdiv(d.Ho, 16);
     q.tiles_x = cdiv(d.Wo, flat ? 16 : 8), q.tiles_y = cdiv(d.Ho, flat ? 8 : 16);
     const size_t lds = (size_t)2 * W24_V * sizeof(float);
@@ -412,6 +485,30 @@
     return ks > 1 ? wino24_ksplit_floats(gridx, ks) : 0;
 }
 
+static int fold_wino_variant(const ramnet_conv_desc &d, int force) {
+    if (d.algo != RAMNET_ALGO_WINOGRAD24 || d.stride != 1) return 0;
+    long wgs22, wgs23;
+    int tx;
+    if (d.in_mode == RAMNET_IN_PARITY4) {
+        if (d.C0 % 16 != 0 || d.Cout % 64 != 0) return 0;
+        const bool flat = cdiv(d.Wo, 16) * cdiv(d.Ho, 8) < cdiv(d.Wo, 8) * cdiv(d.Ho, 16);
+        wgs22 = (long)cdiv(d.Wo, flat ? 16 : 8) * cdiv(d.Ho, flat ? 8 : 16) * d.B * (d.Cout / 64);
+        wgs23 = wino23_tile(d.Ho, d.Wo, tx) / 192 * d.B * (d.Cout / 64);
+    } else if (d.in_mode == RAMNET_IN_PLAIN) {
+        const bool pair = fold_wino_pair(d.Cout, d.C0), wide = pair || (d.Cout % 64 == 0 && d.C0 % 16 == 0);
+        if (!wide || d.C0 % 32 != 0 || d.Ho < 2 || d.Wo < 2) return 0;
+        const int Wt = pair ? d.Wo + 2 : d.Wo, nblk = pair ? 1 : d.Cout / 64, ncls = pair ? 2 : 4;
+        const bool flat = cdiv(Wt, 16) * cdiv(d.Ho, 8) < cdiv(Wt, 8) * cdiv(d.Ho, 16);
+        wgs22 = (long)cdiv(Wt, flat ? 16 : 8) * cdiv(d.Ho, flat ? 8 : 16) * d.B * nblk * ncls;
+        wgs23 = wino23_tile(d.Ho, pair ? d.Wo + 1 : d.Wo, tx) / 192 * d.B * nblk * ncls;
+        if (!force && wino24_ksplit(d, (int)wgs22, d.C0 / 16) > 1) return 0;
+    } else {
+        return 0;
+    }
+    if (force) return 1;
+    return wgs23 >= 256 && 6 * ((wgs23 + 255) / 256) < 5 * ((wgs22 + 255) / 256) ? 1 : 0;
+}
+
 int launch_wino24(const ramnet_conv_desc &d, hipStream_t st) {
     if (d.in_mode == RAMNET_IN_PARITY4) return launch_wino24_dgrad(d, st);
     RAMNET_CHECK_ARG(d.in_mode == RAMNET_IN_PLAIN && d.stride == 1);
@@ -420,13 +517,24 @@
     RAMNET_CHECK_ARG(d.C0 % (wide ? 32 : 16) == 0);
     RAMNET_CHECK_ARG(d.C0 % 8 == 0 && d.Cout % 32 == 0 && d.Hin == d.Ho + 4 && d.Win == d.Wo + 4 && d.HoF == 2 * d.Ho && d.WoF == 2 * d.Wo);
     RAMNET_CHECK_ARG((d.epi == RAMNET_EPI_RELU || d.epi == RAMNET_EPI_LINEAR) && d.beta == 0.f && d.out_s2d == 0 && d.Ho >= 2 && d.Wo >= 2);
+    const bool w23 = d.algo == RAMNET_ALGO_WINOGRAD24_2X3;
+    if (w23) RAMNET_CHECK_ARG(wide && d.splitk_ws == nullptr);
     Wino24Params q;
     q.x = d.x0, q.wp = d.w, q.Hp = d.Hin, q.Wp = d.Win, q.ldx = d.ld0;
     q.nchunks = d.C0 / (wide ? 16 : 8), q.nblk = pair ? 1 : d.Cout / (wide ? 64 : 32);
     q.Hc = d.Ho, q.Wc = d.Wo, q.cpc = 1;
-    const size_t xb = (size_t)d.B * d.Hin * d.Win * d.ld0 * sizeof(float), wb = (size_t)100 * d.C0 * d.Cout * sizeof(float);
+    const size_t xb = (size_t)d.B * d.Hin * d.Win * d.ld0 * sizeof(float), wb = (size_t)(w23 ? 120 : 100) * d.C0 * d.Cout * sizeof(float);
     RAMNET_CHECK_ARG(xb < 0xffffffffull && wb < 0x7fffffffull);
     q.xbytes = (unsigned)xb, q.wbytes = (unsigned)wb;
+    if (w23) {
+        int tx;
+        wino23_tile(d.Ho, pair ? d.Wo + 1 : d.Wo, tx);
+        q.tiles_x = cdiv(pair ? d.Wo + 1 : d.Wo, 3 * tx), q.tiles_y = cdiv(d.Ho, 64 / tx);
+        q.ksplit = 1, q.ws = nullptr, q.cnt = nullptr;
+        const dim3 grid((unsigned)(q.tiles_x * q.tiles_y * d.B * q.nblk * (pair ? 2 : 4)));
+        const size_t lds = (size_t)2 * W23_V * sizeof(float);
+        return pair ? launch_wino23<false, true>(tx, grid, lds, d, q, st) : launch_wino23<false, false>(tx, grid, lds, d, q, st);
+    }
     const int Wt = pair ? d.Wo + 2 : d.Wo;
     const bool flat = wide && cdiv(Wt, 16) * cdiv(d.Ho, 8) < cdiv(Wt, 8) * cdiv(d.Ho, 16);
     q.tiles_x = cdiv(Wt, wide && !flat ? 8 : 16), q.tiles_y = cdiv(d.Ho, flat ? 8 : 16);
@@ -463,24 +571,26 @@
     return 0;
 }
 
+template <int TW>
 __global__ void pack_weight_fold_wino_dgrad_kernel(const float *__restrict__ w, float *__restrict__ wp, int Cout, int Cin, size_t total) {
     const double FA[2][4][5] = {{{.25, 0, 0, 0, 0}, {.75, .75, .25, 0, 0}, {0, .25, .75, .75, .25}, {0, 0, 0, .25, .75}},
                                 {{.75, .25, 0, 0, 0}, {.25, .75, .75, .25, 0}, {0, 0, .25, .75, .75}, {0, 0, 0, 0, .25}}};
     const double G[5][4] = {{0.5, 0, 0, 0}, {-0.5, -0.5, -0.5, -0.5}, {-1.0 / 6, 1.0 / 6, -1.0 / 6, 1.0 / 6}, {1.0 / 6, 1.0 / 3, 2.0 / 3, 4.0 / 3}, {0, 0, 0, 1}};
+    constexpr int WC = TW + 3, NP = 5 * WC;
     const int NB = Cin / 64;
     for (size_t i = blockIdx.x * (size_t)blockDim.x + threadIdx.x; i < total; i += (size_t)gridDim.x * blockDim.x) {
         size_t r = i;
         const int j = (int)(r & 3), l15 = (int)((r >> 2) & 15), ks = (int)((r >> 6) & 3), cq = (int)((r >> 8) & 3);
         r >>= 10;
-        const int pos = (int)(r % 25);
-        r /= 25;
+        const int pos = (int)(r % NP);
+        r /= NP;
         const int nb = (int)(r % NB), chunk = (int)(r / NB);
         const int k = chunk * 16 + ks * 4 + j, c = nb * 64 + cq * 16 + l15;
-        const int pq = k / Cout, n = k - pq * Cout, pp = pq >> 1, qq = pq & 1, a = pos / 5, b = pos % 5;
+        const int pq = k / Cout, n = k - pq * Cout, pp = pq >> 1, qq = pq & 1, a = pos / WC, b = pos % WC;
         double ga[5], gb[5];
         for (int kh = 0; kh < 5; ++kh) {
             ga[kh] = 0, gb[kh] = 0;
-            for (int t = 0; t < 4; ++t) ga[kh] += G[a][t] * FA[pp][3 - t][kh], gb[kh] += G[b][t] * FA[qq][3 - t][kh];
+            for (int t = 0; t < 4; ++t) ga[kh] += G[a][t] * FA[pp][3 - t][kh], gb[kh] += fold_wino_gc(TW, b, t) * FA[qq][3 - t][kh];
         }
         double u = 0;
         const float *wk = w + ((size_t)n * Cin + c) * 25;
@@ -583,7 +693,7 @@
     const size_t total = (size_t)100 * Cout * Cin;
     size_t blocks = (total + 255) / 256;
     if (blocks > 65535) blocks = 65535;
-    hipLaunchKernelGGL(pack_weight_fold_wino_kernel, dim3((unsigned)blocks), dim3(256), 0, (hipStream_t)stream, w, wp, Cout, Cin, kc, ncq,
+    hipLaunchKernelGGL(pack_weight_fold_wino_kernel<2>, dim3((unsigned)blocks), dim3(256), 0, (hipStream_t)stream, w, wp, Cout, Cin, kc, ncq,
                        (int)fold_wino_pair(Cout, Cin), total);
     RAMNET_LAUNCH_CHECK();
     return 0;
@@ -594,10 +704,36 @@
     const size_t total = (size_t)100 * Cout * Cin;
     size_t blocks = (total + 255) / 256;
     if (blocks > 65535) blocks = 65535;
-    hipLaunchKernelGGL(pack_weight_fold_wino_dgrad_kernel, dim3((unsigned)blocks), dim3(256), 0, (hipStream_t)stream, w, wp, Cout, Cin, total);
-    RAMNET_LAUNCH_CHECK();
-    return 0;
-}
+    hipLaunchKernelGGL(pack_weight_fold_wino_dgrad_kernel<2>, dim3((unsigned)blocks), dim3(256), 0, (hipStream_t)stream, w, wp, Cout, Cin, total);
+    RAMNET_LAUNCH_CHECK();
+    return 0;
+}
+
+extern "C" size_t ramnet_packed_weight_elems_fold_wino2x3(int Cout, int Cin) { return (size_t)120 * Cout * Cin; }
+
+extern "C" int ramnet_pack_weight_fold_wino2x3(const float *w, float *wp, int Cout, int Cin, void *stream) {
+    int kc, ncq;
+    RAMNET_CHECK_ARG(w && wp && Cout > 0 && Cin > 0 && fold_wino_geometry(Cout, Cin, kc, ncq) && kc == 16);
+    const size_t total = (size_t)120 * Cout * Cin;
+    size_t blocks = (total + 255) / 256;
+    if (blocks > 65535) blocks = 65535;
+    hipLaunchKernelGGL(pack_weight_fold_wino_kernel<3>, dim3((unsigned)blocks), dim3(256), 0, (hipStream_t)stream, w, wp, Cout, Cin, kc, ncq,
+                       (int)fold_wino_pair(Cout, Cin), total);
+    RAMNET_LAUNCH_CHECK();
+    return 0;
+}
+
+extern "C" int ramnet_pack_weight_fold_wino2x3_dgrad(const float *w, float *wp, int Cout, int Cin, void *stream) {
+    RAMNET_CHECK_ARG(w && wp && Cout > 0 && Cin > 0 && Cin % 64 == 0 && (4 * Cout) % 16 == 0);
+    const size_t total = (size_t)120 * Cout * Cin;
+    size_t blocks = (total + 255) / 256;
+    if (blocks > 65535) blocks = 65535;
+    hipLaunchKernelGGL(pack_weight_fold_wino_dgrad_kernel<3>, dim3((unsigned)blocks), dim3(256), 0, (hipStream_t)stream, w, wp, Cout, Cin, total);
+    RAMNET_LAUNCH_CHECK();
+    return 0;
+}
+
+extern "C" int ramnet_fold_wino_variant(const ramnet_conv_desc *d, int force) { return d ? fold_wino_variant(*d, force) : 0; }
 
 extern "C" int ramnet_pack_border_weights(const float *w, float *rows, float *cols, float *rows_t, float *cols_t, int Cout, int Cin, void *stream) {
     RAMNET_CHECK_ARG(w && rows && cols && rows_t && cols_t && Cout > 0 && Cin > 0);
diff --git a/rpg_ramnet_amd/ops.py b/rpg_ramnet_amd/ops.py
--- a/rpg_ramnet_amd/ops.py
+++ b/rpg_ramnet_amd/ops.py
@@ -131,6 +131,15 @@
 def set_fold_winograd(on):
     global _FOLD_WINO
     _FOLD_WINO = bool(on)
+
+
+_FOLD_2X3 = "auto"
+
+
+def set_fold_winograd_2x3(mode):
+    global _FOLD_2X3
+    assert mode in ("auto", "off", "force")
+    _FOLD_2X3 = mode
 
 
 def set_fold_upsample(on):
@@ -278,7 +287,7 @@
     key = (id(taps), id(w.cp) if is_ref else 0, w.transposed if is_ref else -1, id(ws_owner), Cout, stride, in_mode, C0, C1, Hin, Win, epi, beta, Ho,
            Wo, os, out_off, frame, out_s2d, wino24, xm_off, tuple(x0.shape), x0.stride(2), _sd(x1), _sd(xm), out.shape[1], out.shape[2],
            out.stride(2), _sd(e0), _sd(e1), _sd(o1), _sd(o2), bias is None, al & 15, _WINOGRAD, _WINO_2X4, _SPLIT_OPERANDS, _HEAD, _S2D_SPARSE, _S2D_2X4,
-           _DESC_EPOCH, x0.device.index)
+           _FOLD_2X3, _DESC_EPOCH, x0.device.index)
     hit = _DESC_CACHE.get(key) if _DESC_CACHE_ON else None
     if hit is not None and (not is_ref or hit[3]() is w.cp) and (ws_owner is None or hit[4]() is ws_owner):
         tmpl, kind, nsplit = hit[0], hit[1], hit[2]
@@ -286,7 +295,10 @@
         d.x0, d.x1, d.xm = _p(x0), _p(x1), _p(xm, xm_off)
         d.bias, d.e0, d.e1 = _p(bias), _p(e0), _p(e1)
         d.out, d.o1, d.o2 = _p(out, out_off), _p(o1), _p(o2)
-        d.w = _p(w) if kind is None else _p(w.cp.pack(0, "head") if kind == "head" else w.cp.pack(w.transposed, kind))
+        if kind in ("f23", "f23d"):
+            d.w = _p(ws_owner.pack_fold_wino2x3_dgrad() if kind == "f23d" else ws_owner.pack_fold_wino2x3())
+        else:
+            d.w = _p(w) if kind is None else _p(w.cp.pack(0, "head") if kind == "head" else w.cp.pack(w.transposed, kind))
         if nsplit:
             d.splitk_ws = _p((w.cp if is_ref else ws_owner).splitk_ws(nsplit, x0.device))
         return d
@@ -347,6 +359,10 @@
         if _SPLIT_OPERANDS and H.lib().ramnet_conv_wino_split_ok(C.byref(d), int(_WINO_2X4 == "force")):
             d.algo, kind = H.ALGO_WINOGRAD_2X4_SPLIT, "2x4s"
         d.w = _p(ref.cp.pack(ref.transposed, kind))
+    if wino24 and cp is not None and _FOLD_2X3 != "off" and H.lib().ramnet_fold_wino_variant(C.byref(d), int(_FOLD_2X3 == "force")):
+        kind = "f23d" if in_mode == H.IN_PARITY4 else "f23"
+        d.algo = H.ALGO_WINOGRAD24_2X3
+        d.w = _p(cp.pack_fold_wino2x3_dgrad() if kind == "f23d" else cp.pack_fold_wino2x3())
     if d.algo in (H.ALGO_WINOGRAD, H.ALGO_WINOGRAD24) and cp is not None:
         n = H.lib().ramnet_conv_splitk_floats(C.byref(d))
         if n:
@@ -796,6 +812,26 @@
             out = torch.empty(L.ramnet_packed_weight_elems_fold_wino(self.Cout, self.Cin), device=w.device, dtype=torch.float32)
             H.check(L.ramnet_pack_weight_fold_wino_dgrad(_p(w), _p(out), self.Cout, self.Cin, _st()), "ramnet_pack_weight_fold_wino_dgrad")
             hit = self._packs["fold24d"] = (v, out)
+        return hit[1]
+
+    def pack_fold_wino2x3(self):
+        v = (self._versions(self.weights), "fold23")
+        hit = self._packs.get("fold23")
+        if hit is None or hit[0] != v:
+            L, w = H.lib(), self._cat_w()
+            out = torch.empty(L.ramnet_packed_weight_elems_fold_wino2x3(self.Cout, self.Cin), device=w.device, dtype=torch.float32)
+            H.check(L.ramnet_pack_weight_fold_wino2x3(_p(w), _p(out), self.Cout, self.Cin, _st()), "ramnet_pack_weight_fold_wino2x3")
+            hit = self._packs["fold23"] = (v, out)
+        return hit[1]
+
+    def pack_fold_wino2x3_dgrad(self):
+        v = (self._versions(self.weights), "fold23d")
+        hit = self._packs.get("fold23d")
+        if hit is None or hit[0] != v:
+            L, w = H.lib(), self._cat_w()
+            out = torch.empty(L.ramnet_packed_weight_elems_fold_wino2x3(self.Cout, self.Cin), device=w.device, dtype=torch.float32)
+            H.check(L.ramnet_pack_weight_fold_wino2x3_dgrad(_p(w), _p(out), self.Cout, self.Cin, _st()), "ramnet_pack_weight_fold_wino2x3_dgrad")
+            hit = self._packs["fold23d"] = (v, out)
         return hit[1]
 
     def _border_pack(self):
@@ -1210,7 +1246,7 @@
         g = torch.empty_like(dy)
         H.check(L.ramnet_relu_bwd(_p(dy), _p(y), _p(g), dy.numel(), _st()), "ramnet_relu_bwd")
     dxpad = torch.empty(B, Hh + 4, W + 4, Cc, device=dev)
-    conv_launch(g, Taps.get("fold", 4, 0, 0, 0), cp.pack_fold_wino_dgrad(), dxpad, Cc, in_mode=H.IN_PARITY4, wino24=True)
+    conv_launch(g, Taps.get("fold", 4, 0, 0, 0), cp.pack_fold_wino_dgrad(), dxpad, Cc, in_mode=H.IN_PARITY4, wino24=True, ws_owner=cp)
     dx = torch.empty(B, Hh, W, Cc, device=dev)
     H.check(L.ramnet_unpad2_fold(_p(dxpad), _p(dx), B, Hh, W, Cc, _st()), "ramnet_unpad2_fold")
     g_rows = torch.empty(2, B * W2, 2 * cp.Cout, device=dev)
```

Measured after the change: 244.3 samples/s (median of 6 runs). +3.0%, better.
